# fluent/fluent-bit

Hardware: AMD Instinct MI355X
Metric: log records/sec (256B apache-combined lines) through parser+grep (higher is better)
Workload: dtype u8

## Files before the change

fluent-bit_amd/__init__.py:

```python
import ctypes
import os
import subprocess
from ctypes import (POINTER, Structure, byref, c_char_p, c_double, c_int, c_int64, c_size_t, c_uint,
                    c_uint64, c_void_p)

_HERE = os.path.dirname(os.path.abspath(__file__))
CSRC = os.path.join(_HERE, "csrc")
LIB_PATH = os.environ.get("FLBGPU_LIB") or os.path.join(CSRC, "libflbgpu.so")

MODIFIED, NOTOUCH = 1, 2


def build(force=False):
    if force:
        subprocess.run(["make", "-C", CSRC, "clean"], check=True, stdout=subprocess.DEVNULL)
    subprocess.run(["make", "-j8", "-C", CSRC, "all"], check=True)


class DevChunk(Structure):
    _fields_ = [("data", c_void_p), ("row_off", c_void_p), ("n", c_uint64), ("bytes", c_uint64)]


_L = None

# ... 134 lines not shown
def init(device=0):
    global _inited
    if lib().flbgpu_init(device) != 0:
        raise RuntimeError("flbgpu_init: " + last_error())
    _inited = True


class Parser:

    def __init__(self, regex=None, time_fmt=None, time_key=None, time_offset=None, time_keep=False,
                 time_strict=True, skip_empty=True, types=None, name="parser", format="regex", no_bare_keys=False, decoders=None,
                 time_zone=None, time_system_timezone=False):
        if format in ("logfmt", "ltsv"):
            self.h = lib().flbgpu_parser_create_kv(_b(name), _b(format), _b(time_fmt), _b(time_key), _b(time_offset), int(time_keep),
                                                   int(time_strict), int(no_bare_keys), _b(types))
        elif format == "json":
            self.h = lib().flbgpu_parser_create_json(_b(name), _b(time_fmt), _b(time_key), _b(time_offset), int(time_keep),
                                                     int(time_strict))
        else:
            self.h = lib().flbgpu_parser_create(_b(name), _b(regex), int(skip_empty), _b(time_fmt), _b(time_key),
                                                _b(time_offset), int(time_keep), int(time_strict), _b(types))
        if not self.h:
            raise ValueError("flbgpu_parser_create: " + last_error())
        for d in decoders or []:
            if lib().flbgpu_parser_add_decoder(self.h, int(bool(d[0])), _b(d[1]), _b(d[2]), _b(d[3] if len(d) > 3 else None)) != 0:
                raise ValueError("flbgpu_parser_add_decoder: " + last_error())
        if time_system_timezone and lib().flbgpu_parser_set_system_timezone(self.h, 1) != 0:
            err = last_error(); self.close()
            raise ValueError("flbgpu_parser_set_system_timezone: " + err)
        if time_zone and lib().flbgpu_parser_set_time_zone(self.h, _b(time_zone)) != 0:
            err = last_error(); self.close()
            raise ValueError("flbgpu_parser_set_time_zone: " + err)

    def do(self, buf):
        out = c_void_p(); sz = c_size_t(); sec = c_int64(); nsec = c_int64()
        r = lib().flbgpu_parser_do(self.h, buf, len(buf), byref(out), byref(sz), byref(sec), byref(nsec))
        if r < 0:
            return r, None, None
        data = ctypes.string_at(out, sz.value)
        _libc.free(out)
        return r, data, (sec.value, nsec.value)

    def close(self):
        if self.h:
            lib().flbgpu_parser_destroy(self.h)
            self.h = None


class _Filter:
    h = None

    def filter(self, data):
        out = c_void_p(); sz = c_size_t()
        r = lib().flbgpu_filter_run(self.h, data, len(data), byref(out), byref(sz))
        if r != MODIFIED:
            return r, None
        b = ctypes.string_at(out, sz.value) if sz.value else b""
        if out.value:
            _libc.free(out)
        return r, b

    def filter_dev(self, chunk, stream=None):
        out = DevChunk()
        r = lib().flbgpu_filter_run_dev(self.h, byref(chunk), byref(out), stream)
        return r, out

    def counts(self):
        a = c_uint64(); b = c_uint64()
        lib().flbgpu_filter_last_counts(self.h, byref(a), byref(b))
        return a.value, b.value

    def regex_corners(self):
        return int(lib().flbgpu_filter_regex_corners(self.h))

    def host_rules(self):
        o = (ctypes.c_uint64 * 4)()
        lib().flbgpu_filter_host_rules(self.h, o)
        return dict(rules=int(o[0]), values=int(o[1]), budget_over=int(o[2]), unhandled=int(o[3]))

    def paths(self):
        o = (ctypes.c_uint64 * 8)()
        lib().flbgpu_filter_paths(self.h, o)
        lp = int(o[0])
        return dict(single_pass=bool(lp & 1), three_port=bool(lp & 2), emit_time=bool(lp & 4), plain_emit=bool(lp & 8), rows_by_length=bool(lp & 16),
                    aside=dict(single_pass=bool(o[1]), three_port=bool(o[2]), emit_time=bool(o[3]), plain_emit=bool(o[4])),
                    tries=int(o[5]), returns=int(o[6]), calls=int(o[7]))

    def profile(self, enable=True):
        lib().flbgpu_filter_profile(self.h, int(enable))

    def profile_read(self):
        names = (c_char_p * 16)(); ms = (c_double * 16)(); ln = (c_uint64 * 16)()
        n = lib().flbgpu_filter_profile_read(self.h, 16, names, ms, ln)
        return {names[i].decode(): (ms[i], ln[i]) for i in range(n)}

    def close(self):
        if self.h:
            lib().flbgpu_filter_destroy(self.h)
            self.h = None


class FilterParser(_Filter):

    def __init__(self, key_name, parsers, reserve_data=False, preserve_key=False):
        self.parsers = list(parsers)
        arr = (c_void_p * len(parsers))(*[p.h for p in parsers])
        self.h = lib().flbgpu_filter_parser_create(_b(key_name), int(reserve_data), int(preserve_key), len(parsers), arr)
        if not self.h:
            raise ValueError("flbgpu_filter_parser_create: " + last_error())


class FilterGrep(_Filter):

    def __init__(self, rules, logical_op=None):
        n = len(rules)
        kinds = (c_char_p * max(n, 1))(*[_b(k) for k, _ in rules])
        vals = (c_char_p * max(n, 1))(*[_b(v) for _, v in rules])
        self.h = lib().flbgpu_filter_grep_create(n, kinds, vals, _b(logical_op))
        if not self.h:
            raise ValueError("flbgpu_filter_grep_create: " + last_error())


def _props(props):
    n = len(props)
    names = (c_char_p * max(n, 1))(*[_b(k) for k, _ in props])
    vals = (c_char_p * max(n, 1))(*[_b(v) for _, v in props])
    return n, names, vals


class FilterModify(_Filter):

    def __init__(self, props):
        self.h = lib().flbgpu_filter_modify_create(*_props(props))
        if not self.h:
            raise ValueError("flbgpu_filter_modify_create: " + last_error())

    def overread(self):
        return int(lib().flbgpu_modify_overread(self.h))


def modify_parse_check(props):
    buf = ctypes.create_string_buffer(1 << 16)
    if lib().flbgpu_modify_parse_check(*_props(props), buf, len(buf)) != 0:
        raise ValueError(last_error())
    return buf.value.decode()


class FilterRecordModifier(_Filter):

    def __init__(self, props):
        self.h = lib().flbgpu_filter_record_modifier_create(*_props(props))
        if not self.h:
            raise ValueError("flbgpu_filter_record_modifier_create: " + last_error())


def record_modifier_parse_check(props):
    buf = ctypes.create_string_buffer(1 << 17)
    if lib().flbgpu_record_modifier_parse_check(*_props(props), buf, len(buf)) != 0:
        raise ValueError(last_error())
    return buf.value.decode()


JSON_FORMAT = {"json": 1, "stream": 2, "lines": 3}
JSON_DATE = {"double": 0, "iso8601": 1, "epoch": 2, "java_sql_timestamp": 3, "epoch_ms": 4}


class JsonFormatter(_Filter):
# ... 767 lines not shown
```

fluent-bit_amd/csrc/flbgpu.cpp:

```cpp
#include <condition_variable>
#include <functional>
#include <atomic>
#include <chrono>
#include <mutex>
#include <thread>
#include "host_int.hpp"
#include "grep_lane.hpp"
#include "perm.hpp"

using namespace flbgpu;

static thread_local std::string g_err;
static int g_cus = 0;

int flbgpu::device_cus() { return g_cus; }

void flbgpu::set_err(const char *fmt, ...) {
    char buf[1024];
    va_list ap;
    va_start(ap, fmt);
    vsnprintf(buf, sizeof(buf), fmt, ap);
    va_end(ap);
    g_err = buf;
    if (getenv("FLBGPU_DEBUG")) fprintf(stderr, "[flbgpu] %s\n", buf);
// ... 888 lines not shown
        if ((int) f->rules.size() >= MAX_RULES) { set_err("filter_grep: more than %d rules", MAX_RULES); if (bt) rx::bt_free(bt); delete f; return nullptr; }
        f->rules.push_back(r);
        f->host_rx.push_back(bt);
        rule_field.push_back(field);
        rule_pat.push_back(sp + 1);
    }
    if (f->logical_op == OP_OR && f->rules.size() >= 2 && !f->has_host_rules && !getenv("FLBGPU_NO_MERGE")) {
        std::vector<std::string> keys;
        std::vector<std::vector<int>> members;
        for (size_t i = 0; i < f->rules.size(); i++) {
            size_t k = 0;
            while (k < keys.size() && keys[k] != rule_field[i]) k++;
            if (k == keys.size()) { keys.push_back(rule_field[i]); members.emplace_back(); }
            members[k].push_back((int) i);
        }
        auto inline_group = [&](const std::string &pat) -> std::string {
            const char *ps, *pe;
            unsigned opts;
            rx::split_flb_pattern(pat.c_str(), &ps, &pe, &opts);
            std::string fl;
            if (opts & rx::OPT_IGNORECASE) fl += 'i';
            if (opts & rx::OPT_MULTILINE) fl += 'm';
            if (opts & rx::OPT_EXTEND) fl += 'x';
            std::string g = "(?" + fl + ":" + std::string(ps, pe);
            if (opts & rx::OPT_EXTEND) g += "\n";
            return g + ")";
        };
        std::vector<GrepRule> out;
        const int type = f->rules[0].type;
        std::function<void(const std::string &, const std::vector<int> &)> merge = [&](const std::string &field, const std::vector<int> &idx) {
            if (idx.size() == 1) { out.push_back(f->rules[(size_t) idx[0]]); return; }
            std::string pat;
            for (size_t q = 0; q < idx.size(); q++) pat += (q ? "|" : "") + inline_group(rule_pat[(size_t) idx[q]]);
            GrepRule r;
            memset(&r, 0, sizeof(r));
            r.type = type;
            std::string why;
            if (compile_rule(field, pat.c_str(), r, f->rule_blobs, why)) { out.push_back(r); return; }
            const std::vector<int> a(idx.begin(), idx.begin() + (long) idx.size() / 2), b(idx.begin() + (long) idx.size() / 2, idx.end());
            merge(field, a);
            merge(field, b);
        };
        for (size_t k = 0; k < keys.size(); k++) merge(keys[k], members[k]);
        f->rules.swap(out);
        f->host_rx.assign(f->rules.size(), nullptr);
    }
    if (!filter_common_init(f) || !f->d_rules.ensure(std::max<size_t>(1, f->rules.size()) * sizeof(GrepRule))) { delete f; return nullptr; }
    if (!f->rules.empty() &&
        hipMemcpy(f->d_rules.p, f->rules.data(), f->rules.size() * sizeof(GrepRule), hipMemcpyHostToDevice) != hipSuccess) {
        set_err("upload failed");
        delete f;
        return nullptr;
    }
    return f;
}

extern "C" void flbgpu_filter_destroy(flbgpu_filter *f) { delete f; }

extern "C" int flbgpu_filter_paths(flbgpu_filter *f, uint64_t *out8) {
    if (!f || !out8) return -1;
    out8[0] = f->last_path; out8[1] = f->tile.off; out8[2] = f->fx5.off; out8[3] = f->defer.off; out8[4] = f->plain.off;
    out8[5] = f->tile.probes + f->fx5.probes + f->defer.probes + f->plain.probes;
    out8[6] = f->tile.returns + f->fx5.returns + f->defer.returns + f->plain.returns;
    out8[7] = f->calls;
    return 0;
}

extern "C" int flbgpu_filter_host_rules(flbgpu_filter *f, uint64_t *out4) {
    if (!f || !out4) return -1;
    uint64_t k = 0;
    for (auto *b : f->host_rx) if (b) k++;
    for (auto *p : f->parsers) if (p->bt) k++;
    out4[0] = k; out4[1] = f->host_values; out4[2] = f->host_budget_over; out4[3] = f->host_unhandled;
    if (f->l2m_gate) { for (auto *b : f->l2m_gate->host_rx) if (b) out4[0]++; out4[1] += f->l2m_gate->host_values; out4[2] += f->l2m_gate->host_budget_over; }
    return 0;
}

extern "C" void flbgpu_parser_destroy(flbgpu_parser *p) {
    if (!p) return;
    if (p->self_filter) delete p->self_filter;
    delete p;
}

struct MiscWords { unsigned long long first_bad; unsigned long long max_row; unsigned long long counts[18]; unsigned int ov_count; unsigned int kept_count; };
static const unsigned int OV_CAP = 1u << 16;

struct PairCtx { PgInline pg; uint32_t *keep_len; const flbgpu_filter *fg; uint32_t *desc; uint32_t dstride; };

struct HostView { const void *dev = nullptr; const uint8_t *host = nullptr; size_t bytes = 0; };
static thread_local HostView g_hostview;

template <class F> static void parallel_rows(uint64_t n, F fn) {
    unsigned nt = std::thread::hardware_concurrency();
    if (nt > 16) nt = 16;
    if (n < 4096 || nt < 2) { fn((uint64_t) 0, n); return; }
    std::vector<std::thread> th;
    const uint64_t per = ((n + nt - 1) / nt + 63) & ~63ull;
    for (unsigned t = 0; t < nt; t++) {
        const uint64_t a = (uint64_t) t * per, b = a + per < n ? a + per : n;
        if (a < b) th.emplace_back([=]() { fn(a, b); });
    }
    for (auto &t : th) t.join();
}

static bool host_chunk(const flbgpu_dev_chunk *in, hipStream_t st, std::vector<uint8_t> &copy, const uint8_t **data, std::vector<uint64_t> &off) {
    off.resize((size_t) in->n + 1);
    if (hipMemcpyAsync(off.data(), in->row_off, ((size_t) in->n + 1) * sizeof(uint64_t), hipMemcpyDeviceToHost, st) != hipSuccess) return false;
    if (g_hostview.dev == in->data && g_hostview.host && g_hostview.bytes >= in->bytes) *data = g_hostview.host;
    else {
        copy.resize((size_t) in->bytes + 16);
        if (hipMemcpyAsync(copy.data(), in->data, (size_t) in->bytes, hipMemcpyDeviceToHost, st) != hipSuccess) return false;
        *data = copy.data();
    }
    return hipStreamSynchronize(st) == hipSuccess;
}

struct SpecCall {
    bool on = false;
    bool last = false;
    uint8_t *sink = nullptr;
    uint64_t sink_cap = 0;
    bool sunk = false;
};
static thread_local SpecCall g_spec;
struct SpecOff {
    bool was;
    SpecOff() : was(g_spec.on) { g_spec.on = false; }
    ~SpecOff() { g_spec.on = was; }
};
static const uint64_t SPEC_MAX_RECORDS = 262144, SPEC_MAX_BYTES = 8u << 20;
static inline bool spec_wanted(uint64_t n, uint64_t bytes) { return n <= SPEC_MAX_RECORDS && bytes <= SPEC_MAX_BYTES && !getenv("FLBGPU_NO_SPEC"); }
static void note_fx5(flbgpu_filter *f, const MiscWords &hm, uint64_t n) {
    if (!f->last_fx5 || n < 64 || !f->parsers[0]->fx2b.ok) return;
    if (hm.counts[9] * 64 > n) f->fx5.bad(); else f->fx5.good();
}
static void note_unsettled(flbgpu_filter *f, const MiscWords &hm, uint64_t n) {
    if (n < 64 || !(f->last_path & 1u)) return;
    if (f->last_fx5 && f->parsers[0]->fx2b.ok && hm.counts[9] * 64 > n) return;
    if (hm.counts[9] * 8 > n || hm.counts[10] * 4 > n) f->tile.bad(); else f->tile.good();
}
static void note_lengths(flbgpu_filter *f, const MiscWords &hm) {
    if (hm.counts[17] == 0) return;
    const double ratio = (double) hm.counts[16] / (double) hm.counts[17];
    if (ratio > 1.35) f->sort_rows = true;
    else if (ratio < 1.15) f->sort_rows = false;
}
static bool ahead_counters_ok(flbgpu_filter *f, const MiscWords &hm, uint64_t n) {
    note_lengths(f, hm);
    note_fx5(f, hm, n);
    note_unsettled(f, hm, n);
    return hm.counts[8] == 0 && hm.counts[2] == 0 && hm.first_bad >= n;
}

static bool host_parser_rx(flbgpu_filter *f, const flbgpu_dev_chunk *in, const ParserMatchArgs &ma, hipStream_t st) {
    const uint64_t n = ma.n;
    const flbgpu_parser *hp = f->parsers[0];
    const DevParser &d = hp->dev;
    const int ncap = 2 * d.nfields;
    std::vector<uint32_t> info(3 * (size_t) n);
    HIPOK(hipMemcpyAsync(info.data(), ma.info, info.size() * sizeof(uint32_t), hipMemcpyDeviceToHost, st));
    std::vector<uint8_t> copy;
    std::vector<uint64_t> off;
    const uint8_t *hd = nullptr;
    if (!host_chunk(in, st, copy, &hd, off)) { set_err("filter_parser: copying the chunk back for the host parser failed"); return false; }
    std::vector<uint32_t> caps((size_t) ncap * n, 0u), tbuf((size_t) TBUF_WORDS * n, 0u);
    std::atomic<uint64_t> over{0}, vals{0}, unhandled{0};
    const uint64_t total_bytes = in->bytes;
// ... 814 lines not shown
    ga.status = f->d_status.as<uint32_t>(); ga.first_bad = &dm->first_bad; ga.counts = dm->counts;
    ga.nslots = own;
    for (size_t i = 0; i < f->rules.size(); i++) ga.slot_rule[ga.rule_slot[i]] = (uint8_t) i;
    GrepArgs &gb = la.g2;
    gb.data = ga.data; gb.row_off = ga.row_off; gb.n = n; gb.bytes = ga.bytes; gb.rules = f2->d_rules.as<GrepRule>();
    gb.nrules = (int) f2->rules.size(); gb.logical_op = f2->logical_op; gb.keep_len = ga.keep_len; gb.status = ga.status;
    gb.first_bad = ga.first_bad; gb.counts = ga.counts; gb.nslots = 0;
    la.two = 1;
    if (!lane_geometry(in, dm, st, la)) return 0;
    const uint64_t nunits = grep_lane_units(la.ntiles);
    if (!f->d_units.ensure(nunits * 8 + 8) || !f2->d_out.ensure(in->bytes + 32)) return 0;
    if (hipMemsetAsync(f->d_units.p, 0, nunits * 8, st) != hipSuccess) return 0;
    la.off_out = f->d_off.as<uint64_t>(); la.out = f2->d_out.as<uint8_t>(); la.out_cap = in->bytes;
    la.unit_state = f->d_units.as<unsigned long long>();
    la.ticket = &dm->counts[12]; la.words = &dm->counts[10];
    { ProfScope ps(f, st, "k_grep_lane(two instances)"); launch_grep_lane(la, g_cus > 0 ? g_cus : 256, st); }
    if (hipMemcpyAsync(&hm, dm, sizeof(hm), hipMemcpyDeviceToHost, st) != hipSuccess || hipStreamSynchronize(st) != hipSuccess) return 0;
    if (hm.counts[11]) return 0;
    f->calls++; f2->calls++;
    const uint64_t dec = hm.counts[0], kept1 = hm.counts[1], kept2 = hm.counts[2], bytes1 = hm.counts[3], bytes2 = hm.counts[10];
    memset(s2, 0, 2 * sizeof(*s2));
    *out = *in;
    f->last_in = f->last_out = dec; f2->last_in = f2->last_out = dec;
    s2[0].ret = s2[1].ret = FLBGPU_FILTER_NOTOUCH;
    s2[0].in_records = s2[0].out_records = s2[1].in_records = s2[1].out_records = dec;
    s2[0].out_bytes = s2[1].out_bytes = in->bytes;
    if (hm.first_bad != ~0ull || trailing_garbage) return 1;
    const bool mod1 = kept1 != dec;
    if (mod1) {
        f->last_out = kept1;
        s2[0].ret = FLBGPU_FILTER_MODIFIED; s2[0].out_records = kept1; s2[0].out_bytes = bytes1;
        if (bytes1 == 0) {
            memset(&s2[1], 0, sizeof(s2[1]));
            f2->last_in = f2->last_out = 0;
            memset(out, 0, sizeof(*out));
            out->data = f2->d_out.p; out->row_off = f->d_off.as<uint64_t>(); out->n = n; out->bytes = 0;
            return 1;
        }
        f2->last_in = f2->last_out = kept1;
        s2[1].in_records = s2[1].out_records = kept1; s2[1].out_bytes = bytes1;
    }
    const bool mod2 = kept2 != (mod1 ? kept1 : dec);
    if (mod2) {
        f2->last_out = kept2;
        s2[1].ret = FLBGPU_FILTER_MODIFIED; s2[1].out_records = kept2; s2[1].out_bytes = bytes2;
    }
    if (mod1 || mod2) { out->data = f2->d_out.p; out->row_off = f->d_off.as<uint64_t>(); out->n = n; out->bytes = bytes2; }
    return 1;
}

bool l2m_gate_dev(flbgpu_filter *gate, const flbgpu_dev_chunk *in, flbgpu_dev_chunk *kept, hipStream_t st) {
    const bool last0 = g_spec.last;
    g_spec.last = false;
    int ret = FLBGPU_FILTER_NOTOUCH;
    memset(kept, 0, sizeof(*kept));
    const bool ok = run_grep_dev(gate, in, kept, st, &ret, false);
    g_spec.last = last0;
    if (!ok) return false;
    if (gate->hp_misc.p && gate->hp_misc.as<MiscWords>()->first_bad != ~0ull) {
        set_err("log_to_metrics: a record of the chunk does not decode and the filter's rules run on the host: the chunk is not counted");
        return false;
    }
    if (ret != FLBGPU_FILTER_MODIFIED) *kept = *in;
    return true;
}

static bool pair_fusable(const flbgpu_filter *fp, const flbgpu_filter *fg) {
    if (getenv("FLBGPU_NO_FUSE")) return false;
    if (fp->kind != F_PARSER || fg->kind != F_GREP) return false;
    if (fp->has_decoders) return false;
    if (fp->pcfg.nparsers != 1 || fp->pcfg.key.is_ra || fp->pcfg.reserve_data || fp->pcfg.preserve_key) return false;
    const DevParser &d = fp->parsers[0]->dev;
    if (d.is_json || !d.plain_types || d.nfields > 32 || d.nfields == 0 || d.nregs_minus1 <= 0) return false;
    if (fg->rules.empty()) return false;
    if (d.utf8.nfa_on || d.ascii.stub) return false;
    for (const GrepRule &r : fg->rules) if (r.utf8.nfa_on) return false;
    if (fp->parsers[0]->bt || fp->host_list || fg->has_host_rules) return false;
    return true;
}

static std::atomic<uint64_t> g_fused_failures{0};
extern "C" uint64_t flbgpu_diag_fused_failures(void) { return g_fused_failures.load(); }

namespace flbgpu { void launch_pg_emit_plain(const PgEmitArgs &a, int nfields, int cus, hipStream_t st); }

static int run_pair_fused(flbgpu_filter *fp, flbgpu_filter *fg, const flbgpu_dev_chunk *in, flbgpu_dev_chunk *out, flbgpu_chain_stat *stats2) {
    hipStream_t st = fp->stream;
    uint64_t n = in->n;
    if (n == 0) return 0;
    MiscWords *dm = nullptr, *hmp = nullptr;
    const DevParser &d0 = fp->parsers[0]->dev;
    if (!fp->d_keep.ensure(n * sizeof(uint32_t))) return -1;
    static thread_local PairCtx pc;
    memset(&pc.pg, 0, sizeof(pc.pg));
    pc.keep_len = fp->d_keep.as<uint32_t>();
    pc.fg = fg;
    pc.dstride = (uint32_t) ((7 + d0.nfields + 15) / 16 * 16);
    pc.desc = nullptr;
    if (!getenv("FLBGPU_NO_DESC") && fp->d_desc.ensure(n * (size_t) pc.dstride * sizeof(uint32_t))) pc.desc = fp->d_desc.as<uint32_t>();
    pc.pg.rules = fg->d_rules.as<GrepRule>(); pc.pg.nrules = (int) fg->rules.size(); pc.pg.logical_op = fg->logical_op;
    for (int f = 0; f < d0.nfields; f++) {
        if (!d0.field_is_time[f]) continue;
        if (d0.time_keep) pc.pg.time_fields |= 1u << f; else pc.pg.static_drop |= 1u << f;
    }
    for (size_t i = 0; i < fg->rules.size(); i++) {
        uint32_t m = 0;
        const DevKey &k = fg->rules[i].key;
        for (int f = 0; f < d0.nfields; f++)
            if (d0.field_name_len[f] == k.key_len && !memcmp(d0.names + d0.field_name_off[f], k.key, (size_t) k.key_len)) m |= 1u << f;
        pc.pg.rule_fmask[i] = m;
        const DevDfa &df = fg->rules[i].dfa;
        pc.pg.rule_lds_bytes[i] = (uint32_t) ((df.d_final + df.nD) - df.cls);
    }
    if (!g_spec.on && hipMemsetAsync(pc.keep_len, 0xFF, n * sizeof(uint32_t), st) != hipSuccess) return -1;
    bool ahead = false;
    if (!parser_size_pass(fp, in, st, &dm, &hmp, &n, &pc, &ahead)) {
        if (fp->again) { fp->again = false; return run_pair_fused(fp, fg, in, out, stats2); }
        return -1;
    }
    MiscWords &hm = *hmp;
    uint64_t &total = *(uint64_t *) (fp->hp_misc.as<uint8_t>() + sizeof(MiscWords));
    if (!ahead && (n == 0 || hm.counts[3] > 0 || hm.ov_count > 0 || hm.counts[14] > 0)) return 0;
    const int cus = g_cus > 0 ? g_cus : 256;
    PgDecideArgs da;
    memset(&da, 0, sizeof(da));
    da.data = (const uint8_t *) in->data; da.row_off = in->row_off; da.n = n; da.n_cols = in->n;
    da.info = fp->d_info.as<uint32_t>(); da.caps = fp->d_caps.as<uint32_t>(); da.out_len = fp->d_len.as<uint32_t>();
    da.rules = pc.pg.rules; da.nrules = pc.pg.nrules; da.logical_op = pc.pg.logical_op;
    for (int i = 0; i < pc.pg.nrules; i++) {
        da.rule_fmask[i] = pc.pg.rule_fmask[i];
        da.rule_lds_off[i] = 0xFFFFFFFFu;
        if (da.lds_total + pc.pg.rule_lds_bytes[i] <= 48 * 1024) { da.rule_lds_off[i] = da.lds_total; da.rule_lds_bytes[i] = pc.pg.rule_lds_bytes[i]; da.lds_total += (pc.pg.rule_lds_bytes[i] + 15) & ~15u; }
    }
    da.keep_len = pc.keep_len; da.counts = dm->counts;
    if (ahead || hm.counts[7] > 0 || hm.counts[2] > 0) { ProfScope ps(fp, st, "k_pg_decide"); launch_pg_decide(da, cus, st); }
    { ProfScope ps(fp, st, "k_scan"); launch_scan(da.keep_len, n, fp->d_scan_tmp.as<uint64_t>(), fp->d_off.as<uint64_t>(), st); }
    total = 0;
    auto emit_args = [&](PgEmitArgs &ea) {
        memset(&ea, 0, sizeof(ea));
        ea.data = da.data; ea.row_off = da.row_off; ea.cfg = fp->pcfg; ea.parsers = fp->d_parsers.as<DevParser>(); ea.n_cols = in->n;
        ea.info = da.info; ea.caps = da.caps; ea.null_mask = fp->d_null.as<uint64_t>();
        ea.keep_len = da.keep_len; ea.n = n; ea.out_off = fp->d_off.as<uint64_t>(); ea.out = fg->d_out.as<uint8_t>();
        ea.desc = pc.desc; ea.dstride = pc.dstride; ea.bytes = in->bytes;
        ea.counts = dm->counts;
        fill_emit_cfg(fp, ea.ec);
    };
    auto defer_failed = [&](unsigned long long c13) -> bool {
        if (!(fp->last_path & 4u)) return false;
        if (c13 == 0) { fp->defer.good(); return false; }
        fp->defer.bad();
        return true;
    };
    auto plain_wanted = [&](const PgEmitArgs &ea) -> bool {
        const bool can = ea.ec.ok && pc.desc != nullptr && !getenv("FLBGPU_EMIT_GENERAL");
        const bool use = can && fp->plain.use(fp->calls);
        if (use) fp->last_path |= 8u;
        return use;
    };
    auto plain_result = [&](unsigned long long left, unsigned long long kept) { if (left * 16 > kept && kept >= 64) fp->plain.bad(); else fp->plain.good(); };
    if (ahead) {
        if (!fg->d_out.ensure(in->bytes * 2 + n * 64 + 65536 + 16)) return -1;
        PgEmitArgs ea;
        emit_args(ea);
        ea.out_cap = fg->d_out.cap - 16;
        const bool plain_emit = plain_wanted(ea);
        { ProfScope ps(fp, st, "k_pg_emit"); if (plain_emit) launch_pg_emit_plain(ea, d0.nfields, cus, st); else launch_pg_emit(ea, d0.nfields, cus, st); }
        uint8_t *sink = g_spec.last ? g_spec.sink : nullptr;
        launch_finish_to_host(ea.out, ea.out_cap, ea.out_off + n, sink, g_spec.sink_cap, dm, &hm, (uint32_t) sizeof(hm), &total, st);
        if (hipStreamSynchronize(st) != hipSuccess) return -1;
        if (plain_emit) plain_result(hm.counts[15], hm.counts[5]);
        if (defer_failed(hm.counts[13]) || (plain_emit && hm.counts[15] > 0) || !ahead_counters_ok(fp, hm, n) || hm.counts[3] > 0 || hm.counts[14] > 0 || hm.ov_count > 0 || total > ea.out_cap) {
            SpecOff usual;
            return run_pair_fused(fp, fg, in, out, stats2);
        }
        if (hm.counts[6] == 0 || hm.counts[5] == hm.counts[6]) return 0;
        fp->last_in = hm.counts[0]; fp->last_out = hm.counts[6];
        fg->last_in = hm.counts[6]; fg->last_out = hm.counts[5];
        if (stats2) {
            stats2[0].ret = FLBGPU_FILTER_MODIFIED; stats2[0].in_records = hm.counts[0]; stats2[0].out_records = hm.counts[6]; stats2[0].out_bytes = hm.counts[4];
            stats2[1].ret = FLBGPU_FILTER_MODIFIED; stats2[1].in_records = hm.counts[6]; stats2[1].out_records = hm.counts[5]; stats2[1].out_bytes = total;
        }
        memset(out, 0, sizeof(*out));
        if (total == 0) return 1;
        out->data = fg->d_out.p; out->row_off = fp->d_off.as<uint64_t>(); out->n = n; out->bytes = total;
        if (sink && total <= g_spec.sink_cap) g_spec.sunk = true;
        return 1;
    }
    if (hipMemcpyAsync(&hm, dm, sizeof(hm), hipMemcpyDeviceToHost, st) != hipSuccess ||
        hipMemcpyAsync(&total, fp->d_off.as<uint64_t>() + n, sizeof(uint64_t), hipMemcpyDeviceToHost, st) != hipSuccess ||
        hipStreamSynchronize(st) != hipSuccess) return -1;
    if (hm.counts[6] == 0 || hm.counts[5] == hm.counts[6] || hm.counts[14] > 0) return 0;
    fp->last_in = hm.counts[0]; fp->last_out = hm.counts[6];
    fg->last_in = hm.counts[6]; fg->last_out = hm.counts[5];
    if (stats2) {
        stats2[0].ret = FLBGPU_FILTER_MODIFIED; stats2[0].in_records = hm.counts[0]; stats2[0].out_records = hm.counts[6]; stats2[0].out_bytes = hm.counts[4];
        stats2[1].ret = FLBGPU_FILTER_MODIFIED; stats2[1].in_records = hm.counts[6]; stats2[1].out_records = hm.counts[5]; stats2[1].out_bytes = total;
    }
    memset(out, 0, sizeof(*out));
    if (total == 0) return 1;
    if (!fg->d_out.ensure(total + 16)) return -1;
    PgEmitArgs ea;
    emit_args(ea);
    const bool plain_emit = plain_wanted(ea);
    { ProfScope ps(fp, st, "k_pg_emit"); if (plain_emit) launch_pg_emit_plain(ea, d0.nfields, cus, st); else launch_pg_emit(ea, d0.nfields, cus, st); }
    unsigned long long *c13 = (unsigned long long *) (fp->hp_misc.as<uint8_t>() + sizeof(MiscWords) + sizeof(uint64_t));
    c13[0] = c13[1] = c13[2] = 0;
    if (hipMemcpyAsync(c13, &dm->counts[13], 3 * sizeof(unsigned long long), hipMemcpyDeviceToHost, st) != hipSuccess) return -1;
    if (hipStreamSynchronize(st) != hipSuccess) return -1;
    if (defer_failed(c13[0])) return run_pair_fused(fp, fg, in, out, stats2);
    if (plain_emit) plain_result(c13[2], hm.counts[5]);
    if (plain_emit && c13[2] > 0) {
        { ProfScope ps(fp, st, "k_pg_emit_general"); launch_pg_emit(ea, d0.nfields, cus, st); }
        if (hipStreamSynchronize(st) != hipSuccess) return -1;
    }
    out->data = fg->d_out.p; out->row_off = fp->d_off.as<uint64_t>(); out->n = n; out->bytes = total;
    return 1;
}

static int run_any_dev(flbgpu_filter *f, const flbgpu_dev_chunk *in, flbgpu_dev_chunk *out, hipStream_t st, bool garbage) {
    int ret = FLBGPU_FILTER_NOTOUCH;
    bool ok;
    f->calls++;
    if (f->kind == F_L2M) {
        ok = run_l2m_dev(f, in, st, &ret);
        if (ok && ret == FLBGPU_FILTER_MODIFIED && out) memset(out, 0, sizeof(*out));
    }
    else if (f->kind == F_MODIFY) ok = run_modify_dev(f, in, out, st, &ret, garbage);
    else if (f->kind == F_RECMOD) ok = run_recmod_dev(f, in, out, st, &ret, garbage);
    else ok = f->kind == F_PARSER ? run_parser_dev(f, in, out, st, &ret) : run_grep_dev(f, in, out, st, &ret, garbage);
    if (!ok) return FLBGPU_FILTER_NOTOUCH;
    return ret;
}

static bool tail_is_clean(const uint8_t *d, size_t len, size_t start) {
    uint64_t count[32];
    int top = 0;
    size_t p = start;
    for (;;) {
        if (p >= len) return true;
        const uint8_t c = d[p];
        const size_t q = p + 1;
        size_t e, k = 0, lb = 0;
        uint64_t n = 0;
        bool container = false;
        if (c <= 0x7f || c >= 0xe0 || c == 0xc0 || c == 0xc2 || c == 0xc3) e = q;
        else if (c == 0xc1) return false;
        else if (c >= 0xa0 && c <= 0xbf) { k = c & 0x1f; if (len - q < k) return q == len; e = q + k; }
        else if (c >= 0x90 && c <= 0x9f) { container = true; n = c & 0x0f; e = q; }
        else if (c >= 0x80 && c <= 0x8f) { container = true; n = 2u * (c & 0x0f); e = q; }
        else {
            switch (c) {
            case 0xcc: case 0xd0: k = 1; break;
            case 0xcd: case 0xd1: k = 2; break;
            case 0xce: case 0xd2: case 0xca: k = 4; break;
            case 0xcf: case 0xd3: case 0xcb: k = 8; break;
            case 0xd4: k = 2; break;
            case 0xd5: k = 3; break;
            case 0xd6: k = 5; break;
            case 0xd7: k = 9; break;
            case 0xd8: k = 17; break;
            case 0xc4: case 0xc7: case 0xd9: lb = 1; break;
            case 0xc5: case 0xc8: case 0xda: case 0xdc: case 0xde: lb = 2; break;
            default: lb = 4; break;
            }
            if (lb == 0) { if (len - q < k) return q == len; e = q + k; }
            else {
                if (len - q < lb) return q == len;
                for (size_t i = 0; i < lb; i++) n = (n << 8) | d[q + i];
                const size_t q2 = q + lb;
                if (c == 0xdc || c == 0xdd) { container = true; e = q2; }
                else if (c == 0xde || c == 0xdf) { container = true; n *= 2; e = q2; }
                else {
                    k = (size_t) n + ((c == 0xc7 || c == 0xc8 || c == 0xc9) ? 1 : 0);
                    if (len - q2 < k) return q2 == len;
                    e = q2 + k;
                }
            }
        }
        if (container) {
            if (top >= 32) return false;
            if (n > 0) { count[top++] = n; p = e; continue; }
        }
        p = e;
        for (;;) {
            if (top == 0) return false;
            if (--count[top - 1] > 0) break;
// ... 510 lines not shown
```

fluent-bit_amd/csrc/fused_kernels.inc:

```

__global__ void __launch_bounds__(256) k_pg_decide(PgDecideArgs a) {
    const uint32_t lane = threadIdx.x & 63;
    LDS_AS uint8_t *lds = (LDS_AS uint8_t *) g_lds;
    for (int i = 0; i < a.nrules; i++) {
        if (a.rule_lds_off[i] == 0xFFFFFFFFu) continue;
        const uint8_t *src = a.rules[i].dfa.cls;
        for (uint32_t k = threadIdx.x; k < a.rule_lds_bytes[i]; k += blockDim.x) lds[a.rule_lds_off[i] + k] = src[k];
    }
    __syncthreads();
    const uint64_t n = a.n, nc = a.n_cols;
    uint32_t n_out = 0, n_keep = 0;
    unsigned long long out_bytes = 0;
    for (uint64_t r = (uint64_t) blockIdx.x * blockDim.x + threadIdx.x; r < n; r += (uint64_t) gridDim.x * blockDim.x) {
        if (a.keep_len[r] != PG_UNDECIDED) continue;
        uint32_t keep_len = 0;
        const uint32_t out_len = a.out_len[r], flags = a.info[r], drop_m = a.info[12 * nc + r], val_off = a.info[1 * nc + r];
        const uint64_t roff = a.row_off[r];
        if (out_len) {
            n_out++;
            out_bytes += out_len;
            const uint8_t *rec = a.data + roff;
            bool keep;
            if (flags & RF_PARSED) {
                if (a.info[4 * nc + r] >= 0xfffffffeu) atomicAdd(&a.counts[14], 1ull);
// ... 99 lines not shown
                        int64_t tsec = ri.ts_sec, tnsec = ri.ts_nsec;
                        int64_t s2 = 0;
                        const bool tok = pge_time(a.data, a.bytes, roff + ri.val_off + tb, &ps, &s2);
                        if (tok && s2 != 0) { tsec = s2; tnsec = 0; }
                        if (!tok || encoder_refuses_time(tsec, tnsec)) atomicAdd(&a.counts[13], 1ull);
                        else { ri.ts_sec = (uint32_t) tsec; ri.ts_nsec = (uint32_t) tnsec; }
                    }
                }
                else if constexpr (!PLAIN) {
                    ri = rec_load(a.info, a.n_cols, r);
                    nm = a.null_mask[r];
                    if (ri.val_len < 0xFFFF && (ri.flags & RF_PARSED)) spans_to_lds(a.caps, a.n_cols, r, ncap, spans + lane, 64);
                }
            }
            const bool lds_caps = actv && (ri.flags & RF_PARSED) && ((fl & RF_DESC) || ri.val_len < 0xFFFF);
            uint32_t lo = 0;
            while (lo < nk) {
                const uint64_t batch_base = __shfl(o0, (int) lo, 64);
                const uint32_t align = (uint32_t) (batch_base & 15);
                const bool fit = lane >= lo && lane < nk && (o1 - batch_base + align) <= (uint64_t) PGE_STG;
                const uint64_t mask = __ballot(fit) >> lo;
                uint32_t m = (~mask == 0) ? 64 - lo : (uint32_t) __builtin_ctzll(~mask);
                if (m > nk - lo) m = nk - lo;
                const bool direct = m == 0;
                if (direct) m = 1;
                if constexpr (PLAIN) {
                    if (lane >= lo && lane < lo + m && o1 > o0) {
                        if (direct || !(lds_caps && a.ec.ok && ri.parser_idx == 0 && (fl & RF_DESC))) atomicAdd(&a.counts[15], 1ull);
                        else {
                            CapsLdsView cv;
                            cv.col = spans + lane; cv.stride = 64;
                            cv.base = a.caps; cv.n = a.n_cols; cv.r = r;
                            LdsSink sk(stg + align + (uint32_t) (o0 - batch_base));
                            sk.src_end = a.data + a.bytes;
                            sk.limit = sk.p + (uint32_t) (o1 - o0);
                            write_record_plain(sk, a.ec, a.data + roff, ri, cv);
                        }
                    }
                }
                else
                if (lane >= lo && lane < lo + m && o1 > o0) {
                    CapsLdsView cv;
                    cv.col = spans + lane; cv.stride = 64;
                    cv.base = a.caps; cv.n = a.n_cols; cv.r = r;
                    CapsView cg;
                    cg.base = a.caps; cg.n = a.n_cols; cg.r = r;
                    if (direct) {
                        ByteSink sk(a.out + o0);
                        sk.limit = a.out + o1;
                        if (lds_caps) write_record(sk, a.cfg, a.parsers, a.data + roff, a.data + roff1, ri, cv, nm);
                        else write_record(sk, a.cfg, a.parsers, a.data + roff, a.data + roff1, ri, cg, nm);
                    }
                    else {
                        LdsSink sk(stg + align + (uint32_t) (o0 - batch_base));
                        sk.src_end = a.data + a.bytes;
                        sk.limit = sk.p + (uint32_t) (o1 - o0);
                        if (lds_caps && a.ec.ok && ri.parser_idx == 0) write_record_plain(sk, a.ec, a.data + roff, ri, cv);
                        else if (lds_caps) write_record(sk, a.cfg, a.parsers, a.data + roff, a.data + roff1, ri, cv, nm);
                        else write_record(sk, a.cfg, a.parsers, a.data + roff, a.data + roff1, ri, cg, nm);
                    }
                }
                if (!direct) {
                    const uint32_t total = (uint32_t) (__shfl(o1, (int) (lo + m - 1), 64) - batch_base);
                    __builtin_amdgcn_fence(__ATOMIC_SEQ_CST, "workgroup");
                    uint8_t *dst = a.out + (batch_base - align);
                    const uint32_t n16 = (align + total + 15) / 16;
                    for (uint32_t u = lane; u < n16; u += 64) {
                        const uint32_t b0 = u * 16, b1 = b0 + 16;
                        if (b0 >= align && b1 <= align + total) *(v4u32 *) (dst + b0) = *(LDS_AS v4u32 *) (stg + b0);
                        else {
                            const uint32_t s0 = b0 < align ? align : b0, s1 = b1 > align + total ? align + total : b1;
                            for (uint32_t qq = s0; qq < s1; qq++) dst[qq] = stg[qq];
                        }
                    }
                    __builtin_amdgcn_fence(__ATOMIC_SEQ_CST, "workgroup");
                }
                lo += m;
            }
        }
        __builtin_amdgcn_fence(__ATOMIC_SEQ_CST, "workgroup");
    }
}

void launch_pg_decide(const PgDecideArgs &a, int cus, hipStream_t st) {
    if (a.n == 0) return;
    uint64_t blocks = (a.n + 255) / 256, cap = (uint64_t) cus * 16;
    if (blocks > cap) blocks = cap;
    hipLaunchKernelGGL(k_pg_decide, dim3((unsigned) blocks), dim3(256), a.lds_total, st, a);
}
static void launch_pg_emit_t(const PgEmitArgs &a, int nfields, int cus, hipStream_t st, bool plain) {
    if (a.n == 0) return;
    static std::atomic<bool> attr_set{false};
    if (!attr_set) {
        (void) hipFuncSetAttribute((const void *) k_pg_emit<false>, hipFuncAttributeMaxDynamicSharedMemorySize, 160 * 1024);
        (void) hipFuncSetAttribute((const void *) k_pg_emit<true>, hipFuncAttributeMaxDynamicSharedMemorySize, 160 * 1024);
        attr_set = true;
    }
    const uint32_t ncap = 2 * (uint32_t) nfields;
    const size_t lds = (size_t) 4 * (PGE_ROWS * 4 + ((ncap * 128 + 15) & ~15u) + (plain ? PGE_STG_PLAIN : PGE_STG_GENERAL));
    uint64_t blocks = (a.n + 4 * PGE_ROWS - 1) / (4 * PGE_ROWS), cap = (uint64_t) cus * (plain ? 12 : 8);
    if (blocks > cap) blocks = cap;
    if (plain) hipLaunchKernelGGL(k_pg_emit<true>, dim3((unsigned) blocks), dim3(256), lds, st, a);
    else hipLaunchKernelGGL(k_pg_emit<false>, dim3((unsigned) blocks), dim3(256), lds, st, a);
}
void launch_pg_emit(const PgEmitArgs &a, int nfields, int cus, hipStream_t st) { launch_pg_emit_t(a, nfields, cus, st, false); }
void launch_pg_emit_plain(const PgEmitArgs &a, int nfields, int cus, hipStream_t st) { launch_pg_emit_t(a, nfields, cus, st, true); }
```

fluent-bit_amd/csrc/kdev.inc:

```

#define DEV __device__ __forceinline__
#define LDS_AS __attribute__((address_space(3)))

extern __shared__ __attribute__((aligned(16))) uint8_t g_lds[];

DEV uint32_t ld8(const uint8_t *p) { return *p; }
DEV uint32_t ldu32(const uint8_t *p) {
    typedef uint32_t u32u __attribute__((aligned(1)));
    return *(const u32u *) p;
}
DEV uint32_t ldbe32(const uint8_t *p) { return __builtin_bswap32(ldu32(p)); }
DEV uint64_t ldbe64(const uint8_t *p) {
    typedef uint64_t u64u __attribute__((aligned(1)));
    return __builtin_bswap64(*(const u64u *) p);
}
DEV uint32_t ldbe16(const uint8_t *p) { return (ld8(p) << 8) | ld8(p + 1); }

typedef uint32_t v4u32 __attribute__((ext_vector_type(4)));
DEV uint32_t v4_byte(const v4u32 w, uint32_t i) {
    const uint64_t h = i < 8 ? ((uint64_t) w.x | ((uint64_t) w.y << 32)) : ((uint64_t) w.z | ((uint64_t) w.w << 32));
    return (uint32_t) (h >> (8 * (i & 7))) & 0xff;
}

struct CountSink {
    uint64_t n = 0;
    bool need_exact = false;
    DEV void note_exact() { need_exact = true; }
    DEV void put(uint32_t) { n++; }
    DEV void copy(const uint8_t *, uint32_t len) { n += len; }
    DEV void words(const uint32_t *, uint32_t nbytes) { n += nbytes; }
    DEV void put32(uint32_t) { n += 4; }
    DEV void put16(const v4u32, uint32_t nbytes) { n += nbytes; }
    DEV void finish() {}
};

struct ByteSink {
    uint8_t *p;
    uint8_t *limit = nullptr;
    DEV void note_exact() {}
    DEV explicit ByteSink(uint8_t *dst) : p(dst) {}
    DEV void put(uint32_t b) { *p++ = (uint8_t) b; }
    DEV void copy(const uint8_t *src, uint32_t len) {
        typedef uint32_t u32u __attribute__((aligned(1)));
        typedef uint32_t v4 __attribute__((ext_vector_type(4)));
        typedef v4 v4u __attribute__((aligned(1)));
        uint32_t i = 0;
        for (; i + 64 <= len; i += 64) {
            const v4 w0 = *(const v4u *) (src + i), w1 = *(const v4u *) (src + i + 16), w2 = *(const v4u *) (src + i + 32), w3 = *(const v4u *) (src + i + 48);
            *(v4u *) (p + i) = w0; *(v4u *) (p + i + 16) = w1; *(v4u *) (p + i + 32) = w2; *(v4u *) (p + i + 48) = w3;
        }
        for (; i + 16 <= len; i += 16) *(v4u *) (p + i) = *(const v4u *) (src + i);
        for (; i + 4 <= len; i += 4) *(u32u *) (p + i) = *(const u32u *) (src + i);
        for (; i < len; i++) p[i] = (uint8_t) ld8(src + i);
        p += len;
    }
    DEV void words(const uint32_t *w, uint32_t nbytes) {
        typedef uint32_t u32u __attribute__((aligned(1)));
        const uint32_t nw = (nbytes + 3) / 4;
        if (limit && p + 4 * nw <= limit) for (uint32_t i = 0; i < nw; i++) *(u32u *) (p + 4 * i) = w[i];
        else for (uint32_t i = 0; i < nbytes; i++) p[i] = (uint8_t) (w[i >> 2] >> (8 * (i & 3)));
        p += nbytes;
    }
    DEV void put32(uint32_t v) {
        typedef uint32_t u32u __attribute__((aligned(1)));
        *(u32u *) p = v;
        p += 4;
    }
    DEV void put16(const v4u32 w, uint32_t nbytes) {
        typedef v4u32 v4u __attribute__((aligned(1)));
        if (limit && p + 16 <= limit) *(v4u *) p = w;
        else for (uint32_t i = 0; i < nbytes; i++) p[i] = (uint8_t) v4_byte(w, i);
        p += nbytes;
    }
    DEV void finish() {}
};

struct LdsSink {
    __attribute__((address_space(3))) uint8_t *p;
    const uint8_t *src_end = nullptr;
    __attribute__((address_space(3))) uint8_t *limit = nullptr;
    DEV explicit LdsSink(__attribute__((address_space(3))) uint8_t *dst) : p(dst) {}
    DEV void note_exact() {}
    DEV void put(uint32_t b) { *p++ = (uint8_t) b; }
    DEV void copy(const uint8_t *src, uint32_t len) {
        typedef uint32_t u32u __attribute__((aligned(1)));
        typedef uint32_t v4 __attribute__((ext_vector_type(4)));
        typedef v4 v4u __attribute__((aligned(1)));
// ... 87 lines not shown
    else if (n < 65536) { s.put(0xde); pk_be(s, n, 2); }
    else { s.put(0xdf); pk_be(s, n, 4); }
}

enum { T_NIL, T_BOOL, T_UINT, T_NINT, T_F32, T_F64, T_STR, T_BIN, T_EXT, T_ARRAY, T_MAP, T_BAD };

struct Tok {
    int type;
    uint32_t len;
    uint64_t u;
    const uint8_t *next;
};

DEV uint64_t ldu64(const uint8_t *p) {
    typedef uint64_t u64u __attribute__((aligned(1)));
    return *(const u64u *) p;
}

DEV Tok mp_tok_w(uint64_t w, const uint8_t *p, const uint8_t *end) {
    Tok t;
    t.type = T_BAD; t.len = 0; t.u = 0; t.next = p;
    const uint32_t c = (uint32_t) (w & 0xff);
    p++;
    uint32_t need = 0;
    if (c <= 0x7f) { t.type = T_UINT; t.u = c; }
    else if (c >= 0xe0) { t.type = T_NINT; t.u = (uint64_t) (int64_t) (int8_t) c; }
    else if (c >= 0xa0 && c <= 0xbf) { t.type = T_STR; t.len = c & 31; }
    else if (c >= 0x90 && c <= 0x9f) { t.type = T_ARRAY; t.len = c & 15; }
    else if (c >= 0x80 && c <= 0x8f) { t.type = T_MAP; t.len = c & 15; }
    else {
        const uint32_t sh = 4 * (c & 15);
        const uint64_t ttab = c < 0xd0 ? 0x22225488877711b0ull : 0xaa99666888883333ull;
        const uint64_t ntab = c < 0xd0 ? 0x8421844214210000ull : 0x4242421000008421ull;
        t.type = (int) ((ttab >> sh) & 15);
        need = (uint32_t) ((ntab >> sh) & 15);
        if (t.type == T_BAD) return t;
        if (c >= 0xd4 && c <= 0xd8) t.len = 1u << (c - 0xd4);
        if (c == 0xc3) t.u = 1;
        if ((uint64_t) (end - p) < need) { t.type = T_BAD; return t; }
        if (need) {
            uint64_t v;
            if (need == 8) v = ldbe64(p);
            else {
                uint32_t x = (uint32_t) (w >> 8);
                v = need == 1 ? (x & 0xff) : need == 2 ? (((x & 0xff) << 8) | ((x >> 8) & 0xff)) : __builtin_bswap32(x);
            }
            p += need;
            if (t.type == T_UINT || t.type == T_F32 || t.type == T_F64) t.u = v;
            else if (t.type == T_NINT) {
                int64_t sv = need == 1 ? (int64_t) (int8_t) v : need == 2 ? (int64_t) (int16_t) v
                           : need == 4 ? (int64_t) (int32_t) v : (int64_t) v;
                if (sv >= 0) t.type = T_UINT;
                t.u = (uint64_t) sv;
            }
            else t.len = (uint32_t) v;
        }
        if (t.type == T_EXT) {
            if (p >= end) { t.type = T_BAD; return t; }
            t.u = (1 + need) < 8 ? (uint32_t) ((w >> (8 * (1 + need))) & 0xff) : ld8(p);
            p++;
        }
    }
    if (t.type == T_STR || t.type == T_BIN || t.type == T_EXT) {
        if ((uint64_t) (end - p) < t.len) { t.type = T_BAD; return t; }
    }
    t.next = p;
    return t;
}

DEV Tok mp_tok(const uint8_t *p, const uint8_t *end) {
    if (p >= end) {
        Tok t;
        t.type = T_BAD; t.len = 0; t.u = 0; t.next = p;
        return t;
    }
    uint64_t w;
    const uint32_t avail = (uint32_t) ((uint64_t) (end - p) < 9 ? (end - p) : 9);
    if (avail >= 8) w = ldu64(p);
    else { w = 0; for (uint32_t q = 0; q < avail; q++) w |= (uint64_t) ld8(p + q) << (8 * q); }
    return mp_tok_w(w, p, end);
}

constexpr uint32_t MP_MAX_OPEN = 32;
__device__ __noinline__ bool mp_depth_ok(const uint8_t *p, const uint8_t *end, uint32_t open);

DEV const uint8_t *mp_skip(const uint8_t *p, const uint8_t *end, uint32_t open = 2) {
    const uint8_t *p0 = p;
    uint64_t remaining = 1;
    uint32_t nopen = 0;
    while (remaining > 0) {
        Tok t = mp_tok(p, end);
        if (t.type == T_BAD) return nullptr;
        remaining--;
        p = t.next;
        if (t.type == T_STR || t.type == T_BIN || t.type == T_EXT) p += t.len;
        else if (t.type == T_ARRAY) { remaining += t.len; nopen++; }
        else if (t.type == T_MAP) { remaining += 2ull * t.len; nopen++; }
    }
    if (open + nopen > MP_MAX_OPEN && !mp_depth_ok(p0, end, open)) return nullptr;
    return p;
}

DEV const uint8_t *mp_end_of(const Tok &t, const uint8_t *p, const uint8_t *end, uint32_t open = 2) {
    if (t.type == T_BAD) return nullptr;
    if (t.type == T_ARRAY || t.type == T_MAP) return t.len == 0 ? (open >= MP_MAX_OPEN ? nullptr : t.next) : mp_skip(p, end, open);
    if (t.type == T_STR || t.type == T_BIN || t.type == T_EXT) return t.next + t.len;
    return t.next;
}

DEV uint32_t mp_canon_size_scalar(const Tok &t) {
    CountSink cs;
    switch (t.type) {
    case T_NIL: case T_BOOL: return 1;
    case T_UINT: pk_uint(cs, t.u); break;
    case T_NINT: pk_int(cs, (int64_t) t.u); break;
    case T_F32: return 5;
    case T_F64: return 9;
    case T_STR: pk_str_hdr(cs, t.len); cs.n += t.len; break;
    case T_BIN: pk_bin_hdr(cs, t.len); cs.n += t.len; break;
    case T_EXT: pk_ext_hdr(cs, t.len, (uint32_t) t.u); cs.n += t.len; break;
    default: break;
    }
    return (uint32_t) cs.n;
}

template <class S> DEV const uint8_t *mp_canon(const uint8_t *p, const uint8_t *end, S &s, uint32_t open = 2) {
    const uint8_t *p0 = p;
    uint64_t remaining = 1;
    uint32_t nopen = 0;
    while (remaining > 0) {
        Tok t = mp_tok(p, end);
        if (t.type == T_BAD) return nullptr;
        remaining--;
        p = t.next;
        switch (t.type) {
        case T_NIL: s.put(0xc0); break;
        case T_BOOL: s.put(t.u ? 0xc3 : 0xc2); break;
        case T_UINT: pk_uint(s, t.u); break;
        case T_NINT: pk_int(s, (int64_t) t.u); break;
        case T_F32: s.put(0xca); pk_be(s, t.u, 4); break;
        case T_F64: s.put(0xcb); pk_be(s, t.u, 8); break;
        case T_STR: pk_str_hdr(s, t.len); s.copy(p, t.len); p += t.len; break;
        case T_BIN: pk_bin_hdr(s, t.len); s.copy(p, t.len); p += t.len; break;
        case T_EXT: pk_ext_hdr(s, t.len, (uint32_t) t.u); s.copy(p, t.len); p += t.len; break;
        case T_ARRAY: pk_array_hdr(s, t.len); remaining += t.len; nopen++; break;
        case T_MAP: pk_map_hdr(s, t.len); remaining += 2ull * t.len; nopen++; break;
        }
    }
    if (open + nopen > MP_MAX_OPEN && !mp_depth_ok(p0, end, open)) return nullptr;
    return p;
}

__device__ __noinline__ bool mp_depth_ok(const uint8_t *p, const uint8_t *end, uint32_t open) {
    uint64_t stk[MP_MAX_OPEN];
    uint64_t cur = 1;
    uint32_t top = 0;
    for (;;) {
        Tok t = mp_tok(p, end);
        if (t.type == T_BAD) return false;
        p = t.next;
        cur--;
        if (t.type == T_STR || t.type == T_BIN || t.type == T_EXT) p += t.len;
        else if (t.type == T_ARRAY || t.type == T_MAP) {
            if (open + top >= MP_MAX_OPEN) return false;
            const uint64_t n = t.type == T_ARRAY ? (uint64_t) t.len : 2ull * t.len;
            if (n) { stk[top++] = cur; cur = n; }
        }
        while (cur == 0) {
            if (top == 0) return true;
            cur = stk[--top];
        }
    }
}

struct Event {
    uint32_t flags;
    int64_t sec, nsec;
    const uint8_t *meta;
    const uint8_t *meta_end;
    const uint8_t *body;
    const uint8_t *body_end;
};

DEV Event decode_event(const uint8_t *rec, const uint8_t *end, bool lazy_body = false) {
    Event ev;
    ev.flags = RF_BAD; ev.sec = 0; ev.nsec = 0; ev.meta = nullptr; ev.meta_end = nullptr; ev.body = nullptr; ev.body_end = nullptr;
    if (rec == end) { ev.flags = RF_VALID | RF_SKIP; return ev; }
    if ((uint64_t) (end - rec) >= 14 && ldu32(rec) == 0x00d79292u && ld8(rec + 12) == 0x80) {
        const uint32_t s0 = ldbe32(rec + 4), ns0 = ldbe32(rec + 8);
        Tok b0 = mp_tok(rec + 13, end);
        if (b0.type != T_MAP) return ev;
        if (s0 == 0xffffffffu || s0 == 0xfffffffeu) {
            if (ns0 != 0) return ev;
            ev.sec = s0 == 0xffffffffu ? -1 : -2;
        }
        else {
            if (ns0 >= 1000000000u) return ev;
            ev.sec = s0; ev.nsec = ns0;
        }
        ev.meta = rec + 12; ev.meta_end = rec + 13;
        ev.body = rec + 13;
        ev.body_end = lazy_body ? end : mp_skip(rec + 13, end, 1);
        if (!ev.body_end) return ev;
        ev.flags = RF_VALID;
        if (ev.sec < 0) ev.flags |= RF_SKIP;
        return ev;
    }
    Tok root = mp_tok(rec, end);
    if (root.type != T_ARRAY || root.len != 2) return ev;
    const uint8_t *p = root.next;
    Tok h = mp_tok(p, end);
    if (h.type == T_BAD) return ev;
    Tok ts;
    const uint8_t *after_header;
    if (h.type == T_ARRAY) {
        if (h.len != 2) return ev;
        ts = mp_tok(h.next, end);
        if (ts.type == T_BAD) return ev;
        const uint8_t *ts_end = ts.next + ((ts.type == T_EXT || ts.type == T_STR || ts.type == T_BIN) ? ts.len : 0);
        if (ts.type == T_ARRAY || ts.type == T_MAP) return ev;
        Tok m = mp_tok(ts_end, end);
        if (m.type != T_MAP) return ev;
        ev.meta = ts_end;
        ev.meta_end = mp_skip(ts_end, end);
        if (!ev.meta_end) return ev;
        after_header = ev.meta_end;
    }
    else {
        ts = h;
        if (ts.type == T_MAP) return ev;
        after_header = mp_skip(p, end, 1);
        if (!after_header) return ev;
    }
    if (ts.type != T_UINT && ts.type != T_F64 && ts.type != T_EXT) return ev;
    Tok b = mp_tok(after_header, end);
    if (b.type != T_MAP) return ev;
    ev.body = after_header;
    ev.body_end = lazy_body ? end : mp_skip(after_header, end, 1);
    if (!ev.body_end) return ev;
    if (ts.type == T_UINT) { ev.sec = (int64_t) ts.u; ev.nsec = 0; }
    else if (ts.type == T_F64) {
        double f = __longlong_as_double((long long) ts.u);
        ev.sec = (int64_t) f;
        ev.nsec = (int64_t) ((f - (double) ev.sec) * 1000000000);
    }
    else {
        if (ts.u != 0 || ts.len != 8) return ev;
        uint32_t s = ldbe32(ts.next), ns = ldbe32(ts.next + 4);
        if (s == 0xffffffffu || s == 0xfffffffeu) {
            if (ns != 0) return ev;
            ev.sec = s == 0xffffffffu ? -1 : -2;
            ev.nsec = 0;
        }
        else {
            if (ns >= 1000000000u) return ev;
            ev.sec = s; ev.nsec = ns;
        }
// ... 1197 lines not shown
    if (i < 64) return (mask >> i) & 1;
    unsigned int n = *cfg.ov_count;
    if (n > cfg.ov_cap) n = cfg.ov_cap;
    for (unsigned int k = 0; k < n; k++) if (cfg.ov_pairs[2 * (size_t) k] == r && cfg.ov_pairs[2 * (size_t) k + 1] == i) return true;
    return false;
}
DEV uint32_t null_count_high(const FParserCfg &cfg, uint64_t r) {
    unsigned int n = *cfg.ov_count;
    if (n == 0) return 0;
    if (n > cfg.ov_cap) n = cfg.ov_cap;
    uint32_t c = 0;
    for (unsigned int k = 0; k < n; k++) {
        if (cfg.ov_pairs[2 * (size_t) k] != r) continue;
        bool dup = false;
        for (unsigned int q = 0; q < k && !dup; q++) dup = cfg.ov_pairs[2 * (size_t) q] == r && cfg.ov_pairs[2 * (size_t) q + 1] == cfg.ov_pairs[2 * (size_t) k + 1];
        if (!dup) c++;
    }
    return c;
}

template <bool EXACT = false, int NW = 1, class S, class CV>
DEV void write_record(S &s, const FParserCfg &cfg, const DevParser *parsers, const uint8_t *rec, const uint8_t *rec_end,
                      const RecInfo &ri, const CV &caps, uint64_t null_mask) {
    s.put32(0x00d79292u); s.put32(__builtin_bswap32(ri.ts_sec)); s.put32(__builtin_bswap32(ri.ts_nsec));
    if (ri.meta_len > 1) mp_canon(rec + ri.meta_off, rec + ri.meta_off + ri.meta_len, s);
    else s.put(0x80);
    const uint8_t *body = rec + ri.body_off, *body_end = body + ri.body_len;
    if (!(ri.flags & RF_PARSED)) {
        mp_canon(body, body_end, s, 1);
        return;
    }
    const DevParser &ps = parsers[ri.parser_idx];
    Tok bm;
    bm.type = T_MAP; bm.len = 0; bm.u = 0; bm.next = body;
    uint32_t nappend = 0;
    bool plain_key = !cfg.key.is_ra;
    if (cfg.reserve_data || cfg.preserve_key) bm = mp_tok(body, body_end);
    if (cfg.reserve_data) {
        nappend = bm.len;
        if (plain_key && !cfg.preserve_key) {
            for (uint32_t i = 0; i < bm.len && i < 64; i++) if ((null_mask >> i) & 1) nappend--;
            if (bm.len > 64) nappend -= null_count_high(cfg, caps.r);
        }
    }
    else if (cfg.preserve_key && plain_key) nappend = 1;
    if (nappend > 0 || ps.is_json) pk_map_hdr(s, ri.nkept + nappend);
    else {
        uint32_t n0 = (uint32_t) ps.nregs_minus1;
        if (n0 < 16) s.put(0x80 | ri.nkept);
        else if (n0 < 65536) { s.put(0xde); pk_be(s, ri.nkept, 2); }
        else { s.put(0xdf); pk_be(s, ri.nkept, 4); }
    }
    const uint8_t *val = rec + ri.val_off;
    if (ps.kv_format) pkv_emit_pairs<EXACT>(ps, val, ri.val_len, s);
    else if (ps.is_json) {
        JsonCounts cc;
        cc.col = const_cast<uint32_t *>(caps.base); cc.n = caps.n; cc.r = caps.r; cc.store = false;
        pjson_emit_pairs<EXACT, NW>(val, ri.val_len, ri.drop_mask, s, cc);
    }
    else
    for (int f = 0; f < ps.nfields; f++) {
        if ((ri.drop_mask >> f) & 1) continue;
        uint32_t b = caps[2 * f], e = caps[2 * f + 1];
        uint32_t vlen = (b == CAP_UNSET || e == CAP_UNSET) ? 0 : e - b;
        const uint8_t *v = (b == CAP_UNSET || e == CAP_UNSET) ? val : val + b;
        s.words(ps.keywords + ps.kw_off[f], (uint32_t) ps.kw_bytes[f]);
        write_field_value<EXACT>(s, ps.field_type[f], v, vlen);
    }
    if (nappend > 0) {
        const uint8_t *p = bm.next;
        for (uint32_t i = 0; i < bm.len; i++) {
            const uint8_t *kend = mp_skip(p, body_end);
            const uint8_t *vend = kend ? mp_skip(kend, body_end) : nullptr;
            if (!vend) return;
            bool take;
            if (cfg.reserve_data) take = !(plain_key && !cfg.preserve_key && null_test(cfg, caps.r, i, null_mask));
            else take = (i == ri.key_index);
            if (take) { mp_canon(p, kend, s); mp_canon(kend, vend, s); }
            p = vend;
        }
    }
}

template <class S, class CV>
DEV void write_record_plain(S &s, const EmitCfg &ec, const uint8_t *rec, const RecInfo &ri, const CV &caps) {
    s.put32(0x00d79292u); s.put32(__builtin_bswap32(ri.ts_sec)); s.put32(__builtin_bswap32(ri.ts_nsec));
    if (ri.meta_len > 1) mp_canon(rec + ri.meta_off, rec + ri.meta_off + ri.meta_len, s);
    else s.put(0x80);
    const uint32_t n0 = (uint32_t) ec.nregs_minus1;
    if (n0 < 16) s.put(0x80 | ri.nkept);
    else if (n0 < 65536) { s.put(0xde); pk_be(s, ri.nkept, 2); }
    else { s.put(0xdf); pk_be(s, ri.nkept, 4); }
    const uint8_t *val = rec + ri.val_off;
    for (int f = 0; f < ec.nfields; f++) {
        if ((ri.drop_mask >> f) & 1) continue;
        const uint32_t b = caps[2 * f], e = caps[2 * f + 1];
        const bool set = b != CAP_UNSET && e != CAP_UNSET;
        const uint32_t vlen = set ? e - b : 0;
        s.words(ec.keywords + ec.kw_off[f], (uint32_t) ec.kw_bytes[f]);
        pk_str_hdr(s, vlen);
        s.copy(set ? val + b : val, vlen);
    }
}

#include "nfa_dev.inc"


template <class CAP>
DEV bool parser_fields_done(const DevParser &ps, const uint8_t *val, CAP &caps, int64_t *tsec, int64_t *tnsec, uint32_t *nkept, uint32_t *drop_mask, uint32_t dbg) {
    bool any = false;
    uint32_t kept = 0, drop = 0;
    int64_t sec = 0; double frac = 0;
    for (int f = 0; f < ps.nfields; f++) {
        uint32_t b = caps.get(2 * f), e = caps.get(2 * f + 1);
        bool set = (b != CAP_UNSET && e != CAP_UNSET);
        if (!set) { caps.set(2 * f, CAP_UNSET); caps.set(2 * f + 1, CAP_UNSET); }
        if (set) any = true;
        uint32_t fl = set ? e - b : 0;
        if (fl == 0 && ps.skip_empty) { drop |= 1u << f; continue; }
        if (ps.field_is_time[f] && !(dbg & 4)) {
            int64_t s2; double f2;
            if (time_lookup(ps, set ? val + b : val, fl, &s2, &f2) == -1) { drop |= 1u << f; continue; }
            sec = s2; frac = f2;
            if (!ps.time_keep) { drop |= 1u << f; continue; }
        }
        kept++;
    }
    if (!any) return false;
    *tsec = sec;
    *tnsec = (int64_t) (frac * 1000000000);
    *nkept = kept;
    *drop_mask = drop;
    return true;
}

template <bool LDS, class CAP>
DEV bool try_parser(const DevParser &ps, const HotTabs<LDS> &hot, const uint8_t *val, uint32_t vlen, uint16_t *chk, uint32_t chk_len, uint32_t nfa_off,
                    CAP &caps, int64_t *tsec, int64_t *tnsec, uint32_t *nkept, uint32_t *drop_mask, uint32_t dbg) {
    if (vlen / CHK_STEP + 2 > chk_len) return false;
    if (dbg & 1) return false;
    bool use_utf8 = false;
    uint32_t wlen = vlen;
    int best = ps.ascii.stub ? -2 : rx_reverse(hot, ps.ascii.r_info, val, vlen, chk);
    if (best == -2) rx_corner_note(ps.utf8, val, vlen);
    if (best == -2 && ps.utf8.nfa_on) {
        if (ps.nregs_minus1 <= 0) return false;
        if (nfa_off + nfa_chk_words(ps.utf8.nfa, vlen) * 2 > chk_len) return false;
        for (int f = 0; f < 2 * ps.nfields; f++) caps.set((uint32_t) f, CAP_UNSET);
        const uint32_t ln = threadIdx.x & 63;
        if (nfa_capture(ps.utf8.nfa, val, vlen, (uint32_t *) (chk - ln + (size_t) nfa_off * 64) + ln, ps.slot2cap, caps, nullptr) < 0) return false;
    }
    else {
    HotTabs<false> hu = hot_global(ps.utf8);
    if (best == -2) {
        use_utf8 = true;
        wlen = u8_walk_len(val, vlen);
        best = ps.utf8.wide ? rx_reverse(hot_global_wide(ps.utf8), ps.utf8.r_info, val, wlen, chk, vlen)
                            : rx_reverse(hu, ps.utf8.r_info, val, wlen, chk, vlen);
    }
    if (best < 0) return false;
    if (ps.nregs_minus1 <= 0) return false;
    for (int f = 0; f < 2 * ps.nfields; f++) caps.set((uint32_t) f, CAP_UNSET);
    if (dbg & 2) return false;
    int endb = !use_utf8 ? rx_forward(ps.ascii, hot, val, vlen, best, chk, ps.slot2cap, caps)
             : ps.utf8.wide ? rx_forward(ps.utf8, hot_global_wide(ps.utf8), val, wlen, best, chk, ps.slot2cap, caps, vlen)
                            : rx_forward(ps.utf8, hu, val, wlen, best, chk, ps.slot2cap, caps, vlen);
    if (endb < 0) return false;
    if (wlen != vlen) {
        for (int f = 0; f < 2 * ps.nfields; f++) if (caps.get((uint32_t) f) == wlen) caps.set((uint32_t) f, vlen);
    }
    }
    return parser_fields_done(ps, val, caps, tsec, tnsec, nkept, drop_mask, dbg);
}

template <class CAP>
DEV bool host_parser_answer(const DevParser &ps, const uint32_t *res, uint64_t n, uint64_t r, const uint8_t *val, uint32_t val_off, CAP &caps,
                            int64_t *tsec, int64_t *tnsec, uint32_t *nkept, uint32_t *drop_mask) {
    if (!res || res[r] != val_off + 1) return false;
    if (ps.nregs_minus1 <= 0) return false;
    for (int f = 0; f < 2 * ps.nfields; f++) caps.set((uint32_t) f, res[(size_t) (1 + f) * n + r]);
    return parser_fields_done(ps, val, caps, tsec, tnsec, nkept, drop_mask, 0u);
}


DEV void recinfo_init(RecInfo &ri) {
    ri.flags = 0; ri.val_off = 0; ri.val_len = 0; ri.key_index = 0; ri.ts_sec = 0; ri.ts_nsec = 0;
    ri.body_off = 0; ri.body_len = 0; ri.meta_off = 0; ri.meta_len = 0; ri.parser_idx = -1; ri.nkept = 0; ri.drop_mask = 0;
// ... 192 lines not shown
            if (a.logical_op == OP_OR && found) { GD_BRK; }
            if (a.logical_op == OP_AND && !found) { GD_BRK; }
        }
        if (a.nrules > 0) keep = (a.rules[last].type == GREP_REGEX) ? found : !found;
    }
    return keep;
}
#undef GD_BLOB
#undef GD_BRK

DEV uint32_t locate_core(const ParserMatchArgs &a, uint64_t r, const uint8_t *rec, const uint8_t *rec_end, uint32_t &n_dec, RecInfo &ri) {
    recinfo_init(ri);
    Event ev = decode_event(rec, rec_end, true);
    ri.flags = ev.flags;
    if (ev.flags & RF_BAD) {
        atomicMin(a.first_bad, (unsigned long long) r);
        return 0;
    }
    if (ev.flags & RF_SKIP) {
        if (rec != rec_end && mp_skip(ev.body, rec_end, 1) != rec_end) {
            ri.flags = RF_BAD;
            atomicMin(a.first_bad, (unsigned long long) r);
        }
        return 0;
    }
    n_dec++;
    ri.body_off = (uint32_t) (ev.body - rec); ri.body_len = (uint32_t) (ev.body_end - ev.body);
    if (ev.meta) { ri.meta_off = (uint32_t) (ev.meta - rec); ri.meta_len = (uint32_t) (ev.meta_end - ev.meta); }
    uint32_t ncand = 0;
    bool whole = false, have_canon = false;
    CountSink canon;
    if (a.cfg.key.is_ra) {
        const uint8_t *v = ra_resolve(a.cfg.key, ev.body, ev.body_end, &whole);
        if (v) {
            Tok t = mp_tok(v, ev.body_end);
            if (t.type == T_STR || t.type == T_BIN) { ri.val_off = (uint32_t) (t.next - rec); ri.val_len = t.len; ncand = 1; }
        }
    }
    else {
        Tok bm = mp_tok(ev.body, ev.body_end);
        const uint8_t *p = bm.next;
        pk_map_hdr(canon, bm.len);
        have_canon = true;
        for (uint32_t i = 0; i < bm.len; i++) {
            Tok kt = mp_tok(p, ev.body_end);
            const uint8_t *kend;
            if (kt.type == T_ARRAY || kt.type == T_MAP) kend = mp_canon(p, ev.body_end, canon);
            else { kend = mp_end_of(kt, p, ev.body_end); canon.n += mp_canon_size_scalar(kt); }
            if (!kend) { p = nullptr; break; }
            Tok vt = mp_tok(kend, ev.body_end);
            if (vt.type == T_ARRAY || vt.type == T_MAP) p = mp_canon(kend, ev.body_end, canon);
            else { p = mp_end_of(vt, kend, ev.body_end); canon.n += mp_canon_size_scalar(vt); }
            if (!p) break;
            if ((kt.type == T_STR || kt.type == T_BIN) && kt.len == (uint32_t) a.cfg.key.key_len &&
                bytes_eq(kt.next, a.cfg.key.key, kt.len) && (vt.type == T_STR || vt.type == T_BIN)) {
                if (ncand == 0) { ri.val_off = (uint32_t) (vt.next - rec); ri.val_len = vt.len; ri.key_index = i; }
                ncand++;
            }
        }
        whole = (p == ev.body_end);
    }
    if (!whole) {
        n_dec--;
        recinfo_init(ri);
        ri.flags = RF_BAD;
        atomicMin(a.first_bad, (unsigned long long) r);
        return 0;
    }
    if (ncand == 1 && a.caps_in_lds && ri.val_len < 0xFFFF && (ri.val_len / CHK_STEP + 2) <= a.chk_len) ri.flags |= RF_CAND;
    else if (ncand >= 1) { ri.flags |= RF_GENERIC; atomicAdd(&a.counts[2], 1ull); }
    uint32_t out_len = 0;
    if (ev.sec < 0 || (uint64_t) ev.sec > 0xffffffffull || ev.nsec < 0 || ev.nsec >= 1000000000LL) ri.flags |= RF_BADTS;
    else {
        ri.ts_sec = (uint32_t) ev.sec; ri.ts_nsec = (uint32_t) ev.nsec;
        CountSink cs;
        cs.n = 12;
        if (ev.meta) mp_canon(ev.meta, ev.meta_end, cs); else cs.n += 1;
        ri.meta_canon = (uint32_t) cs.n - 12;
        if (have_canon) cs.n += canon.n; else mp_canon(ev.body, ev.body_end, cs, 1);
        out_len = (uint32_t) cs.n;
    }
    return out_len;
}
```

fluent-bit_amd/csrc/kernels.hip:

```cpp
#include <hip/hip_runtime.h>
#include <stdint.h>
#include <string.h>
#include <type_traits>
#include "dev.hpp"
#include "numconv.hpp"
#include "dec.hpp"

namespace flbgpu {

#include "kdev.inc"
#include "dec_dev.inc"

constexpr int LOC_BLOCK = 256;
constexpr int LOC_TILE = 18432;


DEV uint32_t locate_one(const ParserMatchArgs &a, uint64_t r, const uint8_t *rec, const uint8_t *rec_end, uint32_t &n_dec) {
    RecInfo ri;
    const uint32_t out_len = locate_core(a, r, rec, rec_end, n_dec, ri);
    rec_store(a.info, a.n, r, ri);
    return out_len;
}

__global__ void __launch_bounds__(LOC_BLOCK) k_parser_locate(ParserMatchArgs a) {
// ... 75 lines not shown
    if (a.pg) {
        for (int i = 0; i < a.pg->nrules; i++) {
            if (a.pg->rule_lds_off[i] == 0xFFFFFFFFu) continue;
            const uint8_t *src = a.pg->rules[i].dfa.cls;
            for (uint32_t k = threadIdx.x; k < a.pg->rule_lds_bytes[i]; k += blockDim.x) pg_lds[a.pg->rule_lds_off[i] + k] = src[k];
        }
        __syncthreads();
    }
    for (uint64_t base = (uint64_t) wave_slot * 64; base < a.n; base += nwaves * 64) {
        const uint64_t r = base + lane;
        if (r >= a.n) continue;
        const uint32_t flags = a.info[r];
        if (!(flags & RF_CAND)) continue;
        const uint32_t vlen = a.info[2 * a.n + r];
        const uint8_t *val = a.data + a.row_off[r] + a.info[1 * a.n + r];
        if (ps.ascii.stub) {
            a.info[r] = flags | RF_GENERIC;
            n_gen++;
            continue;
        }
        int phase = (ps.fwd_first && ps.nregs_minus1 > 0) ? 0 : 1;
        int best = 0, endb = -1;
        for (;;) {
            if (phase == 1) {
                best = rx_reverse(hot0, ps.ascii.r_info, val, vlen, chk);
                if (best < 0 || ps.nregs_minus1 <= 0) break;
                phase = 2;
            }
            for (int c = 0; c < ncap; c++) capl.set((uint32_t) c, CAP_UNSET);
            endb = rx_forward(ps.ascii, hot0, val, vlen, phase == 0 ? 0 : best, phase == 0 ? (const uint16_t *) nullptr : chk, ps.slot2cap, capl);
            if (endb >= 0 || phase == 2) break;
            phase = 1;
        }
        if (endb >= 0) {
            for (int c = 0; c < ncap; c++) a.caps[(uint64_t) c * a.n + r] = capl.get((uint32_t) c);
            uint32_t pgbits = 0;
            if (a.pg) {
                uint32_t drop = a.pg->static_drop, any = 0;
                for (int f = 0; f < ps.nfields; f++) {
                    const uint32_t b = capl.get((uint32_t) (2 * f)), e = capl.get((uint32_t) (2 * f + 1));
                    const bool set = b != CAP_UNSET && e != CAP_UNSET;
                    any |= set ? 1u : 0u;
                    if ((!set || e == b) && ps.skip_empty) drop |= 1u << f;
                }
                uint32_t named = 0;
                for (int i = 0; i < a.pg->nrules; i++) named |= a.pg->rule_fmask[i];
                if (any && !(named & a.pg->time_fields & ~drop)) {
                    struct { const CapLds *c; DEV uint32_t operator[](uint32_t i) const { return c->get(i); } } cv{&capl};
                    const bool keep = pg_grep_parsed<true>(a.pg->rules, a.pg->nrules, a.pg->logical_op, a.pg->rule_fmask, a.pg->rule_lds_off, drop, val, cv,
                                                     (LDS_AS const uint8_t *) pg_lds);
                    pgbits = RF_PGDONE | (keep ? RF_PGKEEP : 0u);
                }
            }
            a.info[r] = flags | RF_RXOK | pgbits;
            if (ps.time_field >= 0) {
                const uint32_t tb = capl.get((uint32_t) (2 * ps.time_field)), te = capl.get((uint32_t) (2 * ps.time_field + 1));
                if (tb != CAP_UNSET && te != CAP_UNSET && te - tb <= 4 * TBUF_WORDS) {
                    const uint32_t tl = te - tb;
                    v4u32 w0 = load16(val + tb, 0, tl), w1 = load16(val + tb + 16, 0, tl > 16 ? tl - 16 : 0);
                    a.tbuf[0 * a.n + r] = w0.x; a.tbuf[1 * a.n + r] = w0.y; a.tbuf[2 * a.n + r] = w0.z; a.tbuf[3 * a.n + r] = w0.w;
                    a.tbuf[4 * a.n + r] = w1.x; a.tbuf[5 * a.n + r] = w1.y; a.tbuf[6 * a.n + r] = w1.z; a.tbuf[7 * a.n + r] = w1.w;
                }
            }
        }
        else if (best == -2 || a.cfg.nparsers > 1) {
            a.info[r] = flags | RF_GENERIC;
            n_gen++;
        }
    }
    for (int o = 32; o > 0; o >>= 1) n_gen += __shfl_down(n_gen, o, 64);
    if (lane == 0 && n_gen) atomicAdd(&a.counts[2], (unsigned long long) n_gen);
}

constexpr int FIN_SLOT = 4 * TBUF_WORDS + 4;
__global__ void __launch_bounds__(256) __attribute__((amdgpu_waves_per_eu(4, 8))) k_parser_finish(ParserMatchArgs a) {
    __shared__ __attribute__((aligned(16))) uint8_t tls_mem[256 * FIN_SLOT];
    __shared__ char fmt_mem[2 * MAX_TIMEFMT];
    LDS_AS uint8_t *tls = (LDS_AS uint8_t *) tls_mem;
    const DevParser &ps = a.parsers[0];
    for (uint32_t i = threadIdx.x; i < 2 * MAX_TIMEFMT; i += blockDim.x) fmt_mem[i] = i < MAX_TIMEFMT ? ps.fmt1[i] : ps.fmt2[i - MAX_TIMEFMT];
    __syncthreads();
    LDS_AS const char *lfmt1 = (LDS_AS const char *) fmt_mem, *lfmt2 = lfmt1 + MAX_TIMEFMT;
    uint32_t n_gen = 0, pg_out = 0, pg_keep = 0, pg_pending = 0;
    unsigned long long pg_bytes = 0;
    const bool size_from_columns = !a.cfg.reserve_data && !(a.cfg.preserve_key && !a.cfg.key.is_ra) && ps.plain_types;
    const uint64_t n = a.n;
    for (uint64_t r = (uint64_t) blockIdx.x * blockDim.x + threadIdx.x; r < n; r += (uint64_t) gridDim.x * blockDim.x) {
        const uint32_t fl0 = a.info[r];
        if (fl0 & RF_PARSED) continue;
        if (!(fl0 & RF_RXOK) || (fl0 & RF_GENERIC)) {
            if (!(fl0 & RF_GENERIC)) a.null_mask[r] = 0;
            if (a.pg_keep_len) { a.pg_keep_len[r] = PG_UNDECIDED; pg_pending++; }
            continue;
        }
        CapsView caps;
        caps.base = a.caps; caps.n = n; caps.r = r;
        bool any = false;
        uint32_t kept = 0, drop = 0, body_bytes = 0;
        int64_t sec = 0; double frac = 0;
        for (int f = 0; f < ps.nfields; f++) {
            uint32_t b = caps[2 * f], e = caps[2 * f + 1];
            bool set = (b != CAP_UNSET && e != CAP_UNSET);
            if (set) any = true;
            uint32_t fl = set ? e - b : 0;
            if (fl == 0 && ps.skip_empty) { drop |= 1u << f; continue; }
            if (ps.field_is_time[f]) {
                int64_t s2; double f2;
                TStr in;
                const uint8_t *tv;
                if (f == ps.time_field && fl <= 4 * TBUF_WORDS) {
                    LDS_AS uint32_t *slot = (LDS_AS uint32_t *) (tls + threadIdx.x * FIN_SLOT);
                    #pragma unroll
                    for (int k = 0; k < TBUF_WORDS; k++) slot[k] = fl > (uint32_t) (4 * k) ? a.tbuf[(uint64_t) k * n + r] : 0;
                    in.lds = (LDS_AS const uint8_t *) slot; in.in_lds = true;
                    tv = (const uint8_t *) 4096;
                }
                else {
                    const uint8_t *val = a.data + a.row_off[r] + a.info[1 * n + r];
                    tv = set ? val + b : val;
                }
                if (in.in_lds && ps.plan.ok && fl == (uint32_t) ps.plan.len && time_fast(ps, in.lds, &s2)) f2 = 0;
                else if (time_lookup_in(ps, in, tv, fl, &s2, &f2, lfmt1, lfmt2) == -1) { drop |= 1u << f; continue; }
                sec = s2; frac = f2;
                if (!ps.time_keep) { drop |= 1u << f; continue; }
            }
            kept++;
            const uint32_t nl = (uint32_t) ps.field_name_len[f];
            body_bytes += (nl < 32 ? 1 : nl < 256 ? 2 : nl < 65536 ? 3 : 5) + nl + (fl < 32 ? 1 : fl < 256 ? 2 : fl < 65536 ? 3 : 5) + fl;
        }
        if (!any) {
            if (a.cfg.nparsers > 1) { a.info[r] = fl0 | RF_GENERIC; n_gen++; }
            else a.null_mask[r] = 0;
            if (a.pg_keep_len) { a.pg_keep_len[r] = PG_UNDECIDED; pg_pending++; }
            continue;
        }
        uint32_t flags = (fl0 | RF_PARSED) & ~(uint32_t) RF_BADTS;
        const uint32_t key_index = a.info[3 * n + r];
        uint64_t null_mask = 0;
        if (!a.cfg.key.is_ra) null_note(a.cfg, r, key_index, null_mask);
        int64_t tsec = a.info[4 * n + r], tnsec = a.info[5 * n + r];
        if (fl0 & RF_BADTS) { tsec = -3; tnsec = 0; }
        int64_t psec = sec, pnsec = (int64_t) (frac * 1000000000);
        bool have_parsed_time = ((uint64_t) psec * 1000000000ull + (uint64_t) pnsec) != 0;
        if (have_parsed_time) { tsec = psec; tnsec = pnsec; }
        a.null_mask[r] = null_mask;
        a.info[10 * n + r] = 0;
        a.info[11 * n + r] = kept;
        a.info[12 * n + r] = drop;
        if (encoder_refuses_time(tsec, tnsec)) {
            a.info[r] = flags | RF_BADTS;
            a.out_len[r] = 0;
            if (a.pg_keep_len) a.pg_keep_len[r] = 0;
            continue;
        }
        a.info[r] = flags;
        a.info[4 * n + r] = (uint32_t) tsec; a.info[5 * n + r] = (uint32_t) tnsec;
        if ((uint32_t) tsec >= 0xfffffffeu) atomicAdd(&a.counts[14], 1ull);
        if (size_from_columns) {
            const uint32_t n0 = (uint32_t) ps.nregs_minus1;
            a.out_len[r] = 12 + a.info[13 * n + r] + (n0 < 16 ? 1 : n0 < 65536 ? 3 : 5) + body_bytes;
        }
        else {
            RecInfo ri = rec_load(a.info, n, r);
            const uint8_t *rec = a.data + a.row_off[r];
            CountSink cs;
            write_record(cs, a.cfg, a.parsers, rec, a.data + a.row_off[r + 1], ri, caps, null_mask);
            a.out_len[r] = (uint32_t) cs.n;
            if (cs.need_exact) { a.info[r] = flags | RF_EXACT; atomicAdd(&a.counts[3], 1ull); }
        }
        if (a.pg_keep_len) {
            const uint32_t ol = a.out_len[r];
            if (fl0 & RF_PGDONE) {
                const bool keep = (fl0 & RF_PGKEEP) != 0;
                a.pg_keep_len[r] = keep ? ol : 0;
                pg_out++; pg_bytes += ol; pg_keep += keep ? 1u : 0u;
            }
            else { a.pg_keep_len[r] = PG_UNDECIDED; pg_pending++; }
        }
    }
    for (int o = 32; o > 0; o >>= 1) {
        n_gen += __shfl_down(n_gen, o, 64);
        pg_out += __shfl_down(pg_out, o, 64); pg_keep += __shfl_down(pg_keep, o, 64); pg_pending += __shfl_down(pg_pending, o, 64);
        pg_bytes += __shfl_down(pg_bytes, o, 64);
    }
    if ((threadIdx.x & 63) == 0) {
        if (n_gen) atomicAdd(&a.counts[2], (unsigned long long) n_gen);
        if (pg_bytes) atomicAdd(&a.counts[4], pg_bytes);
        if (pg_keep) atomicAdd(&a.counts[5], (unsigned long long) pg_keep);
        if (pg_out) atomicAdd(&a.counts[6], (unsigned long long) pg_out);
        if (pg_pending) atomicAdd(&a.counts[7], (unsigned long long) pg_pending);
    }
}

__device__ __noinline__ void pjson_try_wide(const DevParser *ps, const uint8_t *v, uint32_t vlen, uint32_t *caps_base, uint64_t n, uint64_t r,
                                            LDS_AS uint8_t *slot, PjsonTry *out) {
    JsonCounts cc;
    cc.col = caps_base; cc.n = n; cc.r = r; cc.store = true; cc.next = 0;
    *out = pjson_try<true, JSON_GENERIC_WORDS>(*ps, v, vlen, cc, slot);
}
__device__ __noinline__ uint32_t size_record_wide(const FParserCfg *cfg, const DevParser *parsers, const uint8_t *rec, const uint8_t *rec_end,
                                                  const RecInfo *ri, const uint32_t *caps_base, uint64_t n, uint64_t r, uint64_t null_mask) {
    CapsView caps;
    caps.base = caps_base; caps.n = n; caps.r = r;
    CountSink cs;
    write_record<true, JSON_GENERIC_WORDS>(cs, *cfg, parsers, rec, rec_end, *ri, caps, null_mask);
    return (uint32_t) cs.n;
}

__global__ void __launch_bounds__(256) k_parser_generic(ParserMatchArgs a) {
    __shared__ __attribute__((aligned(16))) uint8_t gen_slots[256 * 64];
    LDS_AS uint8_t *slot = (LDS_AS uint8_t *) gen_slots + threadIdx.x * 64;
    const uint32_t lane = threadIdx.x & 63;
    const uint32_t wave_slot = (blockIdx.x * blockDim.x + threadIdx.x) >> 6;
    const uint64_t nwaves = ((uint64_t) gridDim.x * blockDim.x) >> 6;
    uint16_t *chk = a.chk + ((size_t) wave_slot * a.chk_len) * 64 + lane;
    for (uint64_t base = (uint64_t) wave_slot * 64; base < a.n; base += nwaves * 64) {
        uint64_t r = base + lane;
        if (r >= a.n) continue;
        if (!(a.info[r] & RF_GENERIC)) continue;
        const uint8_t *rec = a.data + a.row_off[r];
        const uint8_t *rec_end = a.data + a.row_off[r + 1];
        RecInfo ri;
        recinfo_init(ri);
        uint64_t null_mask = 0;
        CapsView caps;
        caps.base = a.caps; caps.n = a.n; caps.r = r;
        Event ev = decode_event(rec, rec_end);
        ri.flags = ev.flags;
        ri.body_off = (uint32_t) (ev.body - rec); ri.body_len = (uint32_t) (ev.body_end - ev.body);
        if (ev.meta) { ri.meta_off = (uint32_t) (ev.meta - rec); ri.meta_len = (uint32_t) (ev.meta_end - ev.meta); }
        int64_t tsec = ev.sec, tnsec = ev.nsec;
        bool have_out = false, last_ok = false;
        Tok bm = mp_tok(ev.body, ev.body_end);
        const uint8_t *p = bm.next;
        uint32_t nkv = a.cfg.key.is_ra ? 1 : bm.len;
        for (uint32_t i = 0; i < nkv; i++) {
            const uint8_t *vptr = nullptr;
            uint32_t vlen = 0;
            if (a.cfg.key.is_ra) {
                const uint8_t *v = ra_resolve(a.cfg.key, ev.body, ev.body_end);
                if (v) {
                    Tok t = mp_tok(v, ev.body_end);
                    if (t.type == T_STR || t.type == T_BIN) { vptr = t.next; vlen = t.len; }
                }
            }
            else {
                Tok kt = mp_tok(p, ev.body_end);
                const uint8_t *kend = mp_skip(p, ev.body_end);
                Tok vt = mp_tok(kend, ev.body_end);
                p = mp_skip(kend, ev.body_end);
                if ((kt.type == T_STR || kt.type == T_BIN) && kt.len == (uint32_t) a.cfg.key.key_len &&
                    bytes_eq(kt.next, a.cfg.key.key, kt.len) && (vt.type == T_STR || vt.type == T_BIN)) { vptr = vt.next; vlen = vt.len; }
            }
            if (!vptr) continue;
            for (int q = 0; q < a.cfg.nparsers; q++) {
                int64_t ps = 0, pn = 0; uint32_t nk = 0, dm = 0;
                CapGlobal capg;
                capg.base = a.caps; capg.n = a.n; capg.r = r;
                if (a.parsers[q].is_json) {
                    PjsonTry t;
                    if (a.parsers[q].kv_format) t = pkv_try(a.parsers[q], vptr, vlen);
                    else pjson_try_wide(&a.parsers[q], vptr, vlen, a.caps, a.n, r, slot, &t);
                    last_ok = t.ok;
                    ps = t.sec; pn = t.nsec; nk = t.npairs; dm = t.skip;
                }
                else if (a.parsers[q].host_only)
                    last_ok = host_parser_answer(a.parsers[q], a.host_res[a.parsers[q].host_slot & (MAX_HOST_PARSERS - 1)], a.n, r, vptr, (uint32_t) (vptr - rec), capg, &ps, &pn, &nk, &dm);
                else
                last_ok = try_parser(a.parsers[q], hot_global(a.parsers[q].ascii), vptr, vlen, chk, a.chk_len, a.chk_nfa_off, capg, &ps, &pn, &nk, &dm, 0u);
                if (last_ok) {
                    have_out = true;
// ... 520 lines not shown
```

fluent-bit_amd/csrc/kernels_fused.hip:

```cpp
#include <hip/hip_runtime.h>
#include <stdint.h>
#include <string.h>
#include <type_traits>
#include "dev.hpp"
#include "numconv.hpp"

namespace flbgpu {

#include "kdev.inc"

#include "fused_kernels.inc"

}
```

fluent-bit_amd/csrc/tile_kernels.inc:

```

#include <utility>

constexpr uint32_t FX_CAP_STRIDE = 128;

DEV uint32_t fx_special(uint32_t e, uint32_t cn, LDS_AS const uint8_t *lds, uint32_t p2_at, LDS_AS uint8_t *capcol, uint32_t j) {
    if (!(e & 0x40000000u)) {
        e = *(LDS_AS const uint32_t *) (lds + ((e & FX_ROW_MASK) + cn));
        if ((int32_t) e >= 0) return e;
    }
    LDS_AS const uint32_t *p2 = (LDS_AS const uint32_t *) (lds + p2_at) + 2 * (e & 0x3FFFFFFFu);
    *(LDS_AS uint16_t *) (capcol + p2[1]) = (uint16_t) j;
    return p2[0];
}

DEV uint32_t fx_pair_do(uint32_t e, uint32_t p2_at, LDS_AS uint8_t *capcol, uint32_t j) {
    LDS_AS const uint32_t *p2 = (LDS_AS const uint32_t *) (uintptr_t) (p2_at + 8 * (e & 0x3FFFFFFFu));
    *(LDS_AS uint16_t *) (capcol + p2[1]) = (uint16_t) j;
    return p2[0];
}
DEV uint32_t fx_pair(uint32_t e, LDS_AS const uint8_t *lds, uint32_t p2_at, LDS_AS uint8_t *capcol, uint32_t j) {
    if ((int32_t) e < 0) {
        LDS_AS const uint32_t *p2 = (LDS_AS const uint32_t *) (lds + p2_at) + 2 * (e & 0x3FFFFFFFu);
        *(LDS_AS uint16_t *) (capcol + p2[1]) = (uint16_t) j;
        e = p2[0];
    }
    return e;
}

DEV uint32_t fx_walk(LDS_AS const uint8_t *lds, const DevFx &fx, uint32_t vaddr, uint32_t ngroups, LDS_AS uint8_t *capcol) {
    LDS_AS const uint32_t *clsT = (LDS_AS const uint32_t *) lds;
    LDS_AS const uint32_t *vw = (LDS_AS const uint32_t *) (lds + (vaddr & ~3u));
    const uint32_t sh = (vaddr & 3u) * 8, p2_at = fx.off_p2;
    uint32_t e = fx.start_off, j = 0;
    uint32_t dlo = vw[0], dhi = vw[1];
    uint32_t w = __builtin_amdgcn_alignbit(dhi, dlo, sh);
    uint32_t c0 = clsT[w & 255], c1 = clsT[(w >> 8) & 255], c2 = clsT[(w >> 16) & 255], c3 = clsT[w >> 24];
#define FX_STEP(ck, cn)                                                                      \
    {                                                                                        \
        e = *(LDS_AS const uint32_t *) (lds + ((e & FX_ROW_MASK) + (ck)));                   \
        if (__builtin_expect((int32_t) e < 0, 0)) e = fx_special(e, (cn), lds, p2_at, capcol, j); \
        *(LDS_AS uint16_t *) (capcol + (e >> FX_SLOT_SHIFT)) = (uint16_t) j;                 \
        j++;                                                                                 \
    }
    #pragma unroll 1
    for (uint32_t g = 0; g < ngroups; g++) {
        dlo = dhi; dhi = vw[g + 2];
        const uint32_t wn = __builtin_amdgcn_alignbit(dhi, dlo, sh);
        const uint32_t n0 = clsT[wn & 255], n1 = clsT[(wn >> 8) & 255], n2 = clsT[(wn >> 16) & 255], n3 = clsT[wn >> 24];
        FX_STEP(c0, c1) FX_STEP(c1, c2) FX_STEP(c2, c3) FX_STEP(c3, n0)
        c0 = n0; c1 = n1; c2 = n2; c3 = n3;
    }
#undef FX_STEP
    return e & FX_ROW_MASK;
}

__device__ __noinline__ int tile_capture_slow(const DevParser *ps, const uint8_t *val, uint32_t vlen, uint16_t *chk, LDS_AS uint8_t *capcol, uint32_t cap_step = FX_CAP_STRIDE) {
    HotTabs<false> h = hot_global(ps->ascii);
    const int best = rx_reverse(h, ps->ascii.r_info, val, vlen, chk);
    if (best < 0) return best;
    CapLds c;
    c.base = capcol; c.stride_b = cap_step;
    for (int i = 0; i < 2 * ps->nfields; i++) c.set((uint32_t) i, CAP_UNSET);
    return rx_forward(ps->ascii, h, val, vlen, best, chk, ps->slot2cap, c);
}

struct TileCaps {
    CapLds c;
    DEV uint32_t operator[](uint32_t i) const { return c.get(i); }
};

__global__ void __launch_bounds__(512) k_parser_tile(ParserMatchArgs a) {
    const uint32_t lane = threadIdx.x & 63, wave = threadIdx.x >> 6;
    LDS_AS uint8_t *lds = (LDS_AS uint8_t *) g_lds;
    const DevParser &ps = a.parsers[0];
    const DevFx fx = ps.fx;
    {
        typedef uint32_t v4u __attribute__((ext_vector_type(4)));
        const v4u *src = (const v4u *) fx.base;
        LDS_AS v4u *dst = (LDS_AS v4u *) g_lds;
        for (uint32_t i = threadIdx.x; i < fx.bytes / 16; i += blockDim.x) dst[i] = src[i];
        if (a.pg) {
            LDS_AS uint8_t *pg_lds = lds + a.pg_lds_off;
            for (int i = 0; i < a.pg->nrules; i++) {
                if (a.pg->rule_lds_off[i] == 0xFFFFFFFFu) continue;
                const uint8_t *rs = a.pg->rules[i].dfa.cls;
                for (uint32_t k = threadIdx.x; k < a.pg->rule_lds_bytes[i]; k += blockDim.x) pg_lds[a.pg->rule_lds_off[i] + k] = rs[k];
            }
        }
        __syncthreads();
    }
    const uint32_t tile_off = a.tile_lds_off + wave * a.tile_wave_bytes;
    LDS_AS uint8_t *tile = lds + tile_off;
    LDS_AS uint8_t *capcol = tile + TILE_BYTES + 2 * lane;
    CapLds capl;
    capl.base = capcol; capl.stride_b = FX_CAP_STRIDE;
    const uint32_t wave_slot = (blockIdx.x * blockDim.x + threadIdx.x) >> 6;
    const uint64_t nwaves = ((uint64_t) gridDim.x * blockDim.x) >> 6;
    uint16_t *chk = a.chk + ((size_t) wave_slot * a.chk_len) * 64 + lane;
    const uint8_t *data_end = a.data + a.bytes;
    const int ncap = 2 * ps.nfields;
    const bool size_from_columns = !a.cfg.reserve_data && !(a.cfg.preserve_key && !a.cfg.key.is_ra) && ps.plain_types;
    const uint64_t n = a.n;
    uint32_t n_dec = 0, n_gen = 0, n_fin = 0, n_slow = 0, pg_out = 0, pg_keep = 0, pg_pending = 0;
    unsigned long long pg_bytes = 0;
    for (uint64_t base = (uint64_t) wave_slot * 64; base < n; base += nwaves * 64) {
        const uint64_t r = base + lane;
        const uint32_t cnt = (uint32_t) ((n - base) < 64 ? (n - base) : 64);
        uint64_t o0 = 0, o1 = 0;
        if (lane < cnt) { o0 = a.row_off[r]; o1 = a.row_off[r + 1]; }
        uint32_t lo = 0;
        while (lo < cnt) {
            const uint64_t g0 = __shfl(o0, (int) lo, 64);
            const uint32_t align = (uint32_t) (g0 & 15);
            const bool fit = lane >= lo && lane < cnt && (o1 - g0 + align) < (uint64_t) TILE_BYTES;
            const uint64_t mask = __ballot(fit) >> lo;
            uint32_t m = (~mask == 0) ? 64 - lo : (uint32_t) __builtin_ctzll(~mask);
            if (m > cnt - lo) m = cnt - lo;
            const bool direct = (m == 0);
            if (direct) m = 1;
            if (!direct) {
                const uint32_t total = (uint32_t) (__shfl(o1, (int) (lo + m - 1), 64) - g0) + align;
                const uint8_t *src = a.data + (g0 - align);
                typedef uint32_t v4 __attribute__((ext_vector_type(4)));
                for (uint32_t u = lane; u * 16 < total; u += 64) {
                    const uint8_t *p = src + (size_t) u * 16;
                    v4 v;
                    if (p + 16 <= data_end) v = *(const v4 *) p;
                    else {
                        uint32_t t4[4] = {0, 0, 0, 0};
                        for (int q = 0; q < 16 && p + q < data_end; q++) t4[q >> 2] |= (uint32_t) p[q] << (8 * (q & 3));
                        v.x = t4[0]; v.y = t4[1]; v.z = t4[2]; v.w = t4[3];
                    }
                    *(LDS_AS v4 *) (tile + (size_t) u * 16) = v;
                }
                __builtin_amdgcn_fence(__ATOMIC_SEQ_CST, "workgroup");
            }
            const bool act = lane >= lo && lane < lo + m;
            RecInfo ri;
            recinfo_init(ri);
            uint32_t out_len = 0, rec_lds = 0;
            const uint8_t *recg = a.data + o0;
            if (act) {
                const uint8_t *rec, *rec_end;
                if (direct) { rec = recg; rec_end = a.data + o1; }
                else { rec_lds = align + (uint32_t) (o0 - g0); rec = (const uint8_t *) (tile + rec_lds); rec_end = rec + (o1 - o0); }
                out_len = locate_core(a, r, rec, rec_end, n_dec, ri);
                if (direct && (ri.flags & RF_CAND)) { ri.flags = (ri.flags & ~(uint32_t) RF_CAND) | RF_GENERIC; atomicAdd(&a.counts[2], 1ull); }
            }
            const bool cand = act && (ri.flags & RF_CAND);
            const uint32_t vlen = ri.val_len;
            __builtin_amdgcn_fence(__ATOMIC_SEQ_CST, "workgroup");
            if (cand) {
                tile[rec_lds + ri.val_off + vlen] = 0xFF;
                for (uint32_t c = 0; c < fx.nslots; c++) *(LDS_AS uint16_t *) (capcol + c * FX_CAP_STRIDE) = 0xFFFF;
            }
            uint32_t maxlen = cand ? vlen : 0;
            for (int o = 32; o > 0; o >>= 1) { const uint32_t t = (uint32_t) __shfl_xor((int) maxlen, o, 64); maxlen = t > maxlen ? t : maxlen; }
            maxlen = (uint32_t) __builtin_amdgcn_readfirstlane((int) maxlen);
            __builtin_amdgcn_fence(__ATOMIC_SEQ_CST, "workgroup");
            int endb = -1;
            if (cand) {
                const uint32_t S = fx_walk(lds, fx, tile_off + rec_lds + ri.val_off, maxlen / 4 + 1, capcol);
                const uint32_t e_eot = capl.get((uint32_t) ncap + FXS_END_EOT - 1), e_mid = capl.get((uint32_t) ncap + FXS_END_MID - 1),
                               d_eot = capl.get((uint32_t) ncap + FXS_DEAD_EOT - 1), failed = capl.get((uint32_t) ncap + FXS_FAIL - 1);
                int res;
                if (S == fx.poison_off) res = -2;
                else if (failed != CAP_UNSET) res = 0;
                else if (e_mid != CAP_UNSET) { res = 1; endb = (int) e_mid; }
                else if (e_eot != CAP_UNSET) { if (e_eot == vlen) { res = 1; endb = (int) vlen; } else res = -2; }
                else if (d_eot != CAP_UNSET) res = d_eot == vlen ? 0 : -2;
                else res = 0;
                if (res == -2) endb = -2;
                else if (res == 0) { n_slow++; endb = tile_capture_slow(&ps, recg + ri.val_off, vlen, chk, capcol); }
            }
            if (act) {
                uint32_t flags = ri.flags;
                bool done = false;
                bool caps_valid = false, will_finish = false;
                uint32_t keep_len = PG_UNDECIDED;
                uint64_t null_mask = 0;
                if (cand && endb >= 0) {
                    flags |= RF_RXOK;
                    caps_valid = true;
                    bool any = false, slow = !size_from_columns;
                    uint32_t kept = 0, drop = 0, body_bytes = 0, pgdrop = a.pg ? a.pg->static_drop : 0;
                    int64_t sec = 0;
                    for (int f = 0; f < ps.nfields; f++) {
                        const uint32_t b = capl.get((uint32_t) (2 * f)), e = capl.get((uint32_t) (2 * f + 1));
                        const bool set = b != CAP_UNSET && e != CAP_UNSET;
                        any |= set;
                        const uint32_t fl = set ? e - b : 0;
                        if (fl == 0 && ps.skip_empty) { drop |= 1u << f; pgdrop |= 1u << f; continue; }
                        if (ps.field_is_time[f]) {
                            int64_t s2;
                            if (f == ps.time_field && ps.plan.ok && fl == (uint32_t) ps.plan.len &&
                                time_fast(ps, (LDS_AS const uint8_t *) (tile + rec_lds + ri.val_off + b), &s2)) sec = s2;
                            else { slow = true; continue; }
                            if (!ps.time_keep) { drop |= 1u << f; continue; }
                        }
                        kept++;
                        const uint32_t nl = (uint32_t) ps.field_name_len[f];
                        body_bytes += (nl < 32 ? 1 : nl < 256 ? 2 : nl < 65536 ? 3 : 5) + nl + (fl < 32 ? 1 : fl < 256 ? 2 : fl < 65536 ? 3 : 5) + fl;
                    }
                    uint32_t pgbits = 0;
                    if (a.pg && any) {
                        uint32_t named = 0;
                        for (int i = 0; i < a.pg->nrules; i++) named |= a.pg->rule_fmask[i];
                        if (!(named & a.pg->time_fields & ~pgdrop)) {
                            TileCaps cv{capl};
                            const bool keep = pg_grep_parsed<true>(a.pg->rules, a.pg->nrules, a.pg->logical_op, a.pg->rule_fmask, a.pg->rule_lds_off, pgdrop,
                                                             recg + ri.val_off, cv, (LDS_AS const uint8_t *) (lds + a.pg_lds_off));
                            pgbits = RF_PGDONE | (keep ? RF_PGKEEP : 0u);
                        }
                    }
                    flags |= pgbits;
                    if (!any) {
                        if (a.cfg.nparsers > 1) { flags |= RF_GENERIC; n_gen++; }
                    }
                    else if (slow) {
                        n_fin++;
                        will_finish = true;
                        if (ps.time_field >= 0) {
                            const uint32_t tb = capl.get((uint32_t) (2 * ps.time_field)), te = capl.get((uint32_t) (2 * ps.time_field + 1));
                            if (tb != CAP_UNSET && te != CAP_UNSET && te - tb <= 4 * TBUF_WORDS) {
                                const uint32_t tl = te - tb;
                                const uint8_t *tv = recg + ri.val_off + tb;
                                v4u32 w0 = load16(tv, 0, tl), w1 = load16(tv + 16, 0, tl > 16 ? tl - 16 : 0);
                                a.tbuf[0 * n + r] = w0.x; a.tbuf[1 * n + r] = w0.y; a.tbuf[2 * n + r] = w0.z; a.tbuf[3 * n + r] = w0.w;
                                a.tbuf[4 * n + r] = w1.x; a.tbuf[5 * n + r] = w1.y; a.tbuf[6 * n + r] = w1.z; a.tbuf[7 * n + r] = w1.w;
                            }
                        }
                    }
                    else {
                        done = true;
                        if (!a.cfg.key.is_ra) null_note(a.cfg, r, ri.key_index, null_mask);
                        int64_t tsec = ri.ts_sec, tnsec = ri.ts_nsec;
                        if (flags & RF_BADTS) { tsec = -3; tnsec = 0; }
                        if (sec != 0) { tsec = sec; tnsec = 0; }
                        flags = (flags | RF_PARSED) & ~(uint32_t) RF_BADTS;
                        ri.parser_idx = 0; ri.nkept = kept; ri.drop_mask = drop;
                        if (encoder_refuses_time(tsec, tnsec)) {
                            flags |= RF_BADTS;
                            out_len = 0;
                            keep_len = 0;
                        }
                        else {
                            ri.ts_sec = (uint32_t) tsec; ri.ts_nsec = (uint32_t) tnsec;
                            if ((uint32_t) tsec >= 0xfffffffeu) atomicAdd(&a.counts[14], 1ull);
                            const uint32_t n0 = (uint32_t) ps.nregs_minus1;
                            out_len = 12 + ri.meta_canon + (n0 < 16 ? 1 : n0 < 65536 ? 3 : 5) + body_bytes;
                            if (a.pg_keep_len) {
                                if (pgbits & RF_PGDONE) {
                                    const bool keep = (pgbits & RF_PGKEEP) != 0;
                                    keep_len = keep ? out_len : 0;
                                    pg_out++; pg_bytes += out_len; pg_keep += keep ? 1u : 0u;
                                }
                                else pg_pending++;
                            }
                        }
                    }
                }
                else if (cand && (endb == -2 || a.cfg.nparsers > 1)) {
                    flags |= RF_GENERIC;
                    n_gen++;
                }
                ri.flags = flags;
                if (!done) {
                    if (!will_finish) {
                        if (!(flags & RF_GENERIC)) a.null_mask[r] = 0;
                        if (a.pg_keep_len) { a.pg_keep_len[r] = PG_UNDECIDED; pg_pending++; }
                    }
                    rec_store(a.info, n, r, ri);
                    a.out_len[r] = out_len;
                    if (caps_valid) for (int c = 0; c < ncap; c++) a.caps[(uint64_t) c * n + r] = capl.get((uint32_t) c);
                }
                else {
                    const bool dropped = a.pg_keep_len && keep_len == 0;
                    if (a.pg_keep_len) a.pg_keep_len[r] = keep_len;
                    if (dropped) a.info[r] = flags;
                    else {
                        rec_store(a.info, n, r, ri);
                        a.null_mask[r] = null_mask;
                        a.out_len[r] = out_len;
                        for (int c = 0; c < ncap; c++) a.caps[(uint64_t) c * n + r] = capl.get((uint32_t) c);
                    }
                }
            }
            __builtin_amdgcn_fence(__ATOMIC_SEQ_CST, "workgroup");
            lo += m;
        }
    }
    for (int o = 32; o > 0; o >>= 1) {
        n_dec += __shfl_down(n_dec, o, 64); n_gen += __shfl_down(n_gen, o, 64); n_fin += __shfl_down(n_fin, o, 64); n_slow += __shfl_down(n_slow, o, 64);
        pg_out += __shfl_down(pg_out, o, 64); pg_keep += __shfl_down(pg_keep, o, 64); pg_pending += __shfl_down(pg_pending, o, 64);
        pg_bytes += __shfl_down(pg_bytes, o, 64);
    }
    if (lane == 0) {
        if (n_dec) atomicAdd(&a.counts[0], (unsigned long long) n_dec);
        if (n_gen) atomicAdd(&a.counts[2], (unsigned long long) n_gen);
        if (n_fin) atomicAdd(&a.counts[8], (unsigned long long) n_fin);
        if (n_slow) atomicAdd(&a.counts[9], (unsigned long long) n_slow);
        if (pg_bytes) atomicAdd(&a.counts[4], pg_bytes);
        if (pg_keep) atomicAdd(&a.counts[5], (unsigned long long) pg_keep);
        if (pg_out) atomicAdd(&a.counts[6], (unsigned long long) pg_out);
        if (pg_pending) atomicAdd(&a.counts[7], (unsigned long long) pg_pending);
    }
}

#ifndef REG_STREAM
#define REG_STREAM 0
#endif
constexpr int REG_THREADS = 1024;
constexpr uint32_t REG_TSLOT = 4 * TBUF_WORDS + 4;

__device__ __noinline__ v4u32 ld16_tail(const uint8_t *p, const uint8_t *data_end) {
    v4u32 v;
    uint32_t t4[4] = {0, 0, 0, 0};
    for (int q = 0; q < 16 && p + q < data_end; q++) t4[q >> 2] |= (uint32_t) ld8(p + q) << (8 * (q & 3));
    v.x = t4[0]; v.y = t4[1]; v.z = t4[2]; v.w = t4[3];
    return v;
}
DEV v4u32 ld16_guard(const uint8_t *p, const uint8_t *data_end) {
    if (__builtin_expect(p + 16 <= data_end, 1)) return ldu128(p);
    return ld16_tail(p, data_end);
}

template <int I> DEV uint32_t reg_qw(const v4u32 (&q)[18]) {
    if constexpr (I >= 68) return 0u;
    else if constexpr ((I & 3) == 0) return q[I >> 2].x;
    else if constexpr ((I & 3) == 1) return q[I >> 2].y;
    else if constexpr ((I & 3) == 2) return q[I >> 2].z;
    else return q[I >> 2].w;
}
template <int N> struct RegArr { uint32_t v[N]; };
template <int N, int... Is>
DEV RegArr<N> reg_sel_q(const v4u32 (&q)[18], bool b, std::integer_sequence<int, Is...>) { return RegArr<N>{{(b ? reg_qw<Is + 32>(q) : reg_qw<Is>(q))...}}; }
template <int N, int SH, int... Is>
DEV RegArr<N> reg_sel(const RegArr<N + SH> &in, bool b, std::integer_sequence<int, Is...>) { return RegArr<N>{{(b ? in.v[Is + SH] : in.v[Is])...}}; }
template <int L>
DEV void reg_extract(const v4u32 (&q)[18], uint32_t d0, uint32_t (&out)[L]) {
    const RegArr<L + 31> a32 = reg_sel_q<L + 31>(q, (d0 & 32) != 0, std::make_integer_sequence<int, L + 31>{});
    const RegArr<L + 15> a16 = reg_sel<L + 15, 16>(a32, (d0 & 16) != 0, std::make_integer_sequence<int, L + 15>{});
    const RegArr<L + 7> a8 = reg_sel<L + 7, 8>(a16, (d0 & 8) != 0, std::make_integer_sequence<int, L + 7>{});
    const RegArr<L + 3> a4 = reg_sel<L + 3, 4>(a8, (d0 & 4) != 0, std::make_integer_sequence<int, L + 3>{});
    const RegArr<L + 1> a2 = reg_sel<L + 1, 2>(a4, (d0 & 2) != 0, std::make_integer_sequence<int, L + 1>{});
    const RegArr<L> a1 = reg_sel<L, 1>(a2, (d0 & 1) != 0, std::make_integer_sequence<int, L>{});
    #pragma unroll
    for (int i = 0; i < L; i++) out[i] = a1.v[i];
}
template <int N>
DEV void reg_text(const v4u32 (&q)[18], uint32_t pos, uint32_t (&w)[N]) {
    uint32_t t[N + 1];
    reg_extract<N + 1>(q, pos >> 2, t);
    const uint32_t sh = (pos & 3) * 8;
    #pragma unroll
    for (int i = 0; i < N; i++) w[i] = __builtin_amdgcn_alignbit(t[i + 1], t[i], sh);
}
template <int N, int... Is>
DEV RegArr<N> reg_first(const v4u32 (&q)[18], std::integer_sequence<int, Is...>) { return RegArr<N>{{reg_qw<Is>(q)...}}; }
DEV uint32_t reg_dword_head(const v4u32 (&q)[18], uint32_t pos) {
    const uint32_t d0 = pos >> 2;
    const RegArr<17> all = reg_first<17>(q, std::make_integer_sequence<int, 17>{});
    const RegArr<9> a8 = reg_sel<9, 8>(all, (d0 & 8) != 0, std::make_integer_sequence<int, 9>{});
    const RegArr<5> a4 = reg_sel<5, 4>(a8, (d0 & 4) != 0, std::make_integer_sequence<int, 5>{});
    const RegArr<3> a2 = reg_sel<3, 2>(a4, (d0 & 2) != 0, std::make_integer_sequence<int, 3>{});
    const RegArr<2> a1 = reg_sel<2, 1>(a2, (d0 & 1) != 0, std::make_integer_sequence<int, 2>{});
    return __builtin_amdgcn_alignbit(a1.v[1], a1.v[0], (pos & 3) * 8);
}
struct RegTimeText {
    uint32_t w[8];
    DEV uint32_t operator[](uint32_t o) const {
        const uint32_t u = (uint32_t) __builtin_amdgcn_readfirstlane((int) o);
        uint32_t d;
        switch (u >> 2) {
        case 0: d = w[0]; break; case 1: d = w[1]; break; case 2: d = w[2]; break; case 3: d = w[3]; break;
        case 4: d = w[4]; break; case 5: d = w[5]; break; case 6: d = w[6]; break; default: d = w[7]; break;
        }
        return (d >> (8 * (u & 3))) & 255u;
    }
};

struct RuleText { int f; uint32_t b; v4u32 w; };
template <bool UNGUARDED = false, class CV>
DEV int tc_rule_match(const TileRule &ru, const GrepRule *grules, int i, uint32_t drop, const uint8_t *val, const CV &caps, LDS_AS const uint8_t *pg_lds,
                      const RuleText rt = RuleText{-1, 0, (v4u32) (0)}) {
    const uint32_t m = ru.fmask & ~drop;
// ... 98 lines not shown
    return true;
}

DEV v4u32 lds_ldu128(LDS_AS const uint8_t *p) {
    typedef v4u32 v4u32u __attribute__((aligned(1)));
    return *(LDS_AS const v4u32u *) p;
}

__device__ __noinline__ uint32_t locate_core_ool(const ParserMatchArgs *ap, uint64_t r, const uint8_t *rec, const uint8_t *rec_end, uint32_t *n_dec, RecInfo *ri) {
    uint32_t nd = *n_dec;
    RecInfo t = *ri;
    const uint32_t ol = locate_core(*ap, r, rec, rec_end, nd, t);
    *n_dec = nd; *ri = t;
    return ol;
}

template <bool SLOW, bool STAGE = false, int FXK = 0, int TB = REG_THREADS>
#ifdef REG_WAVES_PER_EU
__global__ void __launch_bounds__(TB) __attribute__((amdgpu_waves_per_eu(REG_WAVES_PER_EU, REG_WAVES_PER_EU))) k_parser_reg(ParserMatchArgs a) {
#else
__global__ void __launch_bounds__(TB) k_parser_reg(ParserMatchArgs a) {
#endif
    const uint32_t lane = threadIdx.x & 63, wave = threadIdx.x >> 6;
    LDS_AS uint8_t *lds = (LDS_AS uint8_t *) g_lds;
    const DevParser &ps = a.parsers[0];
    constexpr bool FX3 = FXK >= 3, FX4 = FXK >= 4, FX5 = FXK == 5;
    constexpr bool PK = FX4;
    const DevFx fx = FX3 ? ps.fx2 : ps.fx;
    const bool sparse = !STAGE && a.n < (((uint64_t) gridDim.x * blockDim.x) >> 6) * 64;
    const uint32_t wave_slot = sparse ? wave * gridDim.x + blockIdx.x : (blockIdx.x * blockDim.x + threadIdx.x) >> 6;
    if (a.fix_list != nullptr) {
        bool idle;
        if constexpr (SLOW) {
            LDS_AS uint32_t *flag = (LDS_AS uint32_t *) lds;
            if (threadIdx.x == 0) *flag = 0;
            __syncthreads();
            const uint64_t nw_ = ((uint64_t) gridDim.x * blockDim.x) >> 6;
            if (lane == 0 && (sparse ? ((const uint32_t *) a.fix_count)[wave_slot] != 0 : wave_slot < ((const uint32_t *) a.fix_count)[2 * nw_])) *flag = 1;
            __syncthreads();
            idle = *flag == 0;
            __syncthreads();
        }
        else idle = (uint64_t) (sparse ? blockIdx.x : blockIdx.x * (blockDim.x >> 6)) * 64 >= a.n;
        if (idle) {
            if (!SLOW && lane == 0) ((uint32_t *) a.fix_count)[wave_slot] = 0;
            return;
        }
    }
    {
        typedef uint32_t v4u __attribute__((ext_vector_type(4)));
        const v4u *src = (const v4u *) fx.base;
        LDS_AS v4u *dst = (LDS_AS v4u *) g_lds;
        for (uint32_t i = threadIdx.x; i < fx.bytes / 16; i += blockDim.x) dst[i] = src[i];
        if (a.pg) {
            LDS_AS uint8_t *pg_lds = lds + a.pg_lds_off;
            for (int i = 0; i < a.pg->nrules; i++) {
                if (a.pg->rule_lds_off[i] == 0xFFFFFFFFu) continue;
                const uint8_t *rs = a.pg->rules[i].dfa.cls;
                for (uint32_t k = threadIdx.x; k < a.pg->rule_lds_bytes[i]; k += blockDim.x) pg_lds[a.pg->rule_lds_off[i] + k] = rs[k];
            }
        }
        if (STAGE && a.stage_nbuf && threadIdx.x == 0) *(LDS_AS uint32_t *) (lds + a.stage_lds_off) = (1u << a.stage_nbuf) - 1u;
        __syncthreads();
    }
    if ((uint32_t) (uintptr_t) lds != 0) __builtin_trap();
#define CFG(member) ((uint32_t) a.tc.member)
    LDS_AS uint8_t *wbase = lds + a.tile_lds_off + wave * a.tile_wave_bytes;
    constexpr uint32_t CAP_STEP = FX4 ? 2u : FX_CAP_STRIDE;
    LDS_AS uint8_t *capcol = FX4 ? wbase + lane * 68u : wbase + ((lane & 31) << 2) + ((lane >> 5) << 1);
    CapLds capl;
    capl.base = capcol; capl.stride_b = CAP_STEP;
    const uint64_t nwaves = ((uint64_t) gridDim.x * blockDim.x) >> 6;
    uint16_t *chk = a.chk + ((size_t) wave_slot * a.chk_len) * 64 + lane;
    const uint8_t *data_end = a.data + a.bytes;
    const int ncap = 2 * a.tc.nfields, tc_nfields = a.tc.nfields;
    const bool size_from_columns = !a.cfg.reserve_data && !(a.cfg.preserve_key && !a.cfg.key.is_ra) && a.tc.plain_types;
    const uint32_t klen = (uint32_t) a.cfg.key.key_len;
    const bool fast_layout = !a.cfg.key.is_ra && klen >= 1 && klen <= 15;
    const bool map32 = a.n > 0 && a.row_off[1] - a.row_off[0] > 13 && a.data[a.row_off[0] + 12] == 0xdf;
    const uint32_t vh_at = (map32 ? 23u : 15u) + klen;
    const uint32_t p2_at = fx.off_p2;
    const uint64_t n = a.n;
    uint32_t n_dec = 0, n_gen = 0, n_fin = 0, n_slow = 0, n_loc = 0, pg_out = 0, pg_keep = 0, pg_pending = 0;
    unsigned long long pg_bytes = 0;
    uint32_t trace_it = 0;
    const uint32_t trace_n = a.trace_iters & 0x7FFFFFFFu;
    const bool trace_me = a.trace != nullptr && SLOW == ((a.trace_iters >> 31) != 0);
#define REG_TRACE_(k) if ((k) < 8 && trace_me && trace_it < trace_n) { __builtin_amdgcn_s_waitcnt(0); if (lane == 0) a.trace[((uint64_t) wave_slot * trace_n + trace_it) * 8 + (k)] = __builtin_amdgcn_s_memtime(); }
#ifdef REG_TRACE_FINE
#define REG_TRACE(k) REG_TRACE_((k) == 0 ? 0 : (k) == 4 ? 1 : (k) >= 5 ? (k) : 8)
#define REG_TRACEF(k) REG_TRACE_(k)
#else
#define REG_TRACE(k) REG_TRACE_(k)
#define REG_TRACEF(k)
#endif
    uint64_t po0 = 0, po1 = 0, prow = 0;
    const uint32_t *perm = SLOW ? nullptr : a.perm;
    if constexpr (!SLOW) {
        const uint64_t r0 = (uint64_t) wave_slot * 64 + lane;
        if (r0 < n) { prow = perm ? (uint64_t) perm[r0] : r0; po0 = a.row_off[prow]; po1 = a.row_off[prow + 1]; }
    }
    unsigned long long len_max = 0, len_sum = 0;
    const bool len_note = !SLOW && !perm && a.len_stat != nullptr && (wave_slot & 7) == 0;
    const bool listed = a.fix_list != nullptr;
    const uint64_t fix_stride = ((n + nwaves * 64 - 1) / (nwaves * 64)) * 64;
    uint32_t *my_fix = listed ? a.fix_list + (uint64_t) wave_slot * fix_stride : nullptr;
    uint32_t *fix_cnt = (uint32_t *) a.fix_count;
    uint32_t nfix = 0;
    const uint32_t *fix_pre = fix_cnt + nwaves;
    const bool dealt = SLOW && listed && !sparse;
    const uint64_t nloop = (SLOW && listed) ? (dealt ? (uint64_t) fix_pre[nwaves] : (uint64_t) fix_cnt[wave_slot]) : n;
    for (uint64_t base = SLOW ? (listed ? (dealt ? (uint64_t) wave_slot : 0) : (a.fix_first & ~63ull) + (uint64_t) wave_slot * 64) : (uint64_t) wave_slot * 64; base < nloop;
         base += (SLOW && listed) ? (dealt ? nwaves : 64) : nwaves * 64, trace_it++) {
        uint64_t r = base + lane;
        bool act = r < nloop;
        if (SLOW && listed && !dealt) { r = act ? (uint64_t) my_fix[r] : 0; act = act && r < n; }
        if (dealt) {
            uint32_t lo = 0, hi = (uint32_t) nwaves;
            while (hi - lo > 1) { const uint32_t mid = (lo + hi) >> 1; if (fix_pre[mid] <= (uint32_t) base) lo = mid; else hi = mid; }
            const uint32_t at = ((uint32_t) base - fix_pre[lo]) * 64 + lane;
            act = at < fix_cnt[lo];
            r = act ? (uint64_t) a.fix_list[(uint64_t) lo * fix_stride + at] : 0;
            act = act && r < n;
        }
        REG_TRACE(0)
        if constexpr (SLOW) { act = act && (a.info[r] & RF_NEEDLOC); if (!__ballot(act)) continue; }
        bool to_fix = false;
        RecInfo ri;
        recinfo_init(ri);
        uint32_t out_len = 0;
        uint64_t o0 = 0, o1 = 0;
        if constexpr (SLOW) { if (act) { o0 = a.row_off[r]; o1 = a.row_off[r + 1]; } }
        else {
            o0 = po0; o1 = po1;
            const uint64_t rn = r + nwaves * 64;
            if (act) r = prow;
            po0 = po1 = 0;
            if (rn < n) { prow = perm ? (uint64_t) perm[rn] : rn; po0 = a.row_off[prow]; po1 = a.row_off[prow + 1]; }
        }
        const uint8_t *recg = a.data + o0;
        const uint32_t rlen = (uint32_t) (o1 - o0);
        v4u32 q[18];
        #pragma unroll
        for (uint32_t k = 0; k < 18; k++) q[k] = (v4u32) (0);
        v4u32 pn0 = (v4u32) (0), pn1 = (v4u32) (0), pn2 = (v4u32) (0), pn3 = (v4u32) (0);
        constexpr bool STREAMW = REG_STREAM && !SLOW && !STAGE;
        if constexpr (!SLOW) {
            if (act && recg + rlen + 400 > data_end) recg = (a.tail_buf && o0 >= a.tail_start) ? a.tail_buf + (o0 - a.tail_start) : nullptr;
        }
        const bool try_fast = !SLOW && act && fast_layout && rlen >= vh_at + 2 && rlen < 0x10000u && recg != nullptr;
        const uint32_t vspan = rlen - (vh_at + 1);
        const uint32_t voff_p = vh_at + (vspan <= 31 ? 1u : vspan <= 256 ? 2u : 3u);
        uint32_t hw[12] = {0, 0, 0, 0, 0, 0, 0, 0, 0, 0, 0, 0};
        const uint32_t maxr = wave_umax(try_fast ? rlen : 0);
        if (len_note) { len_max += (unsigned long long) maxr * (unsigned) __builtin_popcountll(__ballot(try_fast)); if (try_fast) len_sum += rlen; }
        REG_TRACE(1)
        v4u32 h0 = (v4u32) (0), h1 = (v4u32) (0), h2 = (v4u32) (0);
        bool staged = false;
        if constexpr (STAGE) {
            const uint32_t cnt = (uint32_t) ((n - base) < 64 ? (n - base) : 64);
            if (a.stage_nbuf && cnt > 0) {
                const uint64_t wend = __shfl(o1, (int) (cnt - 1), 64);
                if (__ballot(try_fast) && wend + 32 <= a.bytes) {
                    LDS_AS uint32_t *smask = (LDS_AS uint32_t *) (lds + a.stage_lds_off);
                    int sbuf = 0;
                    if (lane == 0) {
                        for (;;) {
// ... 368 lines not shown
                    for (int f = 0; f < 16; f++) if (f < tc_nfields) field(f, cb[f], ce[f]);
                    for (int f = 16; f < tc_nfields; f++) field(f, capl.get((uint32_t) (2 * f)) & UNSET, capl.get((uint32_t) (2 * f + 1)) & UNSET);
                }
                REG_TRACEF(4)
                uint32_t ytext = 0;
                const bool ycheck = !SLOW && CFG(defer_time) && time_here && !(flags & RF_BADTS);
                if (ycheck) {
                    if (ytb == tb) ytext = ytext_q;
                    else ytext = ldu32(val + tb + CFG(year_off));
                }
                auto text_from_memory = [&]() {
                    const v4u32 t0 = load16(val + tb, 0, tfl), t1 = load16(val + tb + 16, 0, tfl > 16 ? tfl - 16 : 0);
                    tt.w[0] = t0.x; tt.w[1] = t0.y; tt.w[2] = t0.z; tt.w[3] = t0.w; tt.w[4] = t1.x; tt.w[5] = t1.y; tt.w[6] = t1.z; tt.w[7] = t1.w;
                };
                if constexpr (SLOW) { if (time_here && !tt_ok && !(a.debug_skip & 64)) text_from_memory(); }
                uint32_t pgbits = 0;
                if (CFG(pg_on) && any && !(CFG(pg_named) & CFG(pg_time_fields) & ~pgdrop) && !(a.debug_skip & 16)) {
                    TileCaps cv{capl};
                    LDS_AS const uint8_t *pg_lds = (LDS_AS const uint8_t *) (lds + a.pg_lds_off);
                    const bool keep = tc.pg_fast ? tc_grep_parsed<!SLOW>(tc, a.pg->rules, pgdrop, val, cv, pg_lds, rt)
                                                 : pg_grep_parsed<true>(a.pg->rules, a.pg->nrules, a.pg->logical_op, a.pg->rule_fmask, a.pg->rule_lds_off, pgdrop, val, cv, pg_lds);
                    pgbits = RF_PGDONE | (keep ? RF_PGKEEP : 0u);
                }
                bool defer = false;
                if (ycheck && (pgbits & RF_PGDONE) && !slow) {
                    const uint32_t t7 = ytext & 0x7F7F7F7Fu, isd = (t7 + 0x50505050u) & ~(t7 + 0x46464646u) & ~ytext & 0x80808080u;
                    const uint32_t year = (ytext & 15u) * 1000u + ((ytext >> 8) & 15u) * 100u + ((ytext >> 16) & 15u) * 10u + ((ytext >> 24) & 15u);
                    defer = isd == 0x80808080u && year >= 1971u && year <= 2105u;
                }
                if constexpr (!SLOW) { if (time_here && !defer && !tt_ok && !(a.debug_skip & 64)) text_from_memory(); }
                REG_TRACE(5)
                if (defer) pgbits |= RF_TIMEPEND;
                if (time_here && !defer && !(a.debug_skip & 32)) {
                    int64_t s2 = 0;
                    bool tok;
                    if constexpr (FX3) {
                        LDS_AS const uint32_t *ctp = (LDS_AS const uint32_t *) (lds + (fx.bytes - 128u));
                        tok = ctp[31] ? time_fast_compiled(ctp, (int) CFG(time_with_tz), (int) CFG(time_offset), tt.w, &s2) : time_fast_plan(tc.plan, tc.time_with_tz, tc.time_offset, tt, &s2);
                    }
                    else tok = time_fast_plan(tc.plan, tc.time_with_tz, tc.time_offset, tt, &s2);
                    if (tok) sec = s2;
                    else slow = true;
                }
                REG_TRACE(6)
                flags |= pgbits;
                if (!any) {
                    if (a.cfg.nparsers > 1) { flags |= RF_GENERIC; n_gen++; }
                }
                else if (slow) {
                    n_fin++;
                    will_finish = true;
                    if (tc.time_field >= 0) {
                        const uint32_t tb2 = capl.get((uint32_t) (2 * tc.time_field)), te = capl.get((uint32_t) (2 * tc.time_field + 1));
                        if (tb2 != CAP_UNSET && te != CAP_UNSET && te - tb2 <= 4 * TBUF_WORDS) {
                            const uint32_t tl = te - tb2;
                            v4u32 w0 = load16(val + tb2, 0, tl), w1 = load16(val + tb2 + 16, 0, tl > 16 ? tl - 16 : 0);
                            a.tbuf[0 * n + r] = w0.x; a.tbuf[1 * n + r] = w0.y; a.tbuf[2 * n + r] = w0.z; a.tbuf[3 * n + r] = w0.w;
                            a.tbuf[4 * n + r] = w1.x; a.tbuf[5 * n + r] = w1.y; a.tbuf[6 * n + r] = w1.z; a.tbuf[7 * n + r] = w1.w;
                        }
                    }
                }
                else {
                    done = true;
                    if (!a.cfg.key.is_ra) null_note(a.cfg, r, ri.key_index, null_mask);
                    int64_t tsec = ri.ts_sec, tnsec = ri.ts_nsec;
                    if (flags & RF_BADTS) { tsec = -3; tnsec = 0; }
                    if (sec != 0) { tsec = sec; tnsec = 0; }
                    flags = (flags | RF_PARSED) & ~(uint32_t) RF_BADTS;
                    ri.parser_idx = 0; ri.nkept = kept; ri.drop_mask = drop;
                    if (encoder_refuses_time(tsec, tnsec)) {
                        flags |= RF_BADTS;
                        out_len = 0;
                        keep_len = 0;
                    }
                    else {
                        ri.ts_sec = (uint32_t) tsec; ri.ts_nsec = (uint32_t) tnsec;
                        if ((uint32_t) tsec >= 0xfffffffeu) atomicAdd(&a.counts[14], 1ull);
                        const uint32_t n0 = CFG(nregs_minus1);
                        out_len = 12 + ri.meta_canon + (n0 < 16 ? 1 : n0 < 65536 ? 3 : 5) + body_bytes;
                        if (a.pg_keep_len) {
                            if (pgbits & RF_PGDONE) {
                                const bool keep = (pgbits & RF_PGKEEP) != 0;
                                keep_len = keep ? out_len : 0;
                                pg_out++; pg_bytes += out_len; pg_keep += keep ? 1u : 0u;
                            }
                            else pg_pending++;
                        }
                    }
                }
            }
            else if (cand && (endb == -2 || a.cfg.nparsers > 1)) {
                flags |= RF_GENERIC;
                n_gen++;
            }
            ri.flags = flags;
            if (!done) {
                if (!will_finish) {
                    if (!(flags & RF_GENERIC)) a.null_mask[r] = 0;
                    if (a.pg_keep_len) { a.pg_keep_len[r] = PG_UNDECIDED; pg_pending++; }
                }
                rec_store(a.info, n, r, ri);
                a.out_len[r] = out_len;
                if (caps_valid) for (int c = 0; c < ncap; c++) a.caps[(uint64_t) c * n + r] = capl.get((uint32_t) c);
            }
            else {
                const bool dropped = a.pg_keep_len && keep_len == 0 && !(a.debug_skip & 8);
                if (a.pg_keep_len) a.pg_keep_len[r] = keep_len;
                if (dropped) a.info[r] = flags;
                else if (a.desc && a.pg_keep_len && keep_len != PG_UNDECIDED) {
                    a.info[r] = flags | RF_DESC;
                    v4u32 *dp = (v4u32 *) (a.desc + (uint64_t) r * a.dstride);
                    v4u32 d0; d0.x = ri.ts_sec; d0.y = ri.ts_nsec; d0.z = ri.val_off; d0.w = ri.drop_mask;
                    dp[0] = d0;
                    if constexpr (PK) {
                        #pragma unroll
                        for (uint32_t k = 1; k < 8; k++) {
                            if (4 * k >= a.dstride) break;
                            uint32_t wv[4];
                            #pragma unroll
                            for (uint32_t j = 0; j < 4; j++) {
                                const uint32_t di = 4 * k + j;
                                if (di == 4) wv[j] = ri.meta_off;
                                else if (di == 5) wv[j] = ri.meta_len;
                                else if (di == 6) wv[j] = ri.nkept;
                                else {
                                    const uint32_t f = di - 7;
                                    wv[j] = (f < 16 && (int) f < tc_nfields) ? __builtin_amdgcn_alignbit(cdw[f + 1 <= 16 ? f + 1 : 16], cdw[f <= 16 ? f : 16], 16) : 0xFFFFFFFFu;
                                }
                            }
                            v4u32 dv; dv.x = wv[0]; dv.y = wv[1]; dv.z = wv[2]; dv.w = wv[3];
                            dp[k] = dv;
                        }
                    }
                    else
                    for (uint32_t k = 1; 4 * k < a.dstride; k++) {
                        uint32_t wv[4];
                        #pragma unroll
                        for (uint32_t j = 0; j < 4; j++) {
                            const uint32_t di = 4 * k + j;
                            if (di == 4) wv[j] = ri.meta_off;
                            else if (di == 5) wv[j] = ri.meta_len;
                            else if (di == 6) wv[j] = ri.nkept;
                            else {
                                const uint32_t c = 2 * (di - 7);
                                const uint32_t lo16 = (int) c < ncap ? capl.get(c) & 0xFFFFu : 0xFFFFu, hi16 = (int) (c + 1) < ncap ? capl.get(c + 1) & 0xFFFFu : 0xFFFFu;
                                wv[j] = lo16 | (hi16 << 16);
                            }
                        }
                        v4u32 dv; dv.x = wv[0]; dv.y = wv[1]; dv.z = wv[2]; dv.w = wv[3];
                        dp[k] = dv;
                    }
                }
                else {
                    rec_store(a.info, n, r, ri);
                    a.null_mask[r] = null_mask;
                    a.out_len[r] = out_len;
                    for (int c = 0; c < ncap; c++) a.caps[(uint64_t) c * n + r] = capl.get((uint32_t) c);
                }
            }
        }
        REG_TRACE(7)
    }
    for (int o = 32; o > 0; o >>= 1) {
        n_dec += __shfl_down(n_dec, o, 64); n_gen += __shfl_down(n_gen, o, 64); n_fin += __shfl_down(n_fin, o, 64); n_slow += __shfl_down(n_slow, o, 64);
        n_loc += __shfl_down(n_loc, o, 64);
        pg_out += __shfl_down(pg_out, o, 64); pg_keep += __shfl_down(pg_keep, o, 64); pg_pending += __shfl_down(pg_pending, o, 64);
        pg_bytes += __shfl_down(pg_bytes, o, 64);
    }
    if (!SLOW && listed && lane == 0) fix_cnt[wave_slot] = nfix;
    if (len_note) {
        for (int o = 32; o > 0; o >>= 1) len_sum += __shfl_down(len_sum, o, 64);
        if (lane == 0 && len_sum) { atomicAdd(&a.len_stat[0], len_max); atomicAdd(&a.len_stat[1], len_sum); }
    }
    if (lane == 0) {
        if (n_dec) atomicAdd(&a.counts[0], (unsigned long long) n_dec);
        if (n_gen) atomicAdd(&a.counts[2], (unsigned long long) n_gen);
        if (n_fin) atomicAdd(&a.counts[8], (unsigned long long) n_fin);
        if (n_slow) atomicAdd(&a.counts[9], (unsigned long long) n_slow);
        if (n_loc) atomicAdd(&a.counts[10], (unsigned long long) n_loc);
        if (pg_bytes) atomicAdd(&a.counts[4], pg_bytes);
        if (pg_keep) atomicAdd(&a.counts[5], (unsigned long long) pg_keep);
        if (pg_out) atomicAdd(&a.counts[6], (unsigned long long) pg_out);
        if (pg_pending) atomicAdd(&a.counts[7], (unsigned long long) pg_pending);
    }
}
#undef CFG
#undef REG_TRACE
#undef REG_TRACEF
#undef REG_TRACE_
#undef REG_HB

__global__ void __launch_bounds__(1024) k_fix_prefix(uint32_t *fix_cnt, uint32_t nw) {
    __shared__ uint32_t wsum[16];
    uint32_t *pre = fix_cnt + nw;
    const uint32_t per = (nw + 1023) / 1024, i0 = threadIdx.x * per;
    uint32_t mine = 0;
    for (uint32_t i = i0; i < i0 + per && i < nw; i++) mine += (fix_cnt[i] + 63) / 64;
    uint32_t incl = mine;
    const uint32_t lane = threadIdx.x & 63, wave = threadIdx.x >> 6;
    for (int o = 1; o < 64; o <<= 1) { const uint32_t t = __shfl_up(incl, o, 64); if (lane >= (uint32_t) o) incl += t; }
    if (lane == 63) wsum[wave] = incl;
    __syncthreads();
    uint32_t before = incl - mine;
    for (uint32_t w = 0; w < wave; w++) before += wsum[w];
    for (uint32_t i = i0; i < i0 + per && i < nw; i++) { pre[i] = before; before += (fix_cnt[i] + 63) / 64; }
    if (threadIdx.x == 1023) pre[nw] = before;
}

void launch_parser_reg(const ParserMatchArgs &a, int grid, int threads, bool fixup, hipStream_t st) {
    static std::atomic<bool> attr_set{false};
    if (!attr_set) {
        (void) hipFuncSetAttribute((const void *) k_parser_reg<false, false>, hipFuncAttributeMaxDynamicSharedMemorySize, 160 * 1024);
        (void) hipFuncSetAttribute((const void *) k_parser_reg<false, true>, hipFuncAttributeMaxDynamicSharedMemorySize, 160 * 1024);
        (void) hipFuncSetAttribute((const void *) k_parser_reg<true, false>, hipFuncAttributeMaxDynamicSharedMemorySize, 160 * 1024);
        (void) hipFuncSetAttribute((const void *) k_parser_reg<false, false, 3>, hipFuncAttributeMaxDynamicSharedMemorySize, 160 * 1024);
        (void) hipFuncSetAttribute((const void *) k_parser_reg<true, false, 3>, hipFuncAttributeMaxDynamicSharedMemorySize, 160 * 1024);
        (void) hipFuncSetAttribute((const void *) k_parser_reg<false, false, 4>, hipFuncAttributeMaxDynamicSharedMemorySize, 160 * 1024);
        (void) hipFuncSetAttribute((const void *) k_parser_reg<true, false, 4>, hipFuncAttributeMaxDynamicSharedMemorySize, 160 * 1024);
        (void) hipFuncSetAttribute((const void *) k_parser_reg<false, false, 3, 768>, hipFuncAttributeMaxDynamicSharedMemorySize, 160 * 1024);
        (void) hipFuncSetAttribute((const void *) k_parser_reg<false, false, 4, 768>, hipFuncAttributeMaxDynamicSharedMemorySize, 160 * 1024);
        (void) hipFuncSetAttribute((const void *) k_parser_reg<false, false, 5>, hipFuncAttributeMaxDynamicSharedMemorySize, 160 * 1024);
        (void) hipFuncSetAttribute((const void *) k_parser_reg<true, false, 5>, hipFuncAttributeMaxDynamicSharedMemorySize, 160 * 1024);
        (void) hipFuncSetAttribute((const void *) k_parser_reg<false, false, 5, 768>, hipFuncAttributeMaxDynamicSharedMemorySize, 160 * 1024);
        (void) hipFuncSetAttribute((const void *) k_parser_reg<true, false, 4, 768>, hipFuncAttributeMaxDynamicSharedMemorySize, 160 * 1024);
        (void) hipFuncSetAttribute((const void *) k_parser_reg<true, false, 5, 768>, hipFuncAttributeMaxDynamicSharedMemorySize, 160 * 1024);
        attr_set = true;
    }
    if (getenv("FLBGPU_DEBUG_LDS")) fprintf(stderr, "k_parser_reg%s: grid %d x %d threads, lds_total %u, tables up to %u, %u a wave, fx2 %u\n", fixup ? " (fix-up)" : "", grid, threads, a.lds_total, a.tile_lds_off, a.tile_wave_bytes, a.use_fx2);
    if (fixup && a.fix_list && a.n >= (uint64_t) grid * (uint64_t) threads) hipLaunchKernelGGL(k_fix_prefix, dim3(1), dim3(1024), 0, st, (uint32_t *) a.fix_count, (uint32_t) (((uint64_t) grid * (uint64_t) threads) >> 6));
    static const bool fix768 = !(getenv("FLBGPU_FIXUP_1024") && atoi(getenv("FLBGPU_FIXUP_1024")) != 0);
    if (a.use_fx2 == 5) {
        if (fixup && threads <= 768 && fix768) hipLaunchKernelGGL((k_parser_reg<true, false, 5, 768>), dim3(grid), dim3(threads), a.lds_total, st, a);
        else if (fixup) hipLaunchKernelGGL((k_parser_reg<true, false, 5>), dim3(grid), dim3(threads), a.lds_total, st, a);
        else if (threads <= 768) hipLaunchKernelGGL((k_parser_reg<false, false, 5, 768>), dim3(grid), dim3(threads), a.lds_total, st, a);
        else hipLaunchKernelGGL((k_parser_reg<false, false, 5>), dim3(grid), dim3(threads), a.lds_total, st, a);
        return;
    }
    if (a.use_fx2 == 4) {
        if (fixup && threads <= 768 && fix768) hipLaunchKernelGGL((k_parser_reg<true, false, 4, 768>), dim3(grid), dim3(threads), a.lds_total, st, a);
        else if (fixup) hipLaunchKernelGGL((k_parser_reg<true, false, 4>), dim3(grid), dim3(threads), a.lds_total, st, a);
        else if (threads <= 768) hipLaunchKernelGGL((k_parser_reg<false, false, 4, 768>), dim3(grid), dim3(threads), a.lds_total, st, a);
        else hipLaunchKernelGGL((k_parser_reg<false, false, 4>), dim3(grid), dim3(threads), a.lds_total, st, a);
        return;
    }
    if (a.use_fx2) {
        if (fixup) hipLaunchKernelGGL((k_parser_reg<true, false, 3>), dim3(grid), dim3(threads), a.lds_total, st, a);
        else if (threads <= 768) hipLaunchKernelGGL((k_parser_reg<false, false, 3, 768>), dim3(grid), dim3(threads), a.lds_total, st, a);
        else hipLaunchKernelGGL((k_parser_reg<false, false, 3>), dim3(grid), dim3(threads), a.lds_total, st, a);
        return;
    }
    if (fixup) hipLaunchKernelGGL((k_parser_reg<true, false>), dim3(grid), dim3(threads), a.lds_total, st, a);
    else if (a.stage_nbuf) hipLaunchKernelGGL((k_parser_reg<false, true>), dim3(grid), dim3(threads), a.lds_total, st, a);
    else hipLaunchKernelGGL((k_parser_reg<false, false>), dim3(grid), dim3(threads), a.lds_total, st, a);
}

void launch_parser_tile(const ParserMatchArgs &a, int grid, int threads, hipStream_t st) {
    static std::atomic<bool> attr_set{false};
    if (!attr_set) {
        (void) hipFuncSetAttribute((const void *) k_parser_tile, hipFuncAttributeMaxDynamicSharedMemorySize, 160 * 1024);
        attr_set = true;
    }
    hipLaunchKernelGGL(k_parser_tile, dim3(grid), dim3(threads), a.lds_total, st, a);
}
```

include/flb_gpu.h:

```cpp
#ifndef FLB_GPU_H
#define FLB_GPU_H

#include <stddef.h>
#include <stdint.h>

#ifdef __cplusplus
extern "C" {
#endif

#define FLBGPU_FILTER_MODIFIED 1
#define FLBGPU_FILTER_NOTOUCH  2

typedef struct flbgpu_parser flbgpu_parser;
typedef struct flbgpu_filter flbgpu_filter;

typedef struct flbgpu_dev_chunk {
    const void *data;
    const uint64_t *row_off;
    uint64_t n;
    uint64_t bytes;
} flbgpu_dev_chunk;

int flbgpu_init(int device);
const char *flbgpu_last_error(void);
// ... 112 lines not shown
typedef struct flbgpu_ml_stream flbgpu_ml_stream;
flbgpu_ml_parser *flbgpu_ml_parser_create(const char *type, const char *match_string, int negate, const char *key_content, int64_t buffer_limit);
int flbgpu_ml_parser_add_rule(flbgpu_ml_parser *p, const char *from_states, const char *regex, const char *to_state);
int flbgpu_ml_parser_builtin(flbgpu_ml_parser *p, const char *name);
int flbgpu_ml_parser_set_subparser(flbgpu_ml_parser *p, flbgpu_parser *sub, const char *key_group, const char *key_pattern);
int flbgpu_ml_parser_init(flbgpu_ml_parser *p);
void flbgpu_ml_parser_destroy(flbgpu_ml_parser *p);
void flbgpu_ml_parser_product(const flbgpu_ml_parser *p, uint32_t *states, uint32_t *classes, uint32_t *live);
flbgpu_ml_stream *flbgpu_ml_stream_create(flbgpu_ml_parser *p);
void flbgpu_ml_stream_destroy(flbgpu_ml_stream *s);
void flbgpu_ml_stream_state(const flbgpu_ml_stream *s, int *rule_to_state, uint64_t *buffered);
uint64_t flbgpu_ml_stream_truncations(const flbgpu_ml_stream *s);
int flbgpu_ml_append(flbgpu_ml_stream *s, const void *text, size_t bytes, uint32_t ts_sec, uint32_t ts_nsec, int skip_empty_lines, int flush,
                     void **out_buf, size_t *out_size, uint64_t *processed, uint64_t *records);
int flbgpu_ml_append_dev(flbgpu_ml_stream *s, const void *d_text, uint64_t bytes, uint32_t ts_sec, uint32_t ts_nsec, int skip_empty_lines, int flush,
                         flbgpu_dev_chunk *out, uint64_t *processed, uint64_t *records);
typedef struct flbgpu_ml_list flbgpu_ml_list;
flbgpu_ml_list *flbgpu_ml_list_create(flbgpu_ml_stream **streams, int n);
void flbgpu_ml_list_destroy(flbgpu_ml_list *l);
int flbgpu_ml_list_lru(const flbgpu_ml_list *l);
int flbgpu_ml_list_append(flbgpu_ml_list *l, const void *text, size_t bytes, uint32_t ts_sec, uint32_t ts_nsec, int skip_empty_lines, int flush,
                          void **out_buf, size_t *out_size, uint64_t *processed, uint64_t *records);
int flbgpu_ml_list_append_dev(flbgpu_ml_list *l, const void *d_text, uint64_t bytes, uint32_t ts_sec, uint32_t ts_nsec, int skip_empty_lines, int flush,
                              flbgpu_dev_chunk *out, uint64_t *processed, uint64_t *records);

int64_t flbgpu_split_lines_host(const void *data, size_t bytes, uint64_t *row_off, size_t cap);

typedef struct flbgpu_sp flbgpu_sp;
flbgpu_sp *flbgpu_sp_create(const char *sql, int str_conv);
void flbgpu_sp_destroy(flbgpu_sp *t);
int flbgpu_sp_info(const flbgpu_sp *t, int *window_type, int64_t *window_sec, int *source_type, const char **source, const char **stream_name);
const char *flbgpu_sp_stream_prop(const flbgpu_sp *t, const char *key);
void flbgpu_sp_set_tag(flbgpu_sp *t, const char *tag, size_t len);
int flbgpu_sp_select_only(const flbgpu_sp *t);
int flbgpu_sp_key_count(const flbgpu_sp *t);
const char *flbgpu_sp_key_name(const flbgpu_sp *t, int i);
int flbgpu_sp_do(flbgpu_sp *t, const void *data, size_t bytes, uint32_t now_sec, uint32_t now_nsec, void **out_buf, size_t *out_size,
                 int64_t *records);
int flbgpu_sp_do_dev(flbgpu_sp *t, const flbgpu_dev_chunk *in, void *stream, uint32_t now_sec, uint32_t now_nsec, void **out_buf,
                     size_t *out_size, int64_t *records);
int flbgpu_sp_select_dev(flbgpu_sp *t, const flbgpu_dev_chunk *in, void *stream, uint32_t now_sec, uint32_t now_nsec, flbgpu_dev_chunk *out,
                         int64_t *records);
int flbgpu_sp_timer(flbgpu_sp *t, uint32_t now_sec, uint32_t now_nsec, void **out_buf, size_t *out_size);
int flbgpu_sp_hop(flbgpu_sp *t);
int64_t flbgpu_sp_window_advance(const flbgpu_sp *t);
int flbgpu_sp_parse_check(const char *sql, char *desc, size_t cap);
void flbgpu_sp_set_index_base(flbgpu_sp *t, uint64_t base);
int64_t flbgpu_sp_export(flbgpu_sp *t, void *buf, size_t cap);
int flbgpu_sp_package_merged(flbgpu_sp *t, const void *const *snaps, const size_t *sizes, int n, uint32_t now_sec, uint32_t now_nsec,
                             void **out_buf, size_t *out_size);
int flbgpu_sp_timer_all_reduce(flbgpu_sp *t, void *rccl_comm, void *stream, uint32_t now_sec, uint32_t now_nsec, void **out_buf,
                               size_t *out_size);
void flbgpu_sp_profile(flbgpu_sp *t, int enable, double *ms2, uint64_t *launches2);

int64_t flbgpu_index_host(const void *data, size_t bytes, uint64_t *row_off, size_t cap, size_t *consumed);
int flbgpu_tail_clean_host(const void *data, size_t bytes, size_t consumed);

typedef struct flbgpu_indexer flbgpu_indexer;
flbgpu_indexer *flbgpu_indexer_create(void);
void flbgpu_indexer_destroy(flbgpu_indexer *ix);
int64_t flbgpu_index_dev(flbgpu_indexer *ix, const void *dev_data, size_t bytes, flbgpu_dev_chunk *out, size_t *consumed);
void flbgpu_indexer_stats(const flbgpu_indexer *ix, uint64_t *candidates, uint64_t *off_chain_rows, uint64_t *rounds);

void *flbgpu_dev_alloc(size_t bytes);
void flbgpu_dev_free(void *p);
int flbgpu_memcpy_h2d(void *dst, const void *src, size_t bytes);
int flbgpu_memcpy_d2h(void *dst, const void *src, size_t bytes);
int flbgpu_sync(void);

void *flbgpu_rx_compile(const char *pattern, int len, unsigned options, int want_captures, char *err, int errlen);
void flbgpu_rx_free(void *h);
int flbgpu_rx_simulate_capture(void *h, const char *s, int len, int *beg, int *end);
int flbgpu_rx_simulate_match(void *h, const char *s, int len);
void flbgpu_rx_info(void *h, int *info12);
int flbgpu_rx_names(void *h, char *buf, int cap);
int flbgpu_host_phases(double *out, int cap);

void *flbgpu_rxbt_compile(const char *pattern, int len, unsigned options, char *err, int errlen);
void flbgpu_rxbt_free(void *h);
int flbgpu_rxbt_search(void *h, const char *s, int len, int *beg, int *end);
int flbgpu_rx_is_nonregular(const char *pattern, int len, unsigned options);
void flbgpu_diag_copy(void *dst, const void *src, size_t n);
uint64_t flbgpu_diag_fused_failures(void);
int flbgpu_rx_simulate_fx(void *h, const char *s, int len, int *beg, int *end);
int flbgpu_rx_simulate_fx2(void *h, const char *s, int len, int *beg, int *end);
int flbgpu_rx_simulate_fx_walk_all(void *h, const char *s, int len, int *beg, int *end);
int flbgpu_rx_simulate_fx3(void *h, const char *s, int len, int *beg, int *end, int *info2);
int flbgpu_rx_fx_tail(void *h, const char *s, int len, int *nkill, unsigned char *kill4, int *first);
int flbgpu_rx_fx_profile(void *h, const char *s, int len, long *out);
void flbgpu_rx_debug_stats(long *out3);
int flbgpu_rx_engine(void *h, int *info6, char *why, int whylen);
int flbgpu_rx_corner(void *h, const char *s, int len, int *flags);
int flbgpu_rx_sample(const char *pattern, int len, unsigned options, unsigned long long seed, char *out, int cap);

int flbgpu_nc_scan_double(const char *s, int len, int mode, int exact, double *out, int *consumed);
int flbgpu_nc_fmt_f6(double v, char *buf, int cap);
int flbgpu_nc_fmt_json_double(double v, int nan_to_null, char *buf);
int flbgpu_nc_fmt_ld(long long v, char *buf);
int flbgpu_nc_scan_double_dev(const char *strs, const uint32_t *off, uint32_t n, int mode, uint64_t *bits, int *consumed);

int flbgpu_calib_run(int mode, void *dev_in, void *dev_out, uint64_t n, int cus);

#ifdef __cplusplus
}
#endif
#endif
```

Baseline: 4.900 billion.

## Fuse keep-length scan into a single-pass plain emit kernel with decoupled lookback

Adds a one-pass emit kernel that computes row output offsets with a tile-level decoupled lookback prefix sum and assembles kept records through an LDS staging buffer. This removes the separate scan kernel and its extra pass over keep lengths and offsets. The decide kernels now also accumulate total kept bytes, so the host can size the output buffer before emitting. Rows the fast path cannot handle fall back to the general emit kernel, and a stuck lookback falls back to the old scan-then-emit path. The change also adds a host-side record assembly entry point.

```diff
diff --git a/fluent-bit_amd/__init__.py b/fluent-bit_amd/__init__.py
--- a/fluent-bit_amd/__init__.py
+++ b/fluent-bit_amd/__init__.py
@@ -240,7 +240,7 @@
         o = (ctypes.c_uint64 * 8)()
         lib().flbgpu_filter_paths(self.h, o)
         lp = int(o[0])
-        return dict(single_pass=bool(lp & 1), three_port=bool(lp & 2), emit_time=bool(lp & 4), plain_emit=bool(lp & 8), rows_by_length=bool(lp & 16),
+        return dict(single_pass=bool(lp & 1), three_port=bool(lp & 2), emit_time=bool(lp & 4), plain_emit=bool(lp & 8), rows_by_length=bool(lp & 16), one_pass_emit=bool(lp & 32),
                     aside=dict(single_pass=bool(o[1]), three_port=bool(o[2]), emit_time=bool(o[3]), plain_emit=bool(o[4])),
                     tries=int(o[5]), returns=int(o[6]), calls=int(o[7]))
 
diff --git a/fluent-bit_amd/csrc/flbgpu.cpp b/fluent-bit_amd/csrc/flbgpu.cpp
--- a/fluent-bit_amd/csrc/flbgpu.cpp
+++ b/fluent-bit_amd/csrc/flbgpu.cpp
@@ -994,7 +994,7 @@
     delete p;
 }
 
-struct MiscWords { unsigned long long first_bad; unsigned long long max_row; unsigned long long counts[18]; unsigned int ov_count; unsigned int kept_count; };
+struct MiscWords { unsigned long long first_bad; unsigned long long max_row; unsigned long long counts[24]; unsigned int ov_count; unsigned int kept_count; };
 static const unsigned int OV_CAP = 1u << 16;
 
 struct PairCtx { PgInline pg; uint32_t *keep_len; const flbgpu_filter *fg; uint32_t *desc; uint32_t dstride; };
@@ -1975,7 +1975,11 @@
 static std::atomic<uint64_t> g_fused_failures{0};
 extern "C" uint64_t flbgpu_diag_fused_failures(void) { return g_fused_failures.load(); }
 
-namespace flbgpu { void launch_pg_emit_plain(const PgEmitArgs &a, int nfields, int cus, hipStream_t st); }
+namespace flbgpu {
+void launch_pg_emit_plain(const PgEmitArgs &a, int nfields, int cus, hipStream_t st);
+size_t pg_emit_onepass_units(uint64_t n);
+void launch_pg_emit_onepass(const PgEmitArgs &a, unsigned long long *lb, int nfields, int cus, hipStream_t st);
+}
 
 static int run_pair_fused(flbgpu_filter *fp, flbgpu_filter *fg, const flbgpu_dev_chunk *in, flbgpu_dev_chunk *out, flbgpu_chain_stat *stats2) {
     hipStream_t st = fp->stream;
@@ -2026,8 +2030,6 @@
         if (da.lds_total + pc.pg.rule_lds_bytes[i] <= 48 * 1024) { da.rule_lds_off[i] = da.lds_total; da.rule_lds_bytes[i] = pc.pg.rule_lds_bytes[i]; da.lds_total += (pc.pg.rule_lds_bytes[i] + 15) & ~15u; }
     }
     da.keep_len = pc.keep_len; da.counts = dm->counts;
-    if (ahead || hm.counts[7] > 0 || hm.counts[2] > 0) { ProfScope ps(fp, st, "k_pg_decide"); launch_pg_decide(da, cus, st); }
-    { ProfScope ps(fp, st, "k_scan"); launch_scan(da.keep_len, n, fp->d_scan_tmp.as<uint64_t>(), fp->d_off.as<uint64_t>(), st); }
     total = 0;
     auto emit_args = [&](PgEmitArgs &ea) {
         memset(&ea, 0, sizeof(ea));
@@ -2051,6 +2053,48 @@
         return use;
     };
     auto plain_result = [&](unsigned long long left, unsigned long long kept) { if (left * 16 > kept && kept >= 64) fp->plain.bad(); else fp->plain.good(); };
+    int plain_known = -1;
+    if (!ahead && hm.counts[7] == 0 && hm.counts[2] == 0 && pc.desc != nullptr && (n >> 40) == 0 && !(getenv("FLBGPU_PG_ONEPASS") && getenv("FLBGPU_PG_ONEPASS")[0] == '0')) {
+        if (hm.counts[6] == 0 || hm.counts[5] == hm.counts[6] || hm.counts[14] > 0) return 0;
+        auto answer = [&]() {
+            total = hm.counts[18];
+            fp->last_in = hm.counts[0]; fp->last_out = hm.counts[6];
+            fg->last_in = hm.counts[6]; fg->last_out = hm.counts[5];
+            if (stats2) {
+                stats2[0].ret = FLBGPU_FILTER_MODIFIED; stats2[0].in_records = hm.counts[0]; stats2[0].out_records = hm.counts[6]; stats2[0].out_bytes = hm.counts[4];
+                stats2[1].ret = FLBGPU_FILTER_MODIFIED; stats2[1].in_records = hm.counts[6]; stats2[1].out_records = hm.counts[5]; stats2[1].out_bytes = total;
+            }
+            memset(out, 0, sizeof(*out));
+        };
+        if (hm.counts[18] == 0) { answer(); return 1; }
+        PgEmitArgs ea;
+        emit_args(ea);
+        plain_known = plain_wanted(ea) ? 1 : 0;
+        const size_t units = pg_emit_onepass_units(n);
+        if (plain_known == 1 && fp->d_units.ensure(units * 8)) {
+            answer();
+            if (!fg->d_out.ensure(total + 16)) return -1;
+            ea.out = fg->d_out.as<uint8_t>(); ea.out_cap = total;
+            if (hipMemsetAsync(fp->d_units.p, 0, units * 8, st) != hipSuccess) return -1;
+            { ProfScope ps(fp, st, "k_pg_emit"); launch_pg_emit_onepass(ea, fp->d_units.as<unsigned long long>(), d0.nfields, cus, st); }
+            const unsigned long long kept = hm.counts[5];
+            if (hipMemcpyAsync(&hm, dm, sizeof(hm), hipMemcpyDeviceToHost, st) != hipSuccess || hipStreamSynchronize(st) != hipSuccess) return -1;
+            if (hm.counts[20] == 0) {
+                fp->last_path |= 32u;
+                if (defer_failed(hm.counts[13])) return run_pair_fused(fp, fg, in, out, stats2);
+                plain_result(hm.counts[15], kept);
+                if (hm.counts[15] > 0) {
+                    { ProfScope ps(fp, st, "k_pg_emit_general"); launch_pg_emit(ea, d0.nfields, cus, st); }
+                    if (hipStreamSynchronize(st) != hipSuccess) return -1;
+                }
+                out->data = fg->d_out.p; out->row_off = fp->d_off.as<uint64_t>(); out->n = n; out->bytes = total;
+                return 1;
+            }
+            if (hipMemsetAsync(&dm->counts[13], 0, 3 * sizeof(unsigned long long), st) != hipSuccess) return -1;
+        }
+    }
+    if (ahead || hm.counts[7] > 0 || hm.counts[2] > 0) { ProfScope ps(fp, st, "k_pg_decide"); launch_pg_decide(da, cus, st); }
+    { ProfScope ps(fp, st, "k_scan"); launch_scan(da.keep_len, n, fp->d_scan_tmp.as<uint64_t>(), fp->d_off.as<uint64_t>(), st); }
     if (ahead) {
         if (!fg->d_out.ensure(in->bytes * 2 + n * 64 + 65536 + 16)) return -1;
         PgEmitArgs ea;
@@ -2094,7 +2138,7 @@
     if (!fg->d_out.ensure(total + 16)) return -1;
     PgEmitArgs ea;
     emit_args(ea);
-    const bool plain_emit = plain_wanted(ea);
+    const bool plain_emit = plain_known >= 0 ? plain_known == 1 : plain_wanted(ea);
     { ProfScope ps(fp, st, "k_pg_emit"); if (plain_emit) launch_pg_emit_plain(ea, d0.nfields, cus, st); else launch_pg_emit(ea, d0.nfields, cus, st); }
     unsigned long long *c13 = (unsigned long long *) (fp->hp_misc.as<uint8_t>() + sizeof(MiscWords) + sizeof(uint64_t));
     c13[0] = c13[1] = c13[2] = 0;
diff --git a/fluent-bit_amd/csrc/fused_kernels.inc b/fluent-bit_amd/csrc/fused_kernels.inc
--- a/fluent-bit_amd/csrc/fused_kernels.inc
+++ b/fluent-bit_amd/csrc/fused_kernels.inc
@@ -205,6 +205,181 @@
     }
 }
 
+constexpr int PG1_BATCH = 64;
+constexpr int PG1_STG = 18 * 1024;
+template <bool PLAIN, int TILE>
+__global__ void __launch_bounds__(256, 4) k_pg_emit(PgEmitArgs a, unsigned long long *lb) {
+    static_assert(PLAIN && TILE % 1024 == 0 && TILE <= 65536, "the plain shape; a thread owns a multiple of four rows; u16 row numbers");
+    constexpr uint32_t RPT = TILE / 256;
+    const uint32_t tid = threadIdx.x, lane = tid & 63, wave = tid >> 6;
+    const uint32_t nf = (uint32_t) a.ec.nfields, dn4 = (7 + nf + 3) & ~3u, slot_dw = dn4 + 4;
+    LDS_AS uint32_t *m32 = (LDS_AS uint32_t *) g_lds;
+    LDS_AS unsigned long long *m64 = (LDS_AS unsigned long long *) (g_lds + 16);
+    LDS_AS uint32_t *wcnt = (LDS_AS uint32_t *) (g_lds + 64);
+    LDS_AS uint16_t *q_row = (LDS_AS uint16_t *) (g_lds + 96);
+    LDS_AS uint32_t *q_off = (LDS_AS uint32_t *) (g_lds + 96 + TILE * 2);
+    LDS_AS uint32_t *slots = (LDS_AS uint32_t *) (g_lds + 96 + TILE * 2 + TILE * 4 + 16);
+    LDS_AS uint8_t *stg = (LDS_AS uint8_t *) (slots + PG1_BATCH * slot_dw);
+    uint64_t *out_off = const_cast<uint64_t *>(a.out_off);
+    const uint64_t ntiles = (a.n + TILE - 1) / TILE;
+    if (tid == 0) m32[1] = 0;
+    for (;;) {
+        if (tid == 0) { const unsigned long long t = atomicAdd(&a.counts[19], 1ull); m32[0] = t < ntiles ? (uint32_t) t : 0xFFFFFFFFu; }
+        __syncthreads();
+        const uint32_t tile = m32[0];
+        if (tile == 0xFFFFFFFFu || m32[1]) break;
+        const uint64_t r0 = (uint64_t) tile * TILE + (uint64_t) tid * RPT;
+        uint32_t kl[RPT];
+        if (r0 + RPT <= a.n) {
+            #pragma unroll
+            for (uint32_t j = 0; j < RPT; j += 4) {
+                const v4u32 x = *(const v4u32 *) (a.keep_len + r0 + j);
+                kl[j] = x.x; kl[j + 1] = x.y; kl[j + 2] = x.z; kl[j + 3] = x.w;
+            }
+        }
+        else {
+            #pragma unroll
+            for (uint32_t j = 0; j < RPT; j++) kl[j] = r0 + j < a.n ? a.keep_len[r0 + j] : 0;
+        }
+        uint64_t tsum = 0;
+        uint32_t tcnt = 0;
+        #pragma unroll
+        for (uint32_t j = 0; j < RPT; j++) { tsum += kl[j]; tcnt += kl[j] != 0; }
+        uint64_t wincl = tsum;
+        #pragma unroll
+        for (int o = 1; o < 64; o <<= 1) { const uint64_t up = __shfl_up(wincl, o, 64); if (lane >= (uint32_t) o) wincl += up; }
+        const uint32_t cincl = jt_dpp_add(tcnt);
+        if (lane == 63) { m64[1 + wave] = wincl; wcnt[wave] = cincl; }
+        __syncthreads();
+        uint64_t woff = 0, tile_sum = 0;
+        uint32_t qoff = 0, cnt = 0;
+        #pragma unroll
+        for (uint32_t w = 0; w < 4; w++) {
+            const uint64_t ws = m64[1 + w];
+            const uint32_t wc = wcnt[w];
+            if (w < wave) { woff += ws; qoff += wc; }
+            tile_sum += ws; cnt += wc;
+        }
+        if (wave == 0) {
+            bool stuck = false;
+            const uint64_t prefix = lb_unit_base(lb, tile, tile_sum, lane, stuck);
+            if (lane == 0) {
+                m64[0] = prefix;
+                if (stuck) { m32[1] = 1; atomicAdd(&a.counts[20], 1ull); }
+            }
+        }
+        __syncthreads();
+        if (m32[1]) break;
+        const uint64_t tbase = m64[0];
+        {
+            uint64_t loc = woff + (wincl - tsum);
+            uint32_t qp = qoff + (cincl - tcnt);
+            uint64_t oo[RPT];
+            #pragma unroll
+            for (uint32_t j = 0; j < RPT; j++) {
+                oo[j] = tbase + loc;
+                if (kl[j]) { q_row[qp] = (uint16_t) (tid * RPT + j); q_off[qp] = (uint32_t) loc; qp++; }
+                loc += kl[j];
+            }
+            if (r0 + RPT <= a.n + 1) {
+                typedef unsigned long long v2u64 __attribute__((ext_vector_type(2)));
+                #pragma unroll
+                for (uint32_t j = 0; j < RPT; j += 2) { v2u64 v; v.x = oo[j]; v.y = oo[j + 1]; *(v2u64 *) (out_off + r0 + j) = v; }
+            }
+            else {
+                #pragma unroll
+                for (uint32_t j = 0; j < RPT; j++) if (r0 + j <= a.n) out_off[r0 + j] = oo[j];
+            }
+            if (tid == 255) {
+                if (r0 + RPT == a.n) out_off[a.n] = tbase + loc;
+                q_off[cnt] = (uint32_t) tile_sum;
+            }
+        }
+        __syncthreads();
+        if (tile_sum >> 32) {
+            if (tid == 0 && cnt) atomicAdd(&a.counts[15], (unsigned long long) cnt);
+            cnt = 0;
+        }
+        uint32_t lo = 0;
+        while (lo < cnt) {
+            const uint32_t bb = q_off[lo];
+            const uint32_t align = (uint32_t) ((tbase + bb) & 15);
+            const uint32_t mmax = cnt - lo < (uint32_t) PG1_BATCH ? cnt - lo : (uint32_t) PG1_BATCH;
+            uint32_t m = 0;
+            #pragma unroll
+            for (uint32_t step = PG1_BATCH; step; step >>= 1) {
+                const uint32_t t = m + step;
+                if (t <= mmax && q_off[lo + t] - bb + align <= (uint32_t) PG1_STG) m = t;
+            }
+            if (m == 0) {
+                if (tid == 0) atomicAdd(&a.counts[15], 1ull);
+                lo++;
+                continue;
+            }
+            {
+                const uint32_t i = tid >> 2, part = tid & 3;
+                if (i < m) {
+                    const uint64_t r = (uint64_t) tile * TILE + q_row[lo + i];
+                    const uint32_t *dp = a.desc + r * a.dstride;
+                    LDS_AS uint32_t *sl = slots + i * slot_dw;
+                    for (uint32_t c = part; 4 * c < dn4; c += 4) *(LDS_AS v4u32 *) (sl + 4 * c) = *(const v4u32 *) (dp + 4 * c);
+                    if (part == 1) { const uint64_t ro = a.row_off[r]; sl[dn4] = (uint32_t) ro; sl[dn4 + 1] = (uint32_t) (ro >> 32); }
+                    if (part == 2) sl[dn4 + 2] = a.info[r];
+                }
+            }
+            __syncthreads();
+            if (tid < m) {
+                LDS_AS uint32_t *sl = slots + tid * slot_dw;
+                const uint32_t fl = sl[dn4 + 2];
+                const bool take = (fl & RF_DESC) && (fl & RF_PARSED) && a.ec.ok;
+                if (!take) atomicAdd(&a.counts[15], 1ull);
+                else if (fl & RF_TIMEPEND) {
+                    const DevParser &ps = a.parsers[0];
+                    const uint32_t tb = ((LDS_AS const uint16_t *) (sl + 7))[2 * (uint32_t) ps.time_field];
+                    const uint64_t roff = (uint64_t) sl[dn4] | ((uint64_t) sl[dn4 + 1] << 32);
+                    int64_t tsec = sl[0], tnsec = sl[1];
+                    int64_t s2 = 0;
+                    const bool tok = pge_time(a.data, a.bytes, roff + sl[2] + tb, &ps, &s2);
+                    if (tok && s2 != 0) { tsec = s2; tnsec = 0; }
+                    if (!tok || encoder_refuses_time(tsec, tnsec)) atomicAdd(&a.counts[13], 1ull);
+                    else { sl[0] = (uint32_t) tsec; sl[1] = (uint32_t) tnsec; }
+                }
+                sl[dn4 + 3] = take ? 1u : 0u;
+            }
+            __syncthreads();
+            for (uint32_t i = tid >> 4; i < m; i += 16) {
+                LDS_AS const uint32_t *sl = slots + i * slot_dw;
+                if (!sl[dn4 + 3]) continue;
+                RecInfo ri;
+                ri.flags = sl[dn4 + 2]; ri.ts_sec = sl[0]; ri.ts_nsec = sl[1]; ri.val_off = sl[2]; ri.drop_mask = sl[3];
+                ri.meta_off = sl[4]; ri.meta_len = sl[5]; ri.nkept = sl[6];
+                const uint64_t roff = (uint64_t) sl[dn4] | ((uint64_t) sl[dn4 + 1] << 32);
+                const uint32_t o0 = q_off[lo + i], o1 = q_off[lo + i + 1];
+                pg_assemble(stg + align + (o0 - bb), o1 - o0, a.ec, ri, (LDS_AS const uint16_t *) (sl + 7), a.data + roff, a.data + a.bytes, tid & 15, 16u);
+            }
+            __syncthreads();
+            {
+                const uint32_t total = q_off[lo + m] - bb;
+                uint8_t *dst = a.out + (tbase + bb - align);
+                const uint32_t n16 = (align + total + 15) / 16;
+                if (tbase + bb + total > a.out_cap) { if (tid == 0) atomicAdd(&a.counts[20], 1ull << 32); }
+                else
+                for (uint32_t u = tid; u < n16; u += 256) {
+                    const uint32_t b0 = u * 16, b1 = b0 + 16;
+                    if (b0 >= align && b1 <= align + total) *(v4u32 *) (dst + b0) = *(LDS_AS v4u32 *) (stg + b0);
+                    else {
+                        const uint32_t s0 = b0 < align ? align : b0, s1 = b1 > align + total ? align + total : b1;
+                        for (uint32_t qq = s0; qq < s1; qq++) dst[qq] = stg[qq];
+                    }
+                }
+            }
+            __syncthreads();
+            lo += m;
+        }
+        __syncthreads();
+    }
+}
+
 void launch_pg_decide(const PgDecideArgs &a, int cus, hipStream_t st) {
     if (a.n == 0) return;
     uint64_t blocks = (a.n + 255) / 256, cap = (uint64_t) cus * 16;
@@ -228,3 +403,18 @@
 }
 void launch_pg_emit(const PgEmitArgs &a, int nfields, int cus, hipStream_t st) { launch_pg_emit_t(a, nfields, cus, st, false); }
 void launch_pg_emit_plain(const PgEmitArgs &a, int nfields, int cus, hipStream_t st) { launch_pg_emit_t(a, nfields, cus, st, true); }
+constexpr int PG1_TILE = 2048;
+size_t pg_emit_onepass_units(uint64_t n) { return ((size_t) ((n + PG1_TILE - 1) / PG1_TILE) + 2) & ~(size_t) 1; }
+void launch_pg_emit_onepass(const PgEmitArgs &a, unsigned long long *lb, int nfields, int cus, hipStream_t st) {
+    if (a.n == 0) return;
+    static std::atomic<bool> attr_set{false};
+    if (!attr_set) {
+        (void) hipFuncSetAttribute((const void *) k_pg_emit<true, PG1_TILE>, hipFuncAttributeMaxDynamicSharedMemorySize, 160 * 1024);
+        attr_set = true;
+    }
+    const uint32_t slot_dw = ((7 + (uint32_t) nfields + 3) & ~3u) + 4;
+    const size_t lds = 96 + (size_t) PG1_TILE * 6 + 16 + (size_t) PG1_BATCH * slot_dw * 4 + PG1_STG + 16;
+    uint64_t blocks = (a.n + PG1_TILE - 1) / PG1_TILE, cap = (uint64_t) cus * 4;
+    if (blocks > cap) blocks = cap;
+    hipLaunchKernelGGL((k_pg_emit<true, PG1_TILE>), dim3((unsigned) blocks), dim3(256), lds, st, a, lb);
+}
diff --git a/fluent-bit_amd/csrc/kdev.inc b/fluent-bit_amd/csrc/kdev.inc
--- a/fluent-bit_amd/csrc/kdev.inc
+++ b/fluent-bit_amd/csrc/kdev.inc
@@ -1,8 +1,13 @@
 
+#ifndef KDEV_HOST_SUBSET
 #define DEV __device__ __forceinline__
+#define DEVNI __device__ __noinline__
+#endif
 #define LDS_AS __attribute__((address_space(3)))
 
+#ifndef KDEV_HOST_SUBSET
 extern __shared__ __attribute__((aligned(16))) uint8_t g_lds[];
+#endif
 
 DEV uint32_t ld8(const uint8_t *p) { return *p; }
 DEV uint32_t ldu32(const uint8_t *p) {
@@ -256,7 +261,7 @@
 }
 
 constexpr uint32_t MP_MAX_OPEN = 32;
-__device__ __noinline__ bool mp_depth_ok(const uint8_t *p, const uint8_t *end, uint32_t open);
+DEVNI bool mp_depth_ok(const uint8_t *p, const uint8_t *end, uint32_t open);
 
 DEV const uint8_t *mp_skip(const uint8_t *p, const uint8_t *end, uint32_t open = 2) {
     const uint8_t *p0 = p;
@@ -325,7 +330,7 @@
     return p;
 }
 
-__device__ __noinline__ bool mp_depth_ok(const uint8_t *p, const uint8_t *end, uint32_t open) {
+DEVNI bool mp_depth_ok(const uint8_t *p, const uint8_t *end, uint32_t open) {
     uint64_t stk[MP_MAX_OPEN];
     uint64_t cur = 1;
     uint32_t top = 0;
@@ -347,6 +352,7 @@
     }
 }
 
+#ifndef KDEV_HOST_SUBSET
 struct Event {
     uint32_t flags;
     int64_t sec, nsec;
@@ -1710,6 +1716,7 @@
     }
 }
 
+#endif
 template <class S, class CV>
 DEV void write_record_plain(S &s, const EmitCfg &ec, const uint8_t *rec, const RecInfo &ri, const CV &caps) {
     s.put32(0x00d79292u); s.put32(__builtin_bswap32(ri.ts_sec)); s.put32(__builtin_bswap32(ri.ts_nsec));
@@ -1731,6 +1738,85 @@
     }
 }
 
+DEV void pga_st32(uint8_t *p, uint32_t v) { typedef uint32_t u32u __attribute__((aligned(1))); *(u32u *) p = v; }
+DEV void pga_st32(LDS_AS uint8_t *p, uint32_t v) { typedef uint32_t u32u __attribute__((aligned(1))); *(LDS_AS u32u *) p = v; }
+template <class D>
+struct SeqSink {
+    D p, lim;
+    DEV SeqSink(D dst, D end) : p(dst), lim(end) {}
+    DEV void note_exact() {}
+    DEV void put(uint32_t b) { if (p < lim) *p = (uint8_t) b; p++; }
+    DEV void copy(const uint8_t *src, uint32_t len) { for (uint32_t i = 0; i < len; i++) put(ld8(src + i)); }
+    DEV void words(const uint32_t *w, uint32_t nbytes) { for (uint32_t i = 0; i < nbytes; i++) put((w[i >> 2] >> (8 * (i & 3))) & 0xff); }
+    DEV void put32(uint32_t v) { for (uint32_t i = 0; i < 4; i++) put((v >> (8 * i)) & 0xff); }
+    DEV void put16(const v4u32 w, uint32_t nbytes) { for (uint32_t i = 0; i < nbytes; i++) put(v4_byte(w, i)); }
+    DEV void finish() {}
+};
+template <class D>
+DEV void pga_piece(D dst, const uint8_t *src, uint32_t nb, const uint8_t *src_end) {
+    typedef v4u32 v4u32u __attribute__((aligned(1)));
+    uint32_t wd[4] = {0, 0, 0, 0};
+    if (src + 16 <= src_end) { const v4u32 w = *(const v4u32u *) src; wd[0] = w.x; wd[1] = w.y; wd[2] = w.z; wd[3] = w.w; }
+    else {
+        #pragma unroll
+        for (uint32_t k = 0; k < 4; k++) {
+            #pragma unroll
+            for (uint32_t q = 0; q < 4; q++) if (4 * k + q < nb) wd[k] |= ld8(src + 4 * k + q) << (8 * q);
+        }
+    }
+    #pragma unroll
+    for (uint32_t k = 0; k < 4; k++) {
+        if (4 * k + 4 <= nb) pga_st32(dst + 4 * k, wd[k]);
+        else {
+            #pragma unroll
+            for (uint32_t q = 0; q < 4; q++) if (4 * k + q < nb) dst[4 * k + q] = (uint8_t) (wd[k] >> (8 * q));
+        }
+    }
+}
+template <class D, class SP>
+DEV void pg_assemble(D out, uint32_t total, const EmitCfg &ec, const RecInfo &ri, SP spans, const uint8_t *rec, const uint8_t *src_end,
+                     uint32_t sl, uint32_t nsl) {
+    uint32_t body = 0;
+    for (int f = 0; f < ec.nfields; f++) {
+        if ((ri.drop_mask >> f) & 1) continue;
+        const uint32_t b = spans[2 * f], e = spans[2 * f + 1];
+        const uint32_t vlen = (b != 0xFFFFu && e != 0xFFFFu) ? e - b : 0;
+        body += (uint32_t) ec.kw_bytes[f] + (vlen < 32 ? 1u : vlen < 256 ? 2u : 3u) + vlen;
+    }
+    if (body > total) return;
+    const uint32_t hdr = total - body;
+    if (sl == 0) {
+        SeqSink<D> s(out, out + hdr);
+        s.put32(0x00d79292u); s.put32(__builtin_bswap32(ri.ts_sec)); s.put32(__builtin_bswap32(ri.ts_nsec));
+        if (ri.meta_len > 1) mp_canon(rec + ri.meta_off, rec + ri.meta_off + ri.meta_len, s);
+        else s.put(0x80);
+        const uint32_t n0 = (uint32_t) ec.nregs_minus1;
+        if (n0 < 16) s.put(0x80 | ri.nkept);
+        else if (n0 < 65536) { s.put(0xde); pk_be(s, ri.nkept, 2); }
+        else { s.put(0xdf); pk_be(s, ri.nkept, 4); }
+    }
+    const uint8_t *val = rec + ri.val_off;
+    uint32_t pos = hdr, pc = 1;
+    for (int f = 0; f < ec.nfields; f++) {
+        if ((ri.drop_mask >> f) & 1) continue;
+        const uint32_t b = spans[2 * f], e = spans[2 * f + 1];
+        const bool set = b != 0xFFFFu && e != 0xFFFFu;
+        const uint32_t vlen = set ? e - b : 0;
+        const uint32_t kb = (uint32_t) ec.kw_bytes[f], khl = kb + (vlen < 32 ? 1u : vlen < 256 ? 2u : 3u);
+        if (pc % nsl == sl) {
+            SeqSink<D> s(out + pos, out + pos + khl);
+            s.words(ec.keywords + ec.kw_off[f], kb);
+            pk_str_hdr(s, vlen);
+        }
+        const uint8_t *v = set ? val + b : val;
+        for (uint32_t j = (sl + nsl - (pc + 1) % nsl) % nsl; 16 * j < vlen; j += nsl)
+            pga_piece(out + pos + khl + 16 * j, v + 16 * j, vlen - 16 * j < 16 ? vlen - 16 * j : 16u, src_end);
+        pos += khl + vlen;
+        pc += 1 + (vlen + 15) / 16;
+    }
+}
+
+#ifndef KDEV_HOST_SUBSET
 #include "nfa_dev.inc"
 
 
@@ -2089,3 +2175,6 @@
     }
     return out_len;
 }
+
+
+#endif
diff --git a/fluent-bit_amd/csrc/kernels.hip b/fluent-bit_amd/csrc/kernels.hip
--- a/fluent-bit_amd/csrc/kernels.hip
+++ b/fluent-bit_amd/csrc/kernels.hip
@@ -181,7 +181,7 @@
     __syncthreads();
     LDS_AS const char *lfmt1 = (LDS_AS const char *) fmt_mem, *lfmt2 = lfmt1 + MAX_TIMEFMT;
     uint32_t n_gen = 0, pg_out = 0, pg_keep = 0, pg_pending = 0;
-    unsigned long long pg_bytes = 0;
+    unsigned long long pg_bytes = 0, pg_kbytes = 0;
     const bool size_from_columns = !a.cfg.reserve_data && !(a.cfg.preserve_key && !a.cfg.key.is_ra) && ps.plain_types;
     const uint64_t n = a.n;
     for (uint64_t r = (uint64_t) blockIdx.x * blockDim.x + threadIdx.x; r < n; r += (uint64_t) gridDim.x * blockDim.x) {
@@ -272,7 +272,7 @@
             if (fl0 & RF_PGDONE) {
                 const bool keep = (fl0 & RF_PGKEEP) != 0;
                 a.pg_keep_len[r] = keep ? ol : 0;
-                pg_out++; pg_bytes += ol; pg_keep += keep ? 1u : 0u;
+                pg_out++; pg_bytes += ol; pg_keep += keep ? 1u : 0u; pg_kbytes += keep ? ol : 0u;
             }
             else { a.pg_keep_len[r] = PG_UNDECIDED; pg_pending++; }
         }
@@ -280,12 +280,13 @@
     for (int o = 32; o > 0; o >>= 1) {
         n_gen += __shfl_down(n_gen, o, 64);
         pg_out += __shfl_down(pg_out, o, 64); pg_keep += __shfl_down(pg_keep, o, 64); pg_pending += __shfl_down(pg_pending, o, 64);
-        pg_bytes += __shfl_down(pg_bytes, o, 64);
+        pg_bytes += __shfl_down(pg_bytes, o, 64); pg_kbytes += __shfl_down(pg_kbytes, o, 64);
     }
     if ((threadIdx.x & 63) == 0) {
         if (n_gen) atomicAdd(&a.counts[2], (unsigned long long) n_gen);
         if (pg_bytes) atomicAdd(&a.counts[4], pg_bytes);
         if (pg_keep) atomicAdd(&a.counts[5], (unsigned long long) pg_keep);
+        if (pg_kbytes) atomicAdd(&a.counts[18], pg_kbytes);
         if (pg_out) atomicAdd(&a.counts[6], (unsigned long long) pg_out);
         if (pg_pending) atomicAdd(&a.counts[7], (unsigned long long) pg_pending);
     }
diff --git a/fluent-bit_amd/csrc/kernels_fused.hip b/fluent-bit_amd/csrc/kernels_fused.hip
--- a/fluent-bit_amd/csrc/kernels_fused.hip
+++ b/fluent-bit_amd/csrc/kernels_fused.hip
@@ -1,6 +1,7 @@
 #include <hip/hip_runtime.h>
 #include <stdint.h>
 #include <string.h>
+#include <atomic>
 #include <type_traits>
 #include "dev.hpp"
 #include "numconv.hpp"
@@ -8,6 +9,7 @@
 namespace flbgpu {
 
 #include "kdev.inc"
+#include "lookback.inc"
 
 #include "fused_kernels.inc"
 
diff --git a/fluent-bit_amd/csrc/pg_assemble_host.cpp b/fluent-bit_amd/csrc/pg_assemble_host.cpp
--- /dev/null
+++ b/fluent-bit_amd/csrc/pg_assemble_host.cpp
@@ -0,0 +1,58 @@
+#include <stddef.h>
+#include <stdint.h>
+#include <string.h>
+#include "dev.hpp"
+#include "../../include/flb_gpu.h"
+
+namespace flbgpu {
+#define KDEV_HOST_SUBSET 1
+#define DEV inline
+#define DEVNI inline
+#include "kdev.inc"
+#undef DEV
+#undef DEVNI
+
+namespace {
+struct HostSpans {
+    const uint16_t *p;
+    uint32_t operator[](uint32_t i) const { return p[i] == 0xFFFF ? CAP_UNSET : p[i]; }
+};
+}
+}
+
+extern "C" int64_t flbgpu_pg_assemble_host(const void *rec, size_t rec_len, const uint32_t *hdr, int nfields, const uint16_t *spans,
+                                           const void *keys, const uint32_t *key_len, int nsl, void *out, size_t cap)
+{
+    using namespace flbgpu;
+    if (!rec || !hdr || !spans || !keys || !key_len || !out || nfields <= 0 || nfields > MAX_NAMES || nsl > 64 || nsl < -64) return -1;
+    EmitCfg ec;
+    memset(&ec, 0, sizeof(ec));
+    ec.ok = 1; ec.nfields = nfields; ec.nregs_minus1 = (int) hdr[7];
+    uint32_t at = 0;
+    const uint8_t *kp = (const uint8_t *) keys;
+    for (int f = 0; f < nfields; f++) {
+        const uint32_t nd = (key_len[f] + 3) / 4;
+        if (key_len[f] > 255 || at + nd > sizeof(ec.keywords) / 4 || at > 255) return -1;
+        ec.kw_off[f] = (uint8_t) at; ec.kw_bytes[f] = (uint8_t) key_len[f];
+        memcpy(ec.keywords + at, kp, key_len[f]);
+        kp += key_len[f]; at += nd;
+    }
+    RecInfo ri;
+    memset(&ri, 0, sizeof(ri));
+    ri.flags = RF_VALID | RF_PARSED | RF_DESC; ri.ts_sec = hdr[0]; ri.ts_nsec = hdr[1]; ri.val_off = hdr[2]; ri.drop_mask = hdr[3];
+    ri.meta_off = hdr[4]; ri.meta_len = hdr[5]; ri.nkept = hdr[6]; ri.parser_idx = 0;
+    const uint8_t *r = (const uint8_t *) rec;
+    HostSpans cv{spans};
+    CountSink cs;
+    write_record_plain(cs, ec, r, ri, cv);
+    if (cs.n > cap) return -2;
+    if (nsl == 0) {
+        ByteSink s((uint8_t *) out);
+        write_record_plain(s, ec, r, ri, cv);
+        return (int64_t) (s.p - (uint8_t *) out);
+    }
+    const int n = nsl < 0 ? -nsl : nsl;
+    for (int k = 0; k < n; k++)
+        pg_assemble((uint8_t *) out, (uint32_t) cs.n, ec, ri, spans, r, r + rec_len, (uint32_t) (nsl < 0 ? n - 1 - k : k), (uint32_t) n);
+    return (int64_t) cs.n;
+}
diff --git a/fluent-bit_amd/csrc/tile_kernels.inc b/fluent-bit_amd/csrc/tile_kernels.inc
--- a/fluent-bit_amd/csrc/tile_kernels.inc
+++ b/fluent-bit_amd/csrc/tile_kernels.inc
@@ -102,7 +102,7 @@
     const bool size_from_columns = !a.cfg.reserve_data && !(a.cfg.preserve_key && !a.cfg.key.is_ra) && ps.plain_types;
     const uint64_t n = a.n;
     uint32_t n_dec = 0, n_gen = 0, n_fin = 0, n_slow = 0, pg_out = 0, pg_keep = 0, pg_pending = 0;
-    unsigned long long pg_bytes = 0;
+    unsigned long long pg_bytes = 0, pg_kbytes = 0;
     for (uint64_t base = (uint64_t) wave_slot * 64; base < n; base += nwaves * 64) {
         const uint64_t r = base + lane;
         const uint32_t cnt = (uint32_t) ((n - base) < 64 ? (n - base) : 64);
@@ -253,7 +253,7 @@
                                 if (pgbits & RF_PGDONE) {
                                     const bool keep = (pgbits & RF_PGKEEP) != 0;
                                     keep_len = keep ? out_len : 0;
-                                    pg_out++; pg_bytes += out_len; pg_keep += keep ? 1u : 0u;
+                                    pg_out++; pg_bytes += out_len; pg_keep += keep ? 1u : 0u; pg_kbytes += keep_len;
                                 }
                                 else pg_pending++;
                             }
@@ -293,7 +293,7 @@
     for (int o = 32; o > 0; o >>= 1) {
         n_dec += __shfl_down(n_dec, o, 64); n_gen += __shfl_down(n_gen, o, 64); n_fin += __shfl_down(n_fin, o, 64); n_slow += __shfl_down(n_slow, o, 64);
         pg_out += __shfl_down(pg_out, o, 64); pg_keep += __shfl_down(pg_keep, o, 64); pg_pending += __shfl_down(pg_pending, o, 64);
-        pg_bytes += __shfl_down(pg_bytes, o, 64);
+        pg_bytes += __shfl_down(pg_bytes, o, 64); pg_kbytes += __shfl_down(pg_kbytes, o, 64);
     }
     if (lane == 0) {
         if (n_dec) atomicAdd(&a.counts[0], (unsigned long long) n_dec);
@@ -302,6 +302,7 @@
         if (n_slow) atomicAdd(&a.counts[9], (unsigned long long) n_slow);
         if (pg_bytes) atomicAdd(&a.counts[4], pg_bytes);
         if (pg_keep) atomicAdd(&a.counts[5], (unsigned long long) pg_keep);
+        if (pg_kbytes) atomicAdd(&a.counts[18], pg_kbytes);
         if (pg_out) atomicAdd(&a.counts[6], (unsigned long long) pg_out);
         if (pg_pending) atomicAdd(&a.counts[7], (unsigned long long) pg_pending);
     }
@@ -566,7 +567,7 @@
     const uint32_t p2_at = fx.off_p2;
     const uint64_t n = a.n;
     uint32_t n_dec = 0, n_gen = 0, n_fin = 0, n_slow = 0, n_loc = 0, pg_out = 0, pg_keep = 0, pg_pending = 0;
-    unsigned long long pg_bytes = 0;
+    unsigned long long pg_bytes = 0, pg_kbytes = 0;
     uint32_t trace_it = 0;
     const uint32_t trace_n = a.trace_iters & 0x7FFFFFFFu;
     const bool trace_me = a.trace != nullptr && SLOW == ((a.trace_iters >> 31) != 0);
@@ -1101,7 +1102,7 @@
                             if (pgbits & RF_PGDONE) {
                                 const bool keep = (pgbits & RF_PGKEEP) != 0;
                                 keep_len = keep ? out_len : 0;
-                                pg_out++; pg_bytes += out_len; pg_keep += keep ? 1u : 0u;
+                                pg_out++; pg_bytes += out_len; pg_keep += keep ? 1u : 0u; pg_kbytes += keep_len;
                             }
                             else pg_pending++;
                         }
@@ -1184,7 +1185,7 @@
         n_dec += __shfl_down(n_dec, o, 64); n_gen += __shfl_down(n_gen, o, 64); n_fin += __shfl_down(n_fin, o, 64); n_slow += __shfl_down(n_slow, o, 64);
         n_loc += __shfl_down(n_loc, o, 64);
         pg_out += __shfl_down(pg_out, o, 64); pg_keep += __shfl_down(pg_keep, o, 64); pg_pending += __shfl_down(pg_pending, o, 64);
-        pg_bytes += __shfl_down(pg_bytes, o, 64);
+        pg_bytes += __shfl_down(pg_bytes, o, 64); pg_kbytes += __shfl_down(pg_kbytes, o, 64);
     }
     if (!SLOW && listed && lane == 0) fix_cnt[wave_slot] = nfix;
     if (len_note) {
@@ -1199,6 +1200,7 @@
         if (n_loc) atomicAdd(&a.counts[10], (unsigned long long) n_loc);
         if (pg_bytes) atomicAdd(&a.counts[4], pg_bytes);
         if (pg_keep) atomicAdd(&a.counts[5], (unsigned long long) pg_keep);
+        if (pg_kbytes) atomicAdd(&a.counts[18], pg_kbytes);
         if (pg_out) atomicAdd(&a.counts[6], (unsigned long long) pg_out);
         if (pg_pending) atomicAdd(&a.counts[7], (unsigned long long) pg_pending);
     }
diff --git a/include/flb_gpu.h b/include/flb_gpu.h
--- a/include/flb_gpu.h
+++ b/include/flb_gpu.h
@@ -218,6 +218,8 @@
 int flbgpu_rx_is_nonregular(const char *pattern, int len, unsigned options);
 void flbgpu_diag_copy(void *dst, const void *src, size_t n);
 uint64_t flbgpu_diag_fused_failures(void);
+int64_t flbgpu_pg_assemble_host(const void *rec, size_t rec_len, const uint32_t *hdr, int nfields, const uint16_t *spans,
+                                const void *keys, const uint32_t *key_len, int nsl, void *out, size_t cap);
 int flbgpu_rx_simulate_fx(void *h, const char *s, int len, int *beg, int *end);
 int flbgpu_rx_simulate_fx2(void *h, const char *s, int len, int *beg, int *end);
 int flbgpu_rx_simulate_fx_walk_all(void *h, const char *s, int len, int *beg, int *end);
```

Result: slower. 3.463 billion (-29.3%).
